# yhinai/EIG-KL-Algorithm

Measured on AMD Instinct MI355X. Metric: wall-clock to final cut (s) + cut size, ibm18.hgr; SpMV GB/s vs HBM peak, lower is better.
Workload: dtype f64 (Lanczos) + f32 (KL gains, bit-exact with cKL)

## Files before the change

### eig-kl-algorithm_amd/csrc/ctx.cpp

```cpp
#include <hip/hip_runtime.h>
#include <rccl/rccl.h>

#include <chrono>
#include <cmath>
#include <cstdlib>
#include <cstring>
#include <atomic>
#include <limits>
#include <map>
#include <memory>
#include <tuple>

#include "ek_internal.hpp"

#ifndef EK_UPD_RED_MAX_NRB
#define EK_UPD_RED_MAX_NRB 256
#endif

#define HIPCHK(call)                                                                                 \
    do {                                                                                             \
        const hipError_t e_ = (call);                                                                \
        if (e_ != hipSuccess) {                                                                      \
            (void)hipGetLastError();     \
            ek::fail(EK_EHIP, "%s failed: %s (%s:%d)", #call, hipGetErrorString(e_), __FILE__, __LINE__); \
        }                                                                                            \
    } while (0)
#define NCCLCHK(call)                                                                                 \
    do {                                                                                              \
        const ncclResult_t r_ = (call);                                                               \
        if (r_ != ncclSuccess) ek::fail(EK_ECOMM, "%s failed: %s", #call, ncclGetErrorString(r_));    \
    } while (0)

namespace {

struct DBuf {
    void* p = nullptr;
    size_t bytes = 0;
    DBuf() = default;
    DBuf(const DBuf&) = delete;
    DBuf& operator=(const DBuf&) = delete;
    ~DBuf() { reset(); }
    void reset() {
        if (p) (void)hipFree(p);
        p = nullptr;
        bytes = 0;
    }
    void ensure(size_t b) {
        if (b <= bytes && p) return;
        reset();
        HIPCHK(hipMalloc(&p, b ? b : 16));
        bytes = b;
    }
    template <class T>
    T* as() const {
        return static_cast<T*>(p);
    }
};

template <class T>
void upload(DBuf& d, const T* h, size_t n, hipStream_t s) {
    d.ensure(n * sizeof(T));
    if (n) HIPCHK(hipMemcpyAsync(d.p, h, n * sizeof(T), hipMemcpyHostToDevice, s));
}

inline int64_t round_up(int64_t x, int64_t m) { return (x + m - 1) / m * m; }

}

struct Uploader {
    ek_ctx* c;
    hipStream_t s;
    unsigned char*& buf;
    size_t& cap;
    size_t off = 0;
    Uploader(ek_ctx* ctx, hipStream_t st, size_t total);
    template <class T>
    void put(DBuf& d, const T* h, size_t n);
};

namespace {
inline int64_t chunk_pad(int64_t n) { return std::max<int64_t>(round_up(n, ek::dev::KL_CHUNK_PAD), ek::dev::KL_CHUNK_PAD); }

}

struct ek_ctx {
    int device = 0;
    int num_cu = 256;
    hipStream_t stream = nullptr;
    hipStream_t kstream = nullptr;
    ncclComm_t comm = nullptr;
    int nranks = 1, rank = 0;
    bool mr = false;
    ek_allgather_fn host_ag = nullptr;
    ek_allreduce_fn host_ar = nullptr;
    void* host_user = nullptr;
    double* stage = nullptr;
    size_t stage_doubles = 0;
    unsigned char* up = nullptr;
    size_t up_bytes = 0;
    unsigned char* kup = nullptr;
    size_t kup_bytes = 0;
    double comm_ms = 0.0;
    int64_t n_ag = 0, n_ar = 0;
    int64_t n = 0, row0 = 0, nrows = 0, nloc = 0, nnz = 0;
    std::vector<int64_t> shard_off;
    int64_t slot = 0;
    DBuf off_d, xexp;
    DBuf spx;
    bool halo = false;
    int halo_calls = 0;
    std::vector<int64_t> hx_base;
    std::vector<int64_t> hx_rcnt;
    std::vector<int64_t> hx_scnt, hx_soff;
    std::vector<int64_t> hx_src;
    std::vector<int32_t> hx_gidx_h;
    int64_t hx_nsend = 0, hx_smax = 0;
    DBuf hx_sidx, hx_sbuf, hx_X, hx_pidx, hx_gidx, hx_gbuf;
    int64_t hx_exchanges = 0, hx_sends = 0, hx_recvs = 0;
    double x_ms = 0.0, ar_ms = 0.0;
    int64_t x_timed = 0, ar_timed = 0;
    bool comm_time = false;
    std::vector<hipEvent_t> cm_ev;
    std::vector<std::pair<int, int>> cm_rec;
    size_t cm_used = 0;
    DBuf own_rowptr, own_col, own_val, own_rb, yown;
    int own_nrb = 0;
    int64_t own_nnz = 0;
    bool own_ready = false;
    hipStream_t gstream = nullptr;
    hipEvent_t ag_ev[2] = {nullptr, nullptr};
    int pn_G = 0, pn_P = 0, pn_pb = 0, pn_max_rows = 0, pn_ndict = 0;
    DBuf pn_wrow, pn_start, pn_word, pn_rid;
    int block_nnz = 1024, nrb_spmv = 0;
    bool spmv_long = true;
    DBuf rb, rowptr, col, val, pk, rel, dict;
    int colbits = 0;
    int64_t mat_bytes = 0;
    DBuf V, Vn, f, w, xfull, part, h1, h2, alpha, offd, fn2, npart, apart, Qd, scal, bov;
    DBuf V32, Vn32;
    DBuf fbk;
    DBuf actr;
    DBuf gctr;
    DBuf wpart, omega, prost, pflags;
    DBuf cflag;
    std::map<std::tuple<int, int, int, const void*, const void*>, hipGraphExec_t> lz_graphs;
    std::map<std::tuple<int, int, int, const void*, const void*>, int> lz_seen;
    std::vector<uint64_t> lz_sig;
    int64_t kl_n = 0, kl_n0 = 0, kl_n1 = 0, kl_nets = 0;
    DBuf kl_rowptr, kl_col, kl_w, kl_side, kl_side_init, kl_locked, kl_gp0, kl_gp1, kl_order0, kl_order1, kl_plist, kl_pinfo0, kl_pinfo1, kl_nd, kl_cinfo0, kl_cinfo1,
        kl_ckey0, kl_ckey1, kl_aux, kl_seg, kl_cutpart, kl_cut0, kl_log, kl_out, kl_sides_tmp, kl_count, kl_netptr, kl_pins;
    bool kl_graph_ready = false, kl_part_ready = false, kl_seg_ok = false, kl_segc_ok = false;
    DBuf kl_segc, kl_wdict;
    DBuf lb_netptr, lb_pins, lb_icnt, lb_rcnt, lb_cur, lb_ip, lb_rp, lb_tiles, lb_inc, lb_scol, lb_sval, lb_tval,
        lb_ulen, lb_len, lb_diag, lb_long, lb_cnt, lb_off, lb_table, lb_flags, lb_codes;
    int kl_nwd = 0, kl_wcolbits = 0;
    std::vector<int32_t> kl_rowptr_h;
    std::vector<hipEvent_t> spmv_ev;
    double* pin = nullptr;
    size_t pin_doubles = 0;
    hipStream_t cstream = nullptr;
    hipEvent_t chk_done[2] = {nullptr, nullptr}, chk_copied[2] = {nullptr, nullptr};
    hipEvent_t fin_ev = nullptr;
    double* chk_pin = nullptr;
    unsigned* chk_word = nullptr;
    unsigned chk_seq = 0;
    double* q_pin = nullptr;
    DBuf fied, sp_out, sp_tmp;
    int64_t fied_n = 0;
    DBuf rk_tmp;
};

Uploader::Uploader(ek_ctx* ctx, hipStream_t st, size_t total)
    : c(ctx), s(st), buf(st == ctx->kstream ? ctx->kup : ctx->up), cap(st == ctx->kstream ? ctx->kup_bytes : ctx->up_bytes) {
    total = (total + 64) * 2;
    if (cap < total) {
        if (buf) HIPCHK(hipHostFree(buf));
        buf = nullptr;
        cap = 0;
        HIPCHK(hipHostMalloc(reinterpret_cast<void**>(&buf), total, hipHostMallocDefault));
        cap = total;
    }
}

template <class T>
void Uploader::put(DBuf& d, const T* h, size_t n) {
    d.ensure(n * sizeof(T));
    if (!n) return;
    off = (off + 63) / 64 * 64;
    if (off + n * sizeof(T) > cap) ek::fail(EK_EINVAL, "upload staging overflow");
    std::memcpy(buf + off, h, n * sizeof(T));
    HIPCHK(hipMemcpyAsync(d.p, buf + off, n * sizeof(T), hipMemcpyHostToDevice, s));
    off += n * sizeof(T);
}

namespace {

void set_device(ek_ctx* c) { HIPCHK(hipSetDevice(c->device)); }

ek_ctx* check_ctx(ek_ctx* c) {
    if (!c) ek::fail(EK_EINVAL, "null ek_ctx");
    set_device(c);
    return c;
}

ek::dev::SpmvMat spmv_mat(const ek_ctx* c) {
    ek::dev::SpmvMat m;
    m.nblocks = c->nrb_spmv;
    if (c->pn_G > 0) {
        m.panel.G = c->pn_G;
        m.panel.P = c->pn_P;
        m.panel.pb = c->pn_pb;
        m.panel.max_rows = c->pn_max_rows;
        m.panel.ndict = c->pn_ndict;
        m.panel.wrow = c->pn_wrow.as<int32_t>();
        m.panel.start = c->pn_start.as<long long>();
        m.panel.word = c->pn_word.as<uint32_t>();
        m.panel.rid = c->pn_rid.as<uint16_t>();
        m.dict = c->dict.as<double>();
        return m;
    }
    m.block_nnz = c->block_nnz;
    m.has_long = c->spmv_long;
    m.desc = c->rb.as<int32_t>();
    m.rowptr = c->rowptr.as<int32_t>();
    if (c->colbits > 0) {
        m.colbits = c->colbits;
        m.pk = c->pk.as<uint32_t>();
        m.rel = c->rel.as<uint16_t>();
        m.dict = c->dict.as<double>();
    } else {
        m.col = c->col.as<int32_t>();
        m.val = c->val.as<double>();
    }
    return m;
}
// ... 2252 lines not shown
        HIPCHK(hipStreamSynchronize(s));
    }
    if (L.proi) {
        ek::dev::ProState ps{};
        HIPCHK(hipMemcpyAsync(&ps, c->prost.p, sizeof(ps), hipMemcpyDeviceToHost, s));
        HIPCHK(hipStreamSynchronize(s));
        if (ps.timeouts)
            ek::fail(EK_EHIP, "Lanczos: %d in-launch wait(s) of the partially reorthogonalised step gave up "
                              "(EK_PRO_INLAUNCH=0 runs the step without them)", ps.timeouts);
    }
    int64_t imax = 0;
    for (int64_t i = 1; i < n; ++i)
        if (std::fabs(v[i]) > std::fabs(v[imax])) imax = i;
    const double sgn = v[imax] < 0 ? -inv : inv;
    c->fied.ensure(size_t(n) * 8);
    ek::dev::fiedler_scale(s, xc, sgn, int(n), c->fied.as<double>());
    HIPCHK(hipGetLastError());
    c->fied_n = n;
    if (c->comm_time) {
        HIPCHK(hipStreamSynchronize(s));
        comm_collect(c);
    }
    c->comm_time = false;
    if (lambda_out) *lambda_out = lambda;
    if (v_out)
        for (int64_t i = 0; i < n; ++i) v_out[i] = v[i] * sgn;
    if (stats) {
        stats->restarts = restarts;
        stats->matvecs = L.matvecs;
        stats->converged = 1;
        stats->residual = std::sqrt(r2);
        stats->total_ms = std::chrono::duration<double, std::milli>(std::chrono::steady_clock::now() - t0).count();
        stats->spmv_ms = L.spmv_ms;
        stats->spmv_timed = L.spmv_timed;
        stats->comm_ms = c->comm_ms;
        stats->allgathers = int32_t(c->n_ag);
        stats->allreduces = int32_t(c->n_ar);
        stats->update32_steps = L.u32_steps;
        stats->update32_fallbacks = 0;
        stats->projected_steps = L.matvecs;
        stats->reprojected = L.repairs;
        stats->ortho_max = ortho_max;
        if (L.pro) {
            ek::dev::ProState ps{};
            HIPCHK(hipMemcpyAsync(&ps, c->prost.p, sizeof(ps), hipMemcpyDeviceToHost, c->stream));
            HIPCHK(hipStreamSynchronize(c->stream));
            stats->projected_steps = ps.projected;
        }
        if (L.b32) {
            unsigned fbn = 0;
            HIPCHK(hipMemcpyAsync(&fbn, c->fbk.p, 4, hipMemcpyDeviceToHost, c->stream));
            HIPCHK(hipStreamSynchronize(c->stream));
            stats->update32_fallbacks = int32_t(fbn);
        }
    }
    return EK_OK;
    EK_CATCH
}

extern "C" {

int ek_kl_graph_setup(ek_ctx* c, int64_t n, const int32_t* rowptr, const int32_t* col, const float* w) {
    EK_TRY
    check_ctx(c);
    ek::PhaseTimer pt("kl_graph_setup");
    if (n <= 0 || n > INT32_MAX || !rowptr || !col || !w) ek::fail(EK_EINVAL, "ek_kl_graph_setup: bad argument");
    const int64_t nnz = rowptr[n];
    for (int64_t r = 0; r < n; ++r)
        if (rowptr[r + 1] < rowptr[r]) ek::fail(EK_EINVAL, "ek_kl_graph_setup: rowptr not monotone");
    {
        std::atomic<bool> bad{false};
        ek::parallel_for(nnz, [&](int64_t lo, int64_t hi) {
            for (int64_t p = lo; p < hi; ++p)
                if (col[p] < 0 || col[p] >= n) bad = true;
        });
        if (bad) ek::fail(EK_EINVAL, "ek_kl_graph_setup: column out of range");
    }
    pt.mark("checks");
    hipStream_t s = c->kstream;
    c->kl_graph_ready = false;
    c->kl_part_ready = false;
    c->kl_n = n;
    c->kl_rowptr_h.assign(rowptr, rowptr + n + 1);
    Uploader up(c, s, (size_t(n) + 1) * 4 + size_t(nnz) * 8 + size_t(nnz) * 4);
    up.put(c->kl_rowptr, rowptr, size_t(n) + 1);
    c->kl_col.ensure((size_t(nnz) + 16) * 4);
    c->kl_w.ensure((size_t(nnz) + 16) * 4);
    HIPCHK(hipMemsetAsync(c->kl_col.as<int32_t>() + nnz, 0, 16 * 4, s));
    HIPCHK(hipMemsetAsync(c->kl_w.as<float>() + nnz, 0, 16 * 4, s));
    if (nnz) {
        unsigned char* const dc = up.buf + up.off;
        unsigned char* const dw = dc + size_t(nnz) * 4;
        ek::parallel_for(nnz, [&](int64_t lo, int64_t hi) {
            std::memcpy(dc + size_t(lo) * 4, col + lo, size_t(hi - lo) * 4);
            std::memcpy(dw + size_t(lo) * 4, w + lo, size_t(hi - lo) * 4);
        });
        HIPCHK(hipMemcpyAsync(c->kl_col.p, dc, size_t(nnz) * 4, hipMemcpyHostToDevice, s));
        HIPCHK(hipMemcpyAsync(c->kl_w.p, dw, size_t(nnz) * 4, hipMemcpyHostToDevice, s));
        up.off += size_t(nnz) * 8;
    }
    pt.mark("CSR staged");
    std::vector<uint32_t> kw;
    std::vector<float> wdict;
    int wcolbits = 0;
    c->kl_segc_ok = !std::getenv("EK_KL_NOSEGC") &&
                    size_t(nnz) * ek::dev::KL_SEGC_PIECES * sizeof(ek::dev::KLInfo) <= (size_t(32) << 30) &&
                    ek::dev::kl_weight_codes(n, nnz, col, w, kw, wdict, wcolbits);
    pt.mark("weight codes");
    c->kl_seg_ok = !c->kl_segc_ok && size_t(nnz) * ek::dev::KL_SEG_LANES * sizeof(ek::dev::KLInfo) <= (size_t(32) << 30);
    if (c->kl_segc_ok) {
        DBuf dkw;
        up.put(dkw, kw.data(), kw.size());
        upload(c->kl_wdict, wdict.data(), wdict.size(), s);
        c->kl_nwd = int(wdict.size());
        c->kl_wcolbits = wcolbits;
        c->kl_seg.reset();
        c->kl_segc.ensure(size_t(std::max<int64_t>(nnz, 1)) * ek::dev::KL_SEGC_PIECES * sizeof(ek::dev::KLInfo));
        ek::dev::kl_build_segc(s, nnz, c->kl_rowptr.as<int32_t>(), c->kl_col.as<int32_t>(), dkw.as<uint32_t>(),
                               c->kl_segc.as<ek::dev::KLInfo>());
        HIPCHK(hipGetLastError());
        HIPCHK(hipStreamSynchronize(s));
    }
    if (c->kl_seg_ok) {
        c->kl_segc.reset();
        c->kl_seg.ensure(size_t(std::max<int64_t>(nnz, 1)) * ek::dev::KL_SEG_LANES * sizeof(ek::dev::KLInfo));
        ek::dev::kl_build_seg(s, nnz, c->kl_rowptr.as<int32_t>(), c->kl_col.as<int32_t>(), c->kl_w.as<float>(),
                              c->kl_seg.as<ek::dev::KLInfo>());
        HIPCHK(hipGetLastError());
    }
    c->kl_side.ensure(size_t(n));
    c->kl_side_init.ensure(size_t(n));
    c->kl_locked.ensure(std::max(size_t(n), size_t((n + 31) / 32) * 8 + 64));
    c->kl_plist.ensure(size_t(n) * 4);
    c->kl_sides_tmp.ensure(size_t(n));
    c->kl_cutpart.ensure(size_t((n + 255) / 256) * 8);
    c->kl_cut0.ensure(16);
    c->kl_out.ensure(sizeof(ek::dev::KLOut));
    c->kl_count.ensure(64);
    pt.mark("segments queued");
    HIPCHK(hipStreamSynchronize(s));
    pt.mark("synchronised");
    c->kl_graph_ready = true;
    c->kl_part_ready = false;
    return EK_OK;
    EK_CATCH
}

int ek_kl_nets_setup(ek_ctx* c, int64_t nets, const int64_t* net_ptr, const int32_t* pins) {
    EK_TRY
    check_ctx(c);
    if (nets < 0 || !net_ptr || (net_ptr[nets] > 0 && !pins)) ek::fail(EK_EINVAL, "ek_kl_nets_setup: bad argument");
    c->kl_nets = nets;
    Uploader up(c, c->kstream, (size_t(nets) + 1) * 8 + size_t(net_ptr[nets]) * 4);
    up.put(c->kl_netptr, net_ptr, size_t(nets) + 1);
    up.put(c->kl_pins, pins, size_t(net_ptr[nets]));
    c->kl_count.ensure(size_t(3) * size_t(ek::dev::net_cut_blocks(nets)) * sizeof(unsigned));
    HIPCHK(hipStreamSynchronize(c->kstream));
    return EK_OK;
    EK_CATCH
}

}

namespace {
void partition_on_device(ek_ctx* c, int64_t n0, int64_t n1) {
    hipStream_t s = c->stream;
    const int64_t n = c->kl_n;
    c->kl_n0 = n0;
    c->kl_n1 = n1;
    {
        c->kl_pinfo0.ensure(size_t(chunk_pad(n0)) * sizeof(ek::dev::KLInfo));
        c->kl_pinfo1.ensure(size_t(chunk_pad(n1)) * sizeof(ek::dev::KLInfo));
        c->kl_nd.ensure(size_t(std::max<int64_t>(n, 1)) * sizeof(ek::dev::KLInfo));
        ek::dev::kl_build_desc(s, int(n), int(n0), int(n1), int(chunk_pad(n0)), int(chunk_pad(n1)),
                               c->kl_order0.as<int32_t>(), c->kl_order1.as<int32_t>(), c->kl_plist.as<uint32_t>(),
                               c->kl_rowptr.as<int32_t>(), c->kl_pinfo0.as<ek::dev::KLInfo>(),
                               c->kl_pinfo1.as<ek::dev::KLInfo>(), c->kl_nd.as<ek::dev::KLInfo>());
        HIPCHK(hipGetLastError());
        const int64_t nnz = c->kl_rowptr_h[size_t(n)];
        c->kl_aux.ensure(size_t(std::max<int64_t>(nnz, 1)) * sizeof(ek::dev::KLInfo));
        ek::dev::kl_build_aux(s, nnz, c->kl_col.as<int32_t>(), c->kl_nd.as<ek::dev::KLInfo>(),
                              c->kl_aux.as<ek::dev::KLInfo>());
        HIPCHK(hipGetLastError());
        c->kl_cinfo0.ensure(size_t((n0 + ek::dev::KL_CHUNK - 1) / ek::dev::KL_CHUNK + 1) * sizeof(ek::dev::KLInfo));
        c->kl_cinfo1.ensure(size_t((n1 + ek::dev::KL_CHUNK - 1) / ek::dev::KL_CHUNK + 1) * sizeof(ek::dev::KLInfo));
    }
    c->kl_gp0.ensure(size_t(chunk_pad(n0)) * 4);
    c->kl_gp1.ensure(size_t(chunk_pad(n1)) * 4);
    HIPCHK(hipMemsetAsync(c->kl_gp0.p, 0xFF, c->kl_gp0.bytes, s));
    HIPCHK(hipMemsetAsync(c->kl_gp1.p, 0xFF, c->kl_gp1.bytes, s));
    c->kl_ckey0.ensure(size_t((n0 + ek::dev::KL_CHUNK - 1) / ek::dev::KL_CHUNK + 1) * 8);
    c->kl_ckey1.ensure(size_t((n1 + ek::dev::KL_CHUNK - 1) / ek::dev::KL_CHUNK + 1) * 8);
    c->kl_log.ensure(size_t(std::max<int64_t>(1, std::min(n0, n1))) * sizeof(ek_swap));
    HIPCHK(hipStreamSynchronize(s));
    c->kl_part_ready = true;
}

}

extern "C" {

int ek_kl_set_partition(ek_ctx* c, const int32_t* order0, int64_t n0, const int32_t* order1, int64_t n1) {
    EK_TRY
    check_ctx(c);
    if (!c->kl_graph_ready) ek::fail(EK_ESTATE, "ek_kl_set_partition before ek_kl_graph_setup");
    const int64_t n = c->kl_n;
    if (n0 < 0 || n1 < 0 || n0 + n1 != n || (n0 && !order0) || (n1 && !order1))
        ek::fail(EK_EINVAL, "ek_kl_set_partition: the two lists must cover all %lld nodes", (long long)n);
    std::vector<uint8_t> side(size_t(n), 2);
    std::vector<uint32_t> plist(size_t(n), 0);
    for (int64_t i = 0; i < n0; ++i) {
        const int32_t u = order0[i];
        if (u < 0 || u >= n || side[size_t(u)] != 2) ek::fail(EK_EINVAL, "ek_kl_set_partition: bad/duplicate node %d", u);
        side[size_t(u)] = 0;
        plist[size_t(u)] = uint32_t(i);
    }
    for (int64_t i = 0; i < n1; ++i) {
        const int32_t u = order1[i];
        if (u < 0 || u >= n || side[size_t(u)] != 2) ek::fail(EK_EINVAL, "ek_kl_set_partition: bad/duplicate node %d", u);
        side[size_t(u)] = 1;
        plist[size_t(u)] = uint32_t(i) | 0x80000000u;
    }
    hipStream_t s = c->stream;
    Uploader up(c, s, size_t(n0) * 4 + size_t(n1) * 4 + size_t(n) + size_t(n) * 4);
    up.put(c->kl_order0, order0, size_t(n0));
    up.put(c->kl_order1, order1, size_t(n1));
    up.put(c->kl_side_init, side.data(), size_t(n));
    up.put(c->kl_plist, plist.data(), size_t(n));
    partition_on_device(c, n0, n1);
    return EK_OK;
    EK_CATCH
}

int ek_kl_set_partition_fiedler(ek_ctx* c, double* median_out, int64_t* n0_out, int64_t* n1_out) {
    EK_TRY
    check_ctx(c);
    if (!c->kl_graph_ready) ek::fail(EK_ESTATE, "ek_kl_set_partition_fiedler before ek_kl_graph_setup");
    const int64_t n = c->kl_n;
    if (c->fied_n != n || n < 1)
        ek::fail(EK_ESTATE, "ek_kl_set_partition_fiedler: no Fiedler vector of %lld entries on this context",
                 (long long)n);
    if (n > INT32_MAX - 1) ek::fail(EK_EINVAL, "ek_kl_set_partition_fiedler: %lld nodes", (long long)n);
    hipStream_t s = c->stream;
    const int ni = int(n);
    const double* v = c->fied.as<double>();
    const size_t tb = ek::dev::split_tmp_bytes(ni);
    c->sp_tmp.ensure(tb);
    c->sp_out.ensure(64);
    const unsigned hi = unsigned(n / 2), lo = n % 2 == 0 ? hi - 1 : hi;
    auto* keys = c->sp_out.as<unsigned long long>();
    ek::dev::split_select(s, c->sp_tmp.p, v, ni, lo, hi, keys);
    unsigned long long kk[2] = {0ull, 0ull};
    HIPCHK(hipMemcpyAsync(kk, keys, 16, hipMemcpyDeviceToHost, s));
    HIPCHK(hipStreamSynchronize(s));
    const double mid[2] = {ek::dev::key_value(kk[0]), ek::dev::key_value(kk[1])};
    const double med = n % 2 == 0 ? (mid[0] + mid[1]) / 2.0 : mid[0];
    c->kl_order0.ensure(size_t(n) * 4);
    c->kl_order1.ensure(size_t(n) * 4);
    c->kl_side_init.ensure(size_t(n));
    c->kl_plist.ensure(size_t(n) * 4);
    unsigned* n0_dev = reinterpret_cast<unsigned*>(c->sp_out.as<unsigned long long>() + 2);
    ek::dev::split_partition(s, c->sp_tmp.p, v, ni, med, c->kl_order0.as<int32_t>(), c->kl_order1.as<int32_t>(),
                             c->kl_plist.as<uint32_t>(), c->kl_side_init.as<uint8_t>(), n0_dev);
    HIPCHK(hipGetLastError());
    unsigned n0u = 0;
    HIPCHK(hipMemcpyAsync(&n0u, n0_dev, 4, hipMemcpyDeviceToHost, s));
    HIPCHK(hipStreamSynchronize(s));
    const int64_t n0 = int64_t(n0u);
    partition_on_device(c, n0, n - n0);
    if (median_out) *median_out = med;
    if (n0_out) *n0_out = n0;
    if (n1_out) *n1_out = n - n0;
    return EK_OK;
// ... 86 lines not shown
        if (pins[p] < 0) ek::fail(EK_EINVAL, "ek_kway_metrics: pin %d", pins[p]);
        top = std::max(top, pins[p]);
    }
    out[0] = out[1] = out[2] = 0;
    if (nets == 0 || npins == 0) return EK_OK;
    const int64_t nodes = int64_t(top) + 1;
    std::vector<uint8_t> part8(static_cast<size_t>(nodes));
    for (int64_t i = 0; i < nodes; ++i) {
        if (part_host[i] < 0 || part_host[i] >= k)
            ek::fail(EK_EINVAL, "ek_kway_metrics: part %d of node %lld outside [0, %d)", part_host[i], (long long)i, k);
        part8[size_t(i)] = uint8_t(part_host[i]);
    }
    hipStream_t s = c->stream;
    const int nb = ek::dev::kway_metrics_blocks(nets);
    DBuf d_ptr, d_pins, d_part, d_out;
    upload(d_ptr, net_ptr, size_t(nets) + 1, s);
    upload(d_pins, pins, size_t(npins), s);
    upload(d_part, part8.data(), size_t(nodes), s);
    d_out.ensure(size_t(3) * size_t(nb) * sizeof(unsigned));
    ek::dev::kway_metrics(s, nets, d_ptr.as<int64_t>(), d_pins.as<int32_t>(), d_part.as<uint8_t>(), d_out.as<unsigned>());
    HIPCHK(hipGetLastError());
    std::vector<unsigned> parts(size_t(3) * size_t(nb));
    HIPCHK(hipMemcpyAsync(parts.data(), d_out.p, parts.size() * sizeof(unsigned), hipMemcpyDeviceToHost, s));
    HIPCHK(hipStreamSynchronize(s));
    for (int j = 0; j < 3; ++j)
        for (int b = 0; b < nb; ++b) out[j] += int64_t(parts[size_t(j) * size_t(nb) + size_t(b)]);
    return EK_OK;
    EK_CATCH
}

int ek_kl_set_partition_bits(ek_ctx* c, int64_t n, const uint8_t* bits) {
    EK_TRY
    if (n < 0 || (n && !bits)) ek::fail(EK_EINVAL, "ek_kl_set_partition_bits: bad argument");
    std::vector<int32_t> o[2];
    o[0].reserve(size_t(n) / 2 + 1);
    o[1].reserve(size_t(n) / 2 + 1);
    for (int64_t i = 0; i < n; ++i) {
        if (bits[i] > 1) ek::fail(EK_EINVAL, "ek_kl_set_partition_bits: bit %d at node %lld", int(bits[i]), (long long)i);
        o[bits[i]].push_back(int32_t(i));
    }
    return ek_kl_set_partition(c, o[0].data(), int64_t(o[0].size()), o[1].data(), int64_t(o[1].size()));
    EK_CATCH
}

}

namespace {

ek::dev::KLDev kl_dev(ek_ctx* c) {
    ek::dev::KLDev d;
    d.n = int(c->kl_n);
    d.nnz = c->kl_rowptr_h.empty() ? 0 : c->kl_rowptr_h.back();
    d.rowptr = c->kl_rowptr.as<int32_t>();
    d.col = c->kl_col.as<int32_t>();
    d.w = c->kl_w.as<float>();
    d.side = c->kl_side.as<uint8_t>();
    d.side_init = c->kl_side_init.as<uint8_t>();
    d.locked = c->kl_locked.as<uint8_t>();
    d.gp0 = c->kl_gp0.as<float>();
    d.gp1 = c->kl_gp1.as<float>();
    d.order0 = c->kl_order0.as<int32_t>();
    d.order1 = c->kl_order1.as<int32_t>();
    d.plist = c->kl_plist.as<uint32_t>();
    d.pinfo0 = c->kl_pinfo0.as<ek::dev::KLInfo>();
    d.pinfo1 = c->kl_pinfo1.as<ek::dev::KLInfo>();
    d.nd = c->kl_nd.as<ek::dev::KLInfo>();
    d.cinfo0 = c->kl_cinfo0.as<ek::dev::KLInfo>();
    d.cinfo1 = c->kl_cinfo1.as<ek::dev::KLInfo>();
    d.aux = c->kl_aux.as<ek::dev::KLInfo>();
    const bool noseg = std::getenv("EK_KL_NOSEG") != nullptr;
    d.seg = c->kl_seg_ok && !noseg ? c->kl_seg.as<ek::dev::KLInfo>() : nullptr;
    d.segc = c->kl_segc_ok && !noseg ? c->kl_segc.as<ek::dev::KLInfo>() : nullptr;
    d.wdict = c->kl_wdict.as<float>();
    d.nwd = c->kl_nwd;
    d.wcolbits = c->kl_wcolbits;
    d.n0 = int(c->kl_n0);
    d.n1 = int(c->kl_n1);
    d.nck0 = int((c->kl_n0 + ek::dev::KL_CHUNK - 1) / ek::dev::KL_CHUNK);
    d.nck1 = int((c->kl_n1 + ek::dev::KL_CHUNK - 1) / ek::dev::KL_CHUNK);
    d.ckey0 = c->kl_ckey0.as<unsigned long long>();
    d.ckey1 = c->kl_ckey1.as<unsigned long long>();
    d.cut_part = c->kl_cutpart.as<double>();
    d.cut0 = c->kl_cut0.as<float>();
    return d;
}

}

extern "C" int ek_kl_run(ek_ctx* c, int32_t limit, ek_swap* log_out, int64_t cap, ek_kl_result* res) {
    EK_TRY
    check_ctx(c);
    if (!c->kl_graph_ready || !c->kl_part_ready) ek::fail(EK_ESTATE, "ek_kl_run before graph/partition setup");
    hipStream_t s = c->stream;
    const int64_t n = c->kl_n;
    const int lim = limit >= 0 ? limit : int(std::log2(double(n))) + 5;
    const auto d = kl_dev(c);
    hipEvent_t e0, e1, e2;
    HIPCHK(hipEventCreate(&e0));
    HIPCHK(hipEventCreate(&e1));
    HIPCHK(hipEventCreate(&e2));
    struct G {
        hipEvent_t a, b, c;
        ~G() {
            (void)hipEventDestroy(a);
            (void)hipEventDestroy(b);
            (void)hipEventDestroy(c);
        }
    } guard{e0, e1, e2};
    const long long dcap = std::max<int64_t>(1, std::min(c->kl_n0, c->kl_n1));
    auto* out = c->kl_out.as<ek::dev::KLOut>();
    HIPCHK(hipEventRecord(e0, s));
    HIPCHK(hipMemcpyAsync(c->kl_side.p, c->kl_side_init.p, size_t(n), hipMemcpyDeviceToDevice, s));
    HIPCHK(hipMemsetAsync(c->kl_locked.p, 0, size_t(n), s));
    ek::dev::kl_prepare(s, d);
    HIPCHK(hipEventRecord(e1, s));
    ek::dev::kl_loop(s, d, lim, c->kl_log.as<ek_swap>(), dcap, out);
    HIPCHK(hipGetLastError());
    HIPCHK(hipEventRecord(e2, s));
    const bool nets = c->kl_nets > 0;
    const int ncb = nets ? ek::dev::net_cut_blocks(c->kl_nets) : 0;
    std::vector<unsigned> cparts(size_t(3) * size_t(ncb));
    if (nets) {
        ek::dev::kl_replay(s, int(n), c->kl_side_init.as<uint8_t>(), c->kl_log.as<ek_swap>(), &out->best_iter, dcap,
                           c->kl_sides_tmp.as<uint8_t>());
        ek::dev::net_cut(s, c->kl_nets, c->kl_netptr.as<int64_t>(), c->kl_pins.as<int32_t>(),
                         c->kl_side_init.as<uint8_t>(), c->kl_sides_tmp.as<uint8_t>(), c->kl_side.as<uint8_t>(),
                         c->kl_count.as<unsigned>());
    }
    ek::dev::KLOut ho{};
    HIPCHK(hipMemcpyAsync(&ho, out, sizeof ho, hipMemcpyDeviceToHost, s));
    if (nets)
        HIPCHK(hipMemcpyAsync(cparts.data(), c->kl_count.p, cparts.size() * sizeof(unsigned), hipMemcpyDeviceToHost, s));
    HIPCHK(hipStreamSynchronize(s));
    if (ho.status == 3u)
        ek::fail(EK_EHIP, "KL swap loop: an in-launch wait gave up (EK_KL_PIPE=0 runs the loop without them)");
    unsigned long long hc[3] = {0, 0, 0};
    for (int k = 0; k < 3; ++k)
        for (int b = 0; b < ncb; ++b) hc[k] += cparts[size_t(k) * size_t(ncb) + size_t(b)];
    if (log_out && cap > 0) {
        const int64_t k = std::min<int64_t>(cap, ho.iterations);
        if (k) HIPCHK(hipMemcpy(log_out, c->kl_log.p, size_t(k) * sizeof(ek_swap), hipMemcpyDeviceToHost));
    }
    if (res) {
        float loop_ms = 0.f, prep_ms = 0.f;
        HIPCHK(hipEventElapsedTime(&prep_ms, e0, e1));
        HIPCHK(hipEventElapsedTime(&loop_ms, e1, e2));
        res->iterations = ho.iterations;
        res->initial_cut = ho.initial_cut;
        res->best_cut = ho.best_cut;
        res->final_cut = ho.final_cut;
        res->best_iter = ho.best_iter;
        res->net_cut_initial = nets ? int64_t(hc[0]) : -1;
        res->net_cut_best = nets ? int64_t(hc[1]) : -1;
        res->net_cut_final = nets ? int64_t(hc[2]) : -1;
        res->loop_ms = loop_ms;
        if (std::getenv("EK_KL_PROF") && ho.prof[13] == 0x9199ull) {
            const double sw = double(std::max<long long>(1, ho.iterations)), gs = double(std::max<unsigned long long>(1, ho.prof[2]));
            std::fprintf(stderr, "[kl-pipe] %lld swaps: speculated %.1f %%, hits %.1f %%; loop %.0f cycles/swap\n",
                         (long long)ho.iterations, 100.0 * double(ho.prof[0]) / sw, 100.0 * double(ho.prof[1]) / gs,
                         double(ho.prof[12]) / sw);
            std::fprintf(stderr, "[kl-pipe] gain wave 0, cycles/swap: pair wait %.0f, P %.0f, speculative rows %.0f (per "
                         "speculation), pair->barrier1 %.0f\n", double(ho.prof[3]) / gs, double(ho.prof[4]) / gs,
                         double(ho.prof[5]) / double(std::max<unsigned long long>(1, ho.prof[0])), double(ho.prof[6]) / gs);
            std::fprintf(stderr, "[kl-pipe] W wave, cycles/swap: barrier-2 wait %.0f, selection %.0f, pair->barrier1 %.0f, "
                         "G2 span %.0f; G2a wave's G2 span %.0f\n", double(ho.prof[7]) / sw, double(ho.prof[8]) / sw,
                         double(ho.prof[9]) / sw, double(ho.prof[10]) / sw, double(ho.prof[11]) / sw);
// ... 48 lines not shown
```

### eig-kl-algorithm_amd/csrc/ek_internal.hpp

```cpp
#pragma once

#include <cstdint>
#include <cstdio>
#include <functional>
#include <memory>
#include <utility>
#include <string>
#include <type_traits>
#include <vector>

#include "../../include/eigkl.h"

namespace ek {
void set_error(const char* fmt, ...) __attribute__((format(printf, 1, 2)));
struct Error {
    int code;
};
[[noreturn]] void fail(int code, const char* fmt, ...) __attribute__((format(printf, 2, 3)));
int guard_exceptions();

int host_threads();
struct ThreadCap {
    explicit ThreadCap(int cap);
    ~ThreadCap();
    int prev;
};
struct PhaseTimer {
    explicit PhaseTimer(const char* tag);
    void mark(const char* what);
    const char* tag;
    double t0;
    bool on;
};
void cold_stamp(const char* what);
template <class F>
void parallel_for(int64_t n, F&& fn);
template <class F>
void run_threads(int T, F&& fn);
void pool_run(int T, void (*fn)(void*, int), void* ctx);
}

#define EK_TRY try {
#define EK_CATCH \
    }            \
    catch (...) { return ek::guard_exceptions(); }

namespace ek {
template <class T>
struct default_init_allocator : std::allocator<T> {
    template <class U>
    struct rebind {
        using other = default_init_allocator<U>;
    };
    default_init_allocator() = default;
    template <class U>
    default_init_allocator(const default_init_allocator<U>&) noexcept {}
    template <class U>
    void construct(U* p) noexcept {
        ::new (static_cast<void*>(p)) U;
    }
    template <class U, class... A>
    void construct(U* p, A&&... a) {
        ::new (static_cast<void*>(p)) U(std::forward<A>(a)...);
    }
};
template <class T>
using dvec = std::vector<T, default_init_allocator<T>>;
}

struct ek_hgr {
    int64_t nets = 0, nodes = 0;
    ek::dvec<int64_t> net_ptr;
    ek::dvec<int32_t> pins;
    int64_t raw_pairs = -1;
};
namespace ek {
int spmv_setup_hgr(ek_ctx* c, const ek_hgr& h, int32_t* on_device);
}

struct ek_csr {
    int64_t nrows = 0;
    int32_t value_bytes = 8;
    ek::dvec<int32_t> rowptr, col, nfwd;
    ek::dvec<double> val64;
    ek::dvec<float> val32;
};

namespace ek {
void build_laplacian(const ek_hgr& h, ek_csr& out);
void build_laplacian_rows(const ek_hgr& h, int64_t r0, int64_t r1, ek_csr& out);
void build_kl_graph(const ek_hgr& h, ek_csr& out);
void hashtable_order(const uint32_t* keys, int64_t cnt, uint32_t* out, std::vector<int32_t>& scratch);
void hashtable_order(const uint32_t* keys, int64_t cnt, uint32_t* out, std::vector<int32_t>& scratch,
                     std::vector<int32_t>& bk0, std::vector<int32_t>& bk1);
// ... 220 lines not shown
    double* a3 = nullptr;
    double* npart = nullptr;
    const float* V32 = nullptr;
    unsigned* fb = nullptr;
    int merged = 0;
    int cgw = 0;
    int seg0 = 0, m = 0;
    double thresh = 0.0, eps1 = 0.0;
    unsigned* tix = nullptr;
    int rev = 0;
    int cap = 0;
};
int gemvt_pro_capacity(bool nt, bool wide, bool merged, bool b32u, int num_cu);
int gemvt_pro_grid(int nrb, int ncgl, int ldv, bool merged);
void finalize_step(hipStream_t s, const double* npart, int nb, double* fn2_out, const double* h1,
                   const double* h2, int step, double* alpha, double* offd, const double* a3 = nullptr,
                   const double* fn2_i = nullptr, const double* bov_i = nullptr);
void three_term(hipStream_t s, int ldv, const double* apart, int nparts, double* alpha_io, const double* w,
                const double* vi, const double* vim1, const double* fn2_i, const double* bov_i, double* fp,
                float* v32col = nullptr);
void gemm_vq(hipStream_t s, int ldv, const double* V, int m, const double* Q, int kk, double* out,
             float* out32 = nullptr);
void inject_random(hipStream_t s, double* f, int ldv, long long row0, long long nrows, unsigned long long st0);
void zero_pad_rows(hipStream_t s, double* V, int ldv, int nreal, int ncols);
size_t split_tmp_bytes(int n);
void fiedler_scale(hipStream_t s, const double* x, double sgn, int n, double* out);
void split_select(hipStream_t s, void* tmp, const double* v, int n, unsigned k0, unsigned k1,
                  unsigned long long* keys_out);
double key_value(unsigned long long key);
void split_partition(hipStream_t s, void* tmp, const double* v, int n, double med, int32_t* order0, int32_t* order1,
                     uint32_t* plist, uint8_t* side, unsigned* n0_out);
void axpby_norm(hipStream_t s, int ldv, double* f, double sigma, const double* x, double hk, double* npart);
void scale_sub_mean(hipStream_t s, int ldv, double* x, int nreal, const double* mean_sum, double inv_n);
void sum_partial(hipStream_t s, int ldv, const double* x, int nreal, double* npart, int squares);
void resid_partial(hipStream_t s, int ldv, const double* w, const double* x, double lambda, int nreal, double* part);
void start_vector(hipStream_t s, int ldv, long long row0, int nreal, double* x);

#ifndef EK_KL_THREADS
#define EK_KL_THREADS 512
#endif
constexpr int KL_LOOP_THREADS = EK_KL_THREADS;
#ifndef EK_KL_CHUNK
#define EK_KL_CHUNK 2048
#endif
constexpr int KL_CHUNK = EK_KL_CHUNK;
#ifndef EK_KL_CHUNK_GB
#define EK_KL_CHUNK_GB 4096
#endif
constexpr int KL_CHUNK_GB = EK_KL_CHUNK_GB;
constexpr int KL_CHUNK_PAD = KL_CHUNK > KL_CHUNK_GB ? KL_CHUNK : KL_CHUNK_GB;
static_assert(KL_CHUNK_PAD % KL_CHUNK == 0 && KL_CHUNK_PAD % KL_CHUNK_GB == 0, "chunk sizes must nest");
struct alignas(16) KLInfo {
    int32_t a, b, c, d;
};
struct KLDev {
    int n = 0;
    long long nnz = 0;
    const int32_t* rowptr = nullptr;
    const int32_t* col = nullptr;
    const float* w = nullptr;
    uint8_t* side = nullptr;
    const uint8_t* side_init = nullptr;
    uint8_t* locked = nullptr;
    float* gp0 = nullptr;
    float* gp1 = nullptr;
    const int32_t* order0 = nullptr;
    const int32_t* order1 = nullptr;
    const uint32_t* plist = nullptr;
    int n0 = 0, n1 = 0, nck0 = 0, nck1 = 0;
    unsigned long long* ckey0 = nullptr;
    unsigned long long* ckey1 = nullptr;
    double* cut_part = nullptr;
    float* cut0 = nullptr;
    const KLInfo* pinfo0 = nullptr;
    const KLInfo* pinfo1 = nullptr;
    const KLInfo* nd = nullptr;
    KLInfo* cinfo0 = nullptr;
    KLInfo* cinfo1 = nullptr;
    const KLInfo* aux = nullptr;
    const KLInfo* seg = nullptr;
    const KLInfo* segc = nullptr;
    const float* wdict = nullptr;
    int nwd = 0, wcolbits = 0;
};
constexpr int KL_SEGC_PIECES = 8;
constexpr int KL_WDICT_CAP = 4096;
constexpr int KL_SEG_LANES = 16;
constexpr int KL_ITEM_CAP = 256;
size_t kl_loop_lds_bytes(const KLDev& d, bool bitmaps = true, bool fixed = false);
struct KLOut {
    long long iterations;
    long long best_iter;
    float initial_cut, best_cut, final_cut;
    unsigned int status;
    unsigned long long prof[16];
    unsigned long long warr[42];
};
void kl_prepare(hipStream_t s, const KLDev& d);
void kl_build_aux(hipStream_t s, int64_t nnz, const int32_t* col, const KLInfo* nd, KLInfo* aux);
void kl_build_seg(hipStream_t s, int64_t nnz, const int32_t* rowptr, const int32_t* col, const float* w, KLInfo* seg);
void kl_build_desc(hipStream_t s, int n, int n0, int n1, int pad0, int pad1, const int32_t* order0,
                   const int32_t* order1, const uint32_t* plist, const int32_t* rowptr, KLInfo* p0, KLInfo* p1,
                   KLInfo* nd);
void kl_build_segc(hipStream_t s, int64_t nnz, const int32_t* rowptr, const int32_t* col, const uint32_t* kw,
                   KLInfo* segc);
bool kl_weight_codes(int64_t n, int64_t nnz, const int32_t* col, const float* w, std::vector<uint32_t>& kw,
                     std::vector<float>& wdict, int& wcolbits);
void kl_loop(hipStream_t s, const KLDev& d, int limit, ek_swap* log, long long cap, KLOut* out);
void kl_replay(hipStream_t s, int n, const uint8_t* side_init, const ek_swap* log, const long long* count,
               long long cap, uint8_t* sides_out);
int net_cut_blocks(int64_t nets);
void net_cut(hipStream_t s, int64_t nets, const int64_t* net_ptr, const int32_t* pins, const uint8_t* side_a,
             const uint8_t* side_b, const uint8_t* side_c, unsigned* part);

size_t rank_tmp_bytes(int n);
void rank_partition(hipStream_t s, void* tmp, const double* v, int n, const unsigned long long* key, unsigned n1,
                    int32_t* order0, int32_t* order1, uint32_t* plist, uint8_t* side, unsigned* n0_out);
int kway_metrics_blocks(int64_t nets);
void kway_metrics(hipStream_t s, int64_t nets, const int64_t* net_ptr, const int32_t* pins, const uint8_t* part,
                  unsigned* out);

}
}

#include <algorithm>
#include <thread>
template <class F>
void ek::parallel_for(int64_t n, F&& fn) {
    const int64_t T = std::min<int64_t>(host_threads(), std::max<int64_t>(1, n / 4096));
    if (T <= 1) {
        fn(int64_t(0), n);
        return;
    }
    run_threads(int(T), [&](int t) { fn(n * t / T, n * (t + 1) / T); });
}

template <class F>
void ek::run_threads(int T, F&& fn) {
    if (T <= 1) {
        if (T == 1) fn(0);
        return;
    }
    using Fn = std::remove_reference_t<F>;
    pool_run(T, [](void* c, int t) { (*static_cast<Fn*>(c))(t); }, const_cast<void*>(static_cast<const void*>(&fn)));
}
```

### eig-kl-algorithm_amd/csrc/kernels_kl.hip

```cpp
#include <hip/hip_runtime.h>

#include <cfloat>
#include <algorithm>
#include <atomic>
#include <cstdlib>
#include <cstring>

#include "ek_internal.hpp"

#ifndef EK_KL_PREFETCH
#define EK_KL_PREFETCH 1
#endif
#ifndef EK_KL_NEXT
#define EK_KL_NEXT 0
#endif
#ifndef EK_E_TWO_TRIPS
#define EK_E_TWO_TRIPS 1
#endif
#ifndef EK_G1_DRAIN
#define EK_G1_DRAIN 0
#endif
#ifndef EK_PIPE_SLEEP
#define EK_PIPE_SLEEP 1
#endif
// ... 248 lines not shown
                     (2 * size_t(fixed ? KL_FIX_NCK : kl_sel_pad(d.nck0, d.nck1)) + nck + KL_ITEM_CAP + 4 + 2 * KL_AB_CAP + 2) * 8 +
                     (2 * nck + KL_ITEM_CAP + 4 + 4 + 4) * 4 + 2 * words * 4 +
                     (fixed ? size_t(KL_WDICT_CAP) : size_t(d.segc ? d.nwd : 0)) * 4 +
                     128;
    return b <= 152 * 1024 ? b : 0;
}

template <int CH = KL_CHUNK>
__device__ __forceinline__ u64 chunk_rescan(const float* __restrict__ gp, const KLInfo* __restrict__ pinfo, int s,
                                            int c, int skip, int lane, KLInfo* info, bool* mine) {
    float g[CH / 64];
#pragma unroll
    for (int q = 0; q < CH / 64; ++q) g[q] = gp[c * CH + q * 64 + lane];
    int bq;
    const u64 k = lane_best<CH / 64>(g, s, c * CH, lane, skip, &bq);
    const int bp = c * CH + (bq < 0 ? 0 : bq) * 64 + lane;
    const u64 m = wave_max_u64(k);
    const u64 bal = __ballot(m != 0ull && k == m);
    *mine = bal ? (lane == __ffsll((long long)bal) - 1) : (lane == 0);
    KLInfo inf{0, 0, 0, 0};
    if (bal && *mine) {
        const int4 x = *reinterpret_cast<const int4*>(pinfo + bp);
        inf = KLInfo{x.x, x.y, x.z, x.w};
    }
    __builtin_amdgcn_s_waitcnt(0x0F70);
    *info = inf;
    return m;
}

template <int NQ>
__device__ __forceinline__ u64 chunk_rescan2(const float* __restrict__ gp, const KLInfo* __restrict__ pinfo, int s,
                                             int p0, int skip, int lane, KLInfo* info, bool* mine) {
    float g[NQ];
#pragma unroll
    for (int q = 0; q < NQ; ++q) g[q] = gp[p0 + q * 64 + lane];
    int bq;
    const u64 k = lane_best<NQ>(g, s, p0, lane, skip, &bq);
    const u64 m = wave_max_u64(k);
    const u64 bal = __ballot(m != 0ull && k == m);
    *mine = bal ? (lane == __ffsll((long long)bal) - 1) : (lane == 0);
    KLInfo inf{0, 0, 0, 0};
    if (bal && *mine) {
        const int4 x = *reinterpret_cast<const int4*>(pinfo + p0 + bq * 64 + lane);
        inf = KLInfo{x.x, x.y, x.z, x.w};
    }
    *info = inf;
    return m;
}

template <int NQ>
__device__ __forceinline__ u64 chunk_rescan1(const float* __restrict__ gp, const KLInfo* __restrict__ pinfo, int s,
                                             int p0, int skip, int lane, KLInfo* info, bool* mine) {
    float g[NQ];
    int4 pi[NQ];
#pragma unroll
    for (int q = 0; q < NQ; ++q) {
        const int p = p0 + q * 64 + lane;
        g[q] = gp[p];
        pi[q] = *reinterpret_cast<const int4*>(pinfo + p);
    }
    float bg = s ? FLT_MAX : -FLT_MAX;
    int bq = -1;
    int4 bi = make_int4(0, 0, 0, 0);
#pragma unroll
    for (int q = 0; q < NQ; ++q) {
        const float gq = p0 + q * 64 + lane == skip ? __builtin_nanf("") : g[q];
        const bool better = s ? gq < bg : gq > bg;
        bg = better ? gq : bg;
        bq = better ? q : bq;
        bi.x = better ? pi[q].x : bi.x;
        bi.y = better ? pi[q].y : bi.y;
        bi.z = better ? pi[q].z : bi.z;
        bi.w = better ? pi[q].w : bi.w;
    }
    const int bp = p0 + (bq < 0 ? 0 : bq) * 64 + lane;
    const u64 k = bq < 0 ? 0ull : (s ? key_min(bg, bp) : key_max(bg, bp));
    const u64 m = wave_max_u64(k);
    const u64 bal = __ballot(m != 0ull && k == m);
    *mine = bal ? (lane == __ffsll((long long)bal) - 1) : (lane == 0);
    *info = bal ? KLInfo{bi.x, bi.y, bi.z, bi.w} : KLInfo{0, 0, 0, 0};
    return m;
}

template <bool PROF, bool SEGC, bool GB = false, bool FIX = false>
__global__ __launch_bounds__(KL_LOOP_THREADS) void k_kl_swap_loop(KLDev d, int limit, ek_swap* __restrict__ log,
                                                                  long long cap, KLOut* __restrict__ out) {
    constexpr int NW = KL_LOOP_THREADS / 64;
    constexpr int CH = GB ? KL_CHUNK_GB : KL_CHUNK;
    constexpr int E_PARTS = KL_E_PARTS, NQ_E = CH / 64 / E_PARTS;
    constexpr int W_W = NW - 1, W_EA = NW - 2, W_EB = W_EA - E_PARTS, NG = W_EB - E_PARTS + 1;
    constexpr int W_PF = W_W;
    constexpr int W_FLIP = W_EA - 1;
    static_assert(NG == KL_LOOP_THREADS / 64 - 1 - 2 * KL_E_PARTS, "kl_loop_lds_bytes reserves staging for NG gain waves");
    extern __shared__ __attribute__((aligned(16))) unsigned char smem[];
    const int tid = threadIdx.x, lane = tid & 63, wv = tid >> 6;
    const int half = lane >> 5, hl = lane & 31;
    const int nsel = FIX ? KL_FIX_NCK : kl_sel_pad(d.nck0, d.nck1);
    const int words = (d.n + 31) / 32;
    const int lc0 = FIX ? KL_FIX_NCK : d.nck0, lc1 = FIX ? KL_FIX_NCK : d.nck1;
    KLInfo* ci0 = reinterpret_cast<KLInfo*>(smem);
    KLInfo* ci1 = ci0 + lc0;
    KLInfo* it_info = ci1 + lc1;
    KLInfo* er_info = it_info + KL_ITEM_CAP;
    KLInfo* ab_info = er_info + 2 * E_PARTS;
    KLInfo* nx_info = ab_info + 2 * KL_AB_CAP;
    int4* sg_stage = reinterpret_cast<int4*>(nx_info + 2);
    u64* ck0 = reinterpret_cast<u64*>(sg_stage + NG * KL_STAGE_ROWS * KL_STAGE_ROW);
    u64* ck1 = ck0 + nsel;
    u64* ckn0 = ck1 + nsel;
    u64* ckn1 = ckn0 + lc0;
    u64* it_key = ckn1 + lc1;
    u64* er_key = it_key + KL_ITEM_CAP;
    u64* ab_key = er_key + 2 * E_PARTS;
    u64* nx_key = ab_key + 2 * KL_AB_CAP;
    int* dtag0 = reinterpret_cast<int*>(nx_key + 2);
    int* dtag1 = dtag0 + lc0;
    int* ctag0 = dtag1 + lc1;
    int* ctag1 = ctag0 + lc0;
    int* it_cs = ctag1 + lc1;
    int* s_stop = it_cs + KL_ITEM_CAP;
    int* ab_cnt = s_stop + 4;
    int* nx_ok = ab_cnt + 4;
    uint32_t* s_side = GB ? reinterpret_cast<uint32_t*>(d.locked)
                     : FIX ? reinterpret_cast<uint32_t*>(nx_ok + 4 + KL_WDICT_CAP)
                           : reinterpret_cast<uint32_t*>(nx_ok + 4);
    uint32_t* s_lock = s_side + words;
    float* s_wd = (GB || FIX) ? reinterpret_cast<float*>(nx_ok + 4) : reinterpret_cast<float*>(s_lock + words);
    auto bits_at = [&](const uint32_t* p) -> uint32_t {
        if constexpr (GB) return __hip_atomic_load(p, __ATOMIC_RELAXED, __HIP_MEMORY_SCOPE_AGENT);
        else return *p;
    };
    if constexpr (SEGC)
        for (int i = tid; i < d.nwd; i += KL_LOOP_THREADS) s_wd[i] = d.wdict[i];
    for (int i = tid; i < nsel; i += KL_LOOP_THREADS) {
        ck0[i] = i < d.nck0 ? d.ckey0[i] : 0ull;
        ck1[i] = i < d.nck1 ? d.ckey1[i] : 0ull;
    }
    for (int i = tid; i < d.nck0; i += KL_LOOP_THREADS) {
        ckn0[i] = d.ckey0[i];
        ci0[i] = d.cinfo0[i];
        dtag0[i] = ctag0[i] = -1;
    }
    for (int i = tid; i < d.nck1; i += KL_LOOP_THREADS) {
        ckn1[i] = d.ckey1[i];
        ci1[i] = d.cinfo1[i];
        dtag1[i] = ctag1[i] = -1;
    }
    for (int i = tid; i < words; i += KL_LOOP_THREADS) {
        if constexpr (GB) {
            __hip_atomic_store(s_side + i, side_word(d.side_init, d.n, i), __ATOMIC_RELAXED, __HIP_MEMORY_SCOPE_AGENT);
            __hip_atomic_store(s_lock + i, 0u, __ATOMIC_RELAXED, __HIP_MEMORY_SCOPE_AGENT);
        } else {
            s_side[i] = side_word(d.side_init, d.n, i);
            s_lock[i] = 0u;
        }
    }
    if constexpr (GB) asm volatile("s_waitcnt vmcnt(0)" ::: "memory");
    if (tid < 4) s_stop[tid] = tid == 3 ? -1 : 0;
    if (tid < 4) ab_cnt[tid] = 0;
    if (tid < 4) nx_ok[tid] = 0;
    __syncthreads();
    float cut = *d.cut0, best = cut;
    long long best_it = 0, it = 0;
    unsigned term = 0;
    unsigned long long tph[12] = {}, tstamp = 0;
    int4 pf_inf = make_int4(0, 0, 0, 0);
    int4 pf_seg = make_int4(0, 0, 0, 0), pf_seg2 = make_int4(0, 0, 0, 0), pf_aux = make_int4(0, 0, 0, 0);
    int pf_col = 0;
    float pf_w = 0.0f;
    uint32_t pf_sink = 0u;
    unsigned long long pf_hit_a = 0, pf_hit_b = 0;
    const unsigned long long c_start = PROF ? __builtin_amdgcn_s_memtime() : 0ull;
    const unsigned long long r_start = PROF ? __builtin_amdgcn_s_memrealtime() : 0ull;
    auto stamp = [&](int ph) {
        if constexpr (PROF) {
            if (tid == 0) {
                const unsigned long long t = __builtin_amdgcn_s_memrealtime();
                if (ph >= 0) tph[ph] += t - tstamp;
                tstamp = t;
            }
        }
    };
    unsigned long long w_top = 0, w_arr1 = 0, w_arr2 = 0, w_g2a = 0, w_sel = 0, w_g2r = 0;
    for (;; ++it) {
        stamp(-1);
        if constexpr (PROF) w_top = __builtin_amdgcn_s_memtime();
        if constexpr (EK_KL_PREFETCH) {
            if (wv == W_PF) {
                const int rp = __builtin_amdgcn_readlane(pf_inf.y, 0), ln = __builtin_amdgcn_readlane(pf_inf.z, 0);
                const int rq = __builtin_amdgcn_readlane(pf_inf.y, 32), lq = __builtin_amdgcn_readlane(pf_inf.z, 32);
                const int r0 = half ? rq : rp, l0 = half ? lq : ln;
                if (l0 > 0) {
                    const int last = r0 + l0 - 1;
                    const int rs = min(r0 + hl, last);
                    if constexpr (SEGC) {
                        pf_seg = *reinterpret_cast<const int4*>(d.segc + size_t(rs) * KL_SEGC_PIECES);
                    } else if (d.seg) {
                        pf_seg = *reinterpret_cast<const int4*>(d.seg + size_t(rs) * KL_SEG_LANES);
                        pf_seg2 = *reinterpret_cast<const int4*>(d.seg + size_t(rs) * KL_SEG_LANES + KL_SEG_LANES / 2);
                    }
                    pf_aux = *reinterpret_cast<const int4*>(d.aux + min(r0 + 8 * hl, last));
                    pf_col = d.col[min(r0 + 32 * hl, last)];
                    pf_w = d.w[min(r0 + 32 * hl, last)];
                }
            }
        }
#if EK_G1_DRAIN
        if (wv < NG) __builtin_amdgcn_s_waitcnt(0x0F70);
#endif
        u64 k0 = 0ull, k1 = 0ull;
        v4i dA = v4i{0, 0, 0, 0}, dB = v4i{0, 0, 0, 0};
        bool sel = true;
        if constexpr (EK_KL_NEXT) {
            const int ok = nx_ok[0];
            const u64 nk0 = nx_key[0], nk1 = nx_key[1];
            const v4i ni0 = *reinterpret_cast<const v4i*>(nx_info), ni1 = *reinterpret_cast<const v4i*>(nx_info + 1);
            if (__builtin_amdgcn_readfirstlane(ok)) {
                sel = false;
                k0 = readlane_u64(nk0, 0);
                k1 = readlane_u64(nk1, 0);
                dA = v4i{__builtin_amdgcn_readfirstlane(ni0.x), __builtin_amdgcn_readfirstlane(ni0.y),
                         __builtin_amdgcn_readfirstlane(ni0.z), 0};
                dB = v4i{__builtin_amdgcn_readfirstlane(ni1.x), __builtin_amdgcn_readfirstlane(ni1.y),
                         __builtin_amdgcn_readfirstlane(ni1.z), 0};
            }
        }
        if (sel) {
            u64 k = 0ull;
            const u64* ck = half ? ck1 : ck0;
            if (nsel <= 4 * 32) {
                u64 kv[4];
#pragma unroll
                for (int u = 0; u < 4; ++u) kv[u] = ck[min(hl + 32 * u, nsel - 1)];
#pragma unroll
                for (int u = 0; u < 4; ++u) k = kv[u] > k ? kv[u] : k;
            } else {
                for (int c0 = hl; c0 < nsel; c0 += 8 * 32) {
                    u64 kv[8];
#pragma unroll
                    for (int u = 0; u < 8; ++u) kv[u] = ck[min(c0 + 32 * u, nsel - 1)];
#pragma unroll
                    for (int u = 0; u < 8; ++u) k = kv[u] > k ? kv[u] : k;
                }
            }
            k = half_max_u64(k);
            k0 = readlane_u64(k, 0);
            k1 = readlane_u64(k, 32);
        }
        if (k0 == 0ull || k1 == 0ull) break;
        const int posA = int(~uint32_t(k0 & 0xffffffffull)), posB = int(~uint32_t(k1 & 0xffffffffull));
        const int cA = posA / CH, cB = posB / CH;
        if (sel) {
            dA = *reinterpret_cast<const v4i*>(ci0 + cA);
            dB = *reinterpret_cast<const v4i*>(ci1 + cB);
        }
        const int A = dA.x, pa = dA.y, la = dA.z, B = dB.x, pb = dB.y, lb = dB.z;
        if constexpr (PROF && EK_KL_PREFETCH) {
            if (wv == W_PF) {
                pf_hit_a += __builtin_amdgcn_readlane(pf_inf.x, 0) == A && __builtin_amdgcn_readlane(pf_inf.z, 0) > 0;
                pf_hit_b += __builtin_amdgcn_readlane(pf_inf.x, 32) == B && __builtin_amdgcn_readlane(pf_inf.z, 32) > 0;
            }
        }
        stamp(0);
        if constexpr (PROF) {
            if (A == -7) s_stop[2] = 0;
            w_sel += __builtin_amdgcn_s_memtime() - w_top;
        }
        auto side_now = [&](int x) -> bool {
            return (((bits_at(s_side + (x >> 5)) >> (x & 31)) & 1u) != 0) ^ (x == A) ^ (x == B);
        };
        auto locked_now = [&](int x) -> bool {
            return ((bits_at(s_lock + (x >> 5)) >> (x & 31)) & 1u) || x == A || x == B;
        };
        const int tot = la + lb;
        const int tag = int(it);
        const int abp = EK_KL_NEXT ? (tag & 1) * 2 : 0;
        if (wv == W_W) {
            float gA = 0.f, gB = 0.f;
            if (lane == 0) {
                gA = d.gp0[posA];
                gB = d.gp1[posB];
            }
            float wab = 0.0f;
            bool found = false;
            for (int i = lane; i < la; i += 64)
                if (d.col[pa + i] == B) {
                    wab = d.w[pa + i];
                    found = true;
                }
            const u64 bal = __ballot(found);
            if (bal) wab = __shfl(wab, __ffsll((long long)bal) - 1, 64);
            if (lane == 0) {
                d.gp0[posA] = __builtin_nanf("");
                d.gp1[posB] = __builtin_nanf("");
                const float gain = gA - gB - 2.0f * wab;
                cut -= gain;
                if (cut < best) {
                    best = cut;
                    best_it = it + 1;
                }
                if (it < cap)
                    log[it] = ek_swap{uint32_t(it + 1), uint32_t(A), uint32_t(B), gA, gB, gain, cut, 0u};
                int stop = 0;
                if (gain <= 0.0f) {
                    if (++term > unsigned(limit)) stop = 1;
                } else {
                    term = 0;
                }
                if (it + 1 >= d.n0 || it + 1 >= d.n1) stop = 1;
                s_stop[it & 1] = stop;
            }
            if constexpr (EK_KL_PREFETCH)
                pf_sink ^= uint32_t(pf_seg.x ^ pf_seg.w ^ pf_seg2.x ^ pf_aux.x ^ pf_col) ^ __float_as_uint(pf_w);
        } else if (wv > W_EB - E_PARTS) {
            const int s = wv <= W_EB ? 1 : 0, part = (s ? W_EB : W_EA) - wv;
            const int p0 = (s ? cB : cA) * CH + part * NQ_E * 64;
            if constexpr (EK_E_SLEEP > 0) __builtin_amdgcn_s_sleep(EK_E_SLEEP);
            KLInfo info;
            bool mine;
#if EK_E_TWO_TRIPS
            const u64 kk = s ? chunk_rescan2<NQ_E>(d.gp1, d.pinfo1, 1, p0, posB, lane, &info, &mine)
                             : chunk_rescan2<NQ_E>(d.gp0, d.pinfo0, 0, p0, posA, lane, &info, &mine);
#else
            const u64 kk = s ? chunk_rescan1<NQ_E>(d.gp1, d.pinfo1, 1, p0, posB, lane, &info, &mine)
                             : chunk_rescan1<NQ_E>(d.gp0, d.pinfo0, 0, p0, posA, lane, &info, &mine);
#endif
            if (mine) {
                er_key[s * E_PARTS + part] = kk;
                er_info[s * E_PARTS + part] = info;
            }
        } else {
            constexpr int LPR = SEGC ? 4 : 8, RPW = 64 / LPR;
            int4* stage = sg_stage + wv * KL_STAGE_ROWS * KL_STAGE_ROW;
            for (int i0 = wv * RPW; i0 < tot; i0 += NG * RPW) {
                constexpr int PPL = (SEGC ? KL_SEGC_PIECES : KL_SEG_LANES) / LPR;
                const int gi = i0 + lane / LPR, j8 = lane % LPR, srow = lane / LPR;
                const int pg = gi < tot ? (gi < la ? pa + gi : pb + gi - la) : pa;
                int4 piece[PPL];
                if constexpr (SEGC) {
#pragma unroll
                    for (int r = 0; r < PPL; ++r)
                        piece[r] = *reinterpret_cast<const int4*>(d.segc + size_t(pg) * KL_SEGC_PIECES + j8 + LPR * r);
                } else {
#pragma unroll
                    for (int r = 0; r < PPL; ++r)
                        piece[r] = d.seg ? *reinterpret_cast<const int4*>(d.seg + size_t(pg) * KL_SEG_LANES + j8 + LPR * r)
                                         : make_int4(0, 0, 0, 0);
                }
                const int4 a = j8 == 0 ? *reinterpret_cast<const int4*>(d.aux + pg) : make_int4(0, 0, 0, 0);
                if constexpr (PROF) {
                    if (tid == 0 && (piece[0].x == -12345 || a.x == -12345)) s_stop[2] = 0;
                }
                stamp(10);
                v2f ie_seg = {0.0f, 0.0f};
                if constexpr (SEGC) {
                    const uint32_t cmask = (1u << d.wcolbits) - 1u;
                    v2f cc[PPL][4];
#pragma unroll
                    for (int r = 0; r < PPL; ++r) {
                        const uint32_t wv4[4] = {uint32_t(piece[r].x), uint32_t(piece[r].y), uint32_t(piece[r].z),
                                                 uint32_t(piece[r].w)};
#pragma unroll
                        for (int k = 0; k < 4; ++k) {
                            const float wk = s_wd[wv4[k] >> d.wcolbits];
                            const bool ek = side_now(int(wv4[k] & cmask));
                            cc[r][k] = v2f{ek ? 0.0f : wk, ek ? wk : 0.0f};
                        }
                    }
                    const int lenq = a.z;
#pragma unroll
                    for (int st = 0; st < 4 * PPL; ++st) {
                        if (!__ballot(lenq > 4 * st)) break;
                        v2f x = ie_seg;
#pragma unroll
                        for (int k = 0; k < 4; ++k) x += cc[st / 4][k];
                        ie_seg.x = quad_bcast(x.x, st % 4);
                        ie_seg.y = quad_bcast(x.y, st % 4);
                    }
                } else if (d.seg) {
#pragma unroll
                    for (int r = 0; r < PPL; ++r) {
                        const int4 pc = piece[r];
                        const bool e0 = side_now(pc.x);
                        const bool e1 = side_now(pc.z);
                        const float w0 = __int_as_float(pc.y), w1 = __int_as_float(pc.w);
                        stage[srow * KL_STAGE_ROW + j8 + LPR * r] =
                            make_int4(__float_as_int(e0 ? 0.0f : w0), __float_as_int(e0 ? w0 : 0.0f),
                                      __float_as_int(e1 ? 0.0f : w1), __float_as_int(e1 ? w1 : 0.0f));
                    }
                }
                stamp(11);
                if (j8 != 0 || gi >= tot) continue;
                const int i = gi;
                int4 sg[KL_SEG_LANES];
                if (!SEGC && d.seg) {
#pragma unroll
                    for (int j = 0; j < KL_SEG_LANES; ++j) sg[j] = stage[srow * KL_STAGE_ROW + j];
                }
                const int u = a.x, rp = a.y, len = a.z;
                const bool act = !locked_now(u);
                const uint32_t pl = uint32_t(a.w);
                const int ls = int(pl >> 31), pp = int(pl & 0x7fffffffu), c = pp / CH;
                const bool ab = ls ? c == cB : c == cA;
                const u64 K = (ls ? ck1 : ck0)[c];
                stamp(6);
                float internal = 0.0f, external = 0.0f;
                {
                    int q = 0;
                    if constexpr (SEGC) {
                        internal = ie_seg.x;
                        external = ie_seg.y;
                        q = 2 * KL_SEG_LANES;
                    } else if (d.seg) {
                        v2f ie = {0.0f, 0.0f};
#pragma unroll
                        for (int b = 0; b < KL_SEG_LANES / 4; ++b) {
                            if (!__ballot(len > 8 * b)) break;
#pragma unroll
                            for (int j = 4 * b; j < 4 * b + 4; ++j) {
                                ie += v2f{__int_as_float(sg[j].x), __int_as_float(sg[j].y)};
                                ie += v2f{__int_as_float(sg[j].z), __int_as_float(sg[j].w)};
                            }
                        }
                        internal = ie.x;
                        external = ie.y;
                        q = 2 * KL_SEG_LANES;
                    }
                    if constexpr (PROF) {
                        if (q < len) atomicAdd(&s_stop[2], 1);
                    }
                    for (; q < len; q += 16) {
                        int cc[16];
                        float ww[16];
#pragma unroll
                        for (int k2 = 0; k2 < 16; ++k2) {
                            cc[k2] = d.col[rp + q + k2];
                            ww[k2] = q + k2 < len ? d.w[rp + q + k2] : 0.0f;
                        }
#pragma unroll
                        for (int k2 = 0; k2 < 16; ++k2) {
                            cc[k2] = q + k2 < len ? cc[k2] : 0;
                            const bool e = side_now(cc[k2]);
                            internal += e ? 0.0f : ww[k2];
                            external += e ? ww[k2] : 0.0f;
                        }
                    }
                }
                if constexpr (PROF) {
                    if (tid == 0 && internal == -1.0f) s_stop[2] = 0;
                }
                stamp(7);
                int cs = -1;
                u64 kn = 0ull;
                KLInfo inf{0, 0, 0, 0};
                if (act) {
                    const float g = external - internal;
                    const int s = ls;
                    (s ? d.gp1 : d.gp0)[pp] = g;
                    kn = key_max(s ? -g : g, pp);
                    if (ab) {
                        const int slot = atomicAdd(&ab_cnt[abp + s], 1);
                        if (slot < KL_AB_CAP) {
                            ab_key[s * KL_AB_CAP + slot] = kn;
                            ab_info[s * KL_AB_CAP + slot] = KLInfo{u, rp, len, pp};
                        }
                    } else {
                        if (uint32_t(~uint32_t(K & 0xffffffffull)) == uint32_t(pp) && kn < K) {
                            (s ? dtag1 : dtag0)[c] = tag;
                            s_stop[3] = tag;
                        } else if (kn > K) {
                            atomicMax(&(s ? ckn1 : ckn0)[c], kn);
                            if (i >= KL_ITEM_CAP) {
                                (s ? dtag1 : dtag0)[c] = tag;
                                s_stop[3] = tag;
                            }
                        }
                    }
                    cs = int((pl & 0x80000000u) | uint32_t(c));
                    inf = KLInfo{u, rp, len, pp};
                }
                if (i < KL_ITEM_CAP) {
                    it_key[i] = kn;
                    it_cs[i] = cs;
                    it_info[i] = inf;
                }
            }
        }
        stamp(1);
        if constexpr (PROF) w_arr1 += __builtin_amdgcn_s_memtime() - w_top;
        __syncthreads();
        stamp(2);
        const bool any_tag = s_stop[3] == tag;
        if (wv == W_EA) {
            const int s = half, cS = s ? cB : cA;
            u64 rk[E_PARTS];
            v4i rf[E_PARTS];
#pragma unroll
            for (int q = 0; q < E_PARTS; ++q) {
                rk[q] = er_key[s * E_PARTS + q];
                rf[q] = *reinterpret_cast<const v4i*>(er_info + s * E_PARTS + q);
            }
            const int cnt = ab_cnt[abp + s];
            const int hs = hl < KL_AB_CAP ? hl : KL_AB_CAP - 1;
            const u64 bk_raw = ab_key[s * KL_AB_CAP + hs];
            const v4i bf = *reinterpret_cast<const v4i*>(ab_info + s * KL_AB_CAP + hs);
            const bool have = hl < cnt && hl < KL_AB_CAP;
            const u64 bk = have ? bk_raw : 0ull;
            if (hl == 0) ab_cnt[(EK_KL_NEXT ? 2 - abp : 0) + s] = 0;
            u64 R = rk[0];
            v4i Rf = rf[0];
#pragma unroll
            for (int q = 1; q < E_PARTS; ++q) {
                const bool b = rk[q] > R;
                R = b ? rk[q] : R;
                Rf.x = b ? rf[q].x : Rf.x;
                Rf.y = b ? rf[q].y : Rf.y;
                Rf.z = b ? rf[q].z : Rf.z;
                Rf.w = b ? rf[q].w : Rf.w;
            }
            const int Rpos = int(~uint32_t(R & 0xffffffffull));
            const bool stale = have && R != 0ull && bf.w == Rpos && bk < R;
            if constexpr (PROF) {
                if (stale && bf.x == -7) s_stop[2] = 0;
                w_g2r += __builtin_amdgcn_s_memtime() - w_top;
            }
            const u64 hmask = s ? 0xffffffff00000000ull : 0x00000000ffffffffull;
            const bool st = (__ballot(stale) & hmask) != 0ull || cnt > KL_AB_CAP;
            u64 m = 0ull;
            if (__ballot(cnt > 0)) m = half_max_u64(bk);
            if (!st) {
                if (m > R) {
                    if (have && bk == m) {
                        (s ? ck1 : ck0)[cS] = m;
                        (s ? ckn1 : ckn0)[cS] = m;
                        *reinterpret_cast<v4i*>((s ? ci1 : ci0) + cS) = bf;
                    }
                } else if (hl == 0) {
                    (s ? ck1 : ck0)[cS] = R;
                    (s ? ckn1 : ckn0)[cS] = R;
                    *reinterpret_cast<v4i*>((s ? ci1 : ci0) + cS) = Rf;
                }
            }
            const bool stA = __builtin_amdgcn_readlane(int(st), 0) != 0, stB = __builtin_amdgcn_readlane(int(st), 32) != 0;
            if constexpr (PROF) {
                if (lane == 0) atomicAdd(&s_stop[2], 1000000 * (int(stA) + int(stB)));
            }
            for (int q = 0; q < 2; ++q) {
                if (!(q ? stB : stA)) continue;
                KLInfo info;
                bool mine;
                const u64 kk = q ? chunk_rescan<CH>(d.gp1, d.pinfo1, 1, cB, -1, lane, &info, &mine)
                                 : chunk_rescan<CH>(d.gp0, d.pinfo0, 0, cA, -1, lane, &info, &mine);
                if (mine) {
                    (q ? ck1 : ck0)[q ? cB : cA] = kk;
                    (q ? ckn1 : ckn0)[q ? cB : cA] = kk;
                    (q ? ci1 : ci0)[q ? cB : cA] = info;
                }
            }
        }
        stamp(3);
        if constexpr (PROF) w_g2a += __builtin_amdgcn_s_memtime() - w_top;
        if (wv == W_FLIP && lane == 0) {
            if constexpr (GB) {
                __hip_atomic_fetch_or(s_side + (A >> 5), 1u << (A & 31), __ATOMIC_RELAXED, __HIP_MEMORY_SCOPE_AGENT);
                __hip_atomic_fetch_and(s_side + (B >> 5), ~(1u << (B & 31)), __ATOMIC_RELAXED, __HIP_MEMORY_SCOPE_AGENT);
                __hip_atomic_fetch_or(s_lock + (A >> 5), 1u << (A & 31), __ATOMIC_RELAXED, __HIP_MEMORY_SCOPE_AGENT);
                __hip_atomic_fetch_or(s_lock + (B >> 5), 1u << (B & 31), __ATOMIC_RELAXED, __HIP_MEMORY_SCOPE_AGENT);
                asm volatile("s_waitcnt vmcnt(0)" ::: "memory");
            } else {
                atomicOr(&s_side[A >> 5], 1u << (A & 31));
                atomicAnd(&s_side[B >> 5], ~(1u << (B & 31)));
                atomicOr(&s_lock[A >> 5], 1u << (A & 31));
                atomicOr(&s_lock[B >> 5], 1u << (B & 31));
            }
        }
        if constexpr (EK_KL_NEXT) {
            if (wv == W_PF) {
                const int s = half, cS = s ? cB : cA, nck = s ? d.nck1 : d.nck0;
                const u64* ckn = s ? ckn1 : ckn0;
                u64 k = 0ull;
                for (int c0 = hl; c0 < nck; c0 += 4 * 32) {
                    u64 kv[4];
#pragma unroll
                    for (int u = 0; u < 4; ++u) kv[u] = ckn[min(c0 + 32 * u, nck - 1)];
#pragma unroll
                    for (int u = 0; u < 4; ++u) {
                        const u64 v = kv[u] & (min(c0 + 32 * u, nck - 1) == cS ? 0ull : ~0ull);
                        k = v > k ? v : k;
                    }
                }
                u64 rk[E_PARTS];
                v4i rf[E_PARTS];
#pragma unroll
                for (int q = 0; q < E_PARTS; ++q) {
                    rk[q] = er_key[s * E_PARTS + q];
                    rf[q] = *reinterpret_cast<const v4i*>(er_info + s * E_PARTS + q);
                }
                const int cnt = ab_cnt[abp + s];
                const int hs = hl < KL_AB_CAP ? hl : KL_AB_CAP - 1;
                const u64 bk_raw = ab_key[s * KL_AB_CAP + hs];
                const v4i bf = *reinterpret_cast<const v4i*>(ab_info + s * KL_AB_CAP + hs);
                const int il = lane < tot ? lane : 0;
                const u64 ik = it_key[il];
                const int ics = it_cs[il];
                const v4i iinf = *reinterpret_cast<const v4i*>(it_info + il);
                const bool have = hl < cnt && hl < KL_AB_CAP;
                const u64 bk = have ? bk_raw : 0ull;
                u64 R = rk[0];
                v4i Rf = rf[0];
#pragma unroll
                for (int q = 1; q < E_PARTS; ++q) {
                    const bool b = rk[q] > R;
                    R = b ? rk[q] : R;
                    Rf.x = b ? rf[q].x : Rf.x;
                    Rf.y = b ? rf[q].y : Rf.y;
                    Rf.z = b ? rf[q].z : Rf.z;
                    Rf.w = b ? rf[q].w : Rf.w;
                }
                const int Rpos = int(~uint32_t(R & 0xffffffffull));
                const bool stale = have && R != 0ull && bf.w == Rpos && bk < R;
                const bool bad = any_tag || tot > 64 || __ballot(stale || cnt > KL_AB_CAP) != 0ull;
                const u64 m = __ballot(cnt > 0) ? half_max_u64(bk) : 0ull;
                const u64 kS = m > R ? m : R;
                k = kS > k ? kS : k;
                k = half_max_u64(k);
                const u64 kA = readlane_u64(k, 0), kB = readlane_u64(k, 32);
                const bool own = lane < tot && ics != -1;
                const u64 mA = __ballot(own && ics >= 0 && ik == kA), mB = __ballot(own && ics < 0 && ik == kB);
                const u64 mS = s ? mB : mA;
                v4i desc = Rf;
                if (mA) {
                    const int l = __ffsll((long long)mA) - 1;
                    const v4i t = v4i{__builtin_amdgcn_readlane(iinf.x, l), __builtin_amdgcn_readlane(iinf.y, l),
                                      __builtin_amdgcn_readlane(iinf.z, l), 0};
                    if (!s) desc = t;
                }
                if (mB) {
                    const int l = __ffsll((long long)mB) - 1;
                    const v4i t = v4i{__builtin_amdgcn_readlane(iinf.x, l), __builtin_amdgcn_readlane(iinf.y, l),
                                      __builtin_amdgcn_readlane(iinf.z, l), 0};
                    if (s) desc = t;
                }
                if (!mS && k != R && k != 0ull)
                    desc = *reinterpret_cast<const v4i*>((s ? ci1 : ci0) + int(~uint32_t(k & 0xffffffffull)) / CH);
                if (hl == 0) {
                    nx_key[s] = k;
                    *reinterpret_cast<v4i*>(nx_info + s) = desc;
                }
                if (lane == 0) nx_ok[0] = bad ? 0 : 1;
                if constexpr (EK_KL_PREFETCH) pf_inf = make_int4(desc.x, desc.y, desc.z, 0);
            }
        } else if constexpr (EK_KL_PREFETCH) {
            if (wv == W_PF) {
                const u64* ckn = half ? ckn1 : ckn0;
                const int nck = half ? d.nck1 : d.nck0, cS = half ? cB : cA;
                u64 k = 0ull;
                for (int c0 = hl; c0 < nck; c0 += 4 * 32) {
                    u64 kv[4];
#pragma unroll
                    for (int u = 0; u < 4; ++u) kv[u] = ckn[min(c0 + 32 * u, nck - 1)];
#pragma unroll
                    for (int u = 0; u < 4; ++u) {
                        const u64 v = kv[u] & (min(c0 + 32 * u, nck - 1) == cS ? 0ull : ~0ull);
                        k = v > k ? v : k;
                    }
                }
#pragma unroll
                for (int q = 0; q < E_PARTS; ++q) {
                    const u64 v = er_key[half * E_PARTS + q];
                    k = v > k ? v : k;
                }
                k = half_max_u64(k);
                pf_inf = make_int4(0, 0, 0, 0);
                if (k != 0ull && hl == 0)
                    pf_inf = *reinterpret_cast<const int4*>((half ? d.pinfo1 : d.pinfo0) + int(~uint32_t(k & 0xffffffffull)));
            }
        }
        if (wv == W_EB || wv == W_EB - 1) {
            for (int i = (W_EB - wv) * 64 + lane; i < tot && i < KL_ITEM_CAP; i += 128) {
                const int cs = it_cs[i];
                const u64 kn = it_key[i];
                const int4 inf = *reinterpret_cast<const int4*>(it_info + i);
                if (cs == -1) continue;
                const int s = int(uint32_t(cs) >> 31), c = cs & 0x7fffffff;
                const u64 kmerged = (s ? ckn1 : ckn0)[c];
                const int dt = (s ? dtag1 : dtag0)[c];
                if ((s ? c == cB : c == cA) || dt == tag) continue;
                (s ? ck1 : ck0)[c] = kmerged;
                if (kmerged == kn) *reinterpret_cast<int4*>((s ? ci1 : ci0) + c) = inf;
            }
        }
        for (int i = wv; any_tag && i < tot; i += NW) {
            int cs;
            if (i < KL_ITEM_CAP) cs = it_cs[i];
            else {
                const int u = i < la ? d.col[pa + i] : d.col[pb + i - la];
                cs = locked_now(u) ? -1 : int((uint32_t(d.nd[u].c) & 0x80000000u) |
                                                                     ((uint32_t(d.nd[u].c) & 0x7fffffffu) / CH));
            }
            if (cs == -1) continue;
            const int s = int(uint32_t(cs) >> 31), c = cs & 0x7fffffff;
            if ((s ? dtag1 : dtag0)[c] != tag) continue;
            int claimed = 0;
            if (lane == 0) claimed = atomicMax(&(s ? ctag1 : ctag0)[c], tag) < tag;
            if (!__shfl(claimed, 0, 64)) continue;
            if constexpr (PROF) {
                if (lane == 0) atomicAdd(&s_stop[2], 1);
            }
            KLInfo info;
            bool mine;
            const u64 kk = s ? chunk_rescan<CH>(d.gp1, d.pinfo1, 1, c, -1, lane, &info, &mine)
                             : chunk_rescan<CH>(d.gp0, d.pinfo0, 0, c, -1, lane, &info, &mine);
            if (mine) {
                (s ? ck1 : ck0)[c] = kk;
                (s ? ckn1 : ckn0)[c] = kk;
                (s ? ci1 : ci0)[c] = info;
            }
        }
        stamp(4);
        if constexpr (PROF) w_arr2 += __builtin_amdgcn_s_memtime() - w_top;
        __syncthreads();
        stamp(5);
        if (s_stop[it & 1]) {
            ++it;
            break;
        }
    }
    __syncthreads();
    for (int u = tid; u < d.n; u += KL_LOOP_THREADS) d.side[u] = uint8_t((bits_at(s_side + (u >> 5)) >> (u & 31)) & 1u);
    if (EK_KL_PREFETCH && wv == W_PF && lane == 0 && pf_sink == 0x5a5a5a5au) out->prof[12] = 1ull;
    if (lane == 0 && (NW <= 8 || wv < 8)) {
        out->warr[wv] = w_arr1;
        out->warr[8 + wv] = w_arr2;
        out->warr[16 + wv] = w_g2a;
        out->warr[24 + wv] = w_sel;
        out->warr[32 + wv] = w_g2r;
        if (wv == W_PF) {
            out->warr[40] = pf_hit_a;
            out->warr[41] = pf_hit_b;
        }
    }
    if (wv == W_W && lane == 0) {
        out->iterations = it;
        out->best_iter = best_it;
        out->initial_cut = *d.cut0;
        out->best_cut = best;
        out->final_cut = cut;
        out->status = 2u;
    }
    if (tid == 0) {
        if constexpr (PROF) {
            tph[8] = 100ull * (unsigned long long)(s_stop[2] / 1000000);
            tph[9] = 100ull * (unsigned long long)(s_stop[2] % 1000000);
        }
        for (int i = 0; i < 12; ++i) out->prof[i] = tph[i];
        out->prof[14] = PROF ? __builtin_amdgcn_s_memtime() - c_start : 0ull;
        out->prof[15] = PROF ? __builtin_amdgcn_s_memrealtime() - r_start : 0ull;
    }
}


template <bool PROF, bool SEGC>
__global__ __launch_bounds__(KL_LOOP_THREADS) void k_kl_swap_pipe(KLDev d, int limit, ek_swap* __restrict__ log,
                                                                  long long cap, KLOut* __restrict__ out) {
    constexpr int NW = KL_LOOP_THREADS / 64;
    constexpr int E_PARTS = KL_E_PARTS, NQ_E = KL_CHUNK / 64 / E_PARTS;
    constexpr int W_W = NW - 1, W_EA = NW - 2, W_EB = W_EA - E_PARTS, NG = W_EB - E_PARTS + 1;
    constexpr int W_FLIP = W_EA - 1;
    constexpr int LPR = SEGC ? 4 : 8, RPW = 64 / LPR;
    constexpr int PPL = (SEGC ? KL_SEGC_PIECES : KL_SEG_LANES) / LPR;
    constexpr unsigned POLL_CAP = 1u << 22;
    static_assert(NG == KL_LOOP_THREADS / 64 - 1 - 2 * KL_E_PARTS, "kl_loop_lds_bytes reserves staging for NG gain waves");
    extern __shared__ __attribute__((aligned(16))) unsigned char smem[];
    const int tid = threadIdx.x, lane = tid & 63, wv = tid >> 6;
    const int half = lane >> 5, hl = lane & 31;
    const int nsel = kl_sel_pad(d.nck0, d.nck1);
    const int words = (d.n + 31) / 32;
    KLInfo* ci0 = reinterpret_cast<KLInfo*>(smem);
    KLInfo* ci1 = ci0 + d.nck0;
    KLInfo* it_info = ci1 + d.nck1;
    KLInfo* er_info = it_info + KL_ITEM_CAP;
    KLInfo* ab_info = er_info + 2 * E_PARTS;
    KLInfo* nx_info = ab_info + 2 * KL_AB_CAP;
    int4* sg_stage = reinterpret_cast<int4*>(nx_info + 2);
    u64* ck0 = reinterpret_cast<u64*>(sg_stage + NG * KL_STAGE_ROWS * KL_STAGE_ROW);
    u64* ck1 = ck0 + nsel;
    u64* ckn0 = ck1 + nsel;
    u64* ckn1 = ckn0 + d.nck0;
    u64* it_key = ckn1 + d.nck1;
    u64* er_key = it_key + KL_ITEM_CAP;
    u64* ab_key = er_key + 2 * E_PARTS;
    u64* nx_key = ab_key + 2 * KL_AB_CAP;
    int* dtag0 = reinterpret_cast<int*>(nx_key + 2);
    int* dtag1 = dtag0 + d.nck0;
    int* ctag0 = dtag1 + d.nck1;
    int* ctag1 = ctag0 + d.nck0;
    int* it_cs = ctag1 + d.nck1;
    int* s_stop = it_cs + KL_ITEM_CAP;
    int* ab_cnt = s_stop + 4;
    int* sync = ab_cnt + 4;
    uint32_t* s_side = reinterpret_cast<uint32_t*>(sync + 4);
    uint32_t* s_lock = s_side + words;
    float* s_wd = reinterpret_cast<float*>(s_lock + words);
    u64* sp = reinterpret_cast<u64*>((reinterpret_cast<uintptr_t>(s_wd + (SEGC ? d.nwd : 0)) + 15) & ~uintptr_t(15));
    if constexpr (SEGC)
        for (int i = tid; i < d.nwd; i += KL_LOOP_THREADS) s_wd[i] = d.wdict[i];
    for (int i = tid; i < nsel; i += KL_LOOP_THREADS) {
        ck0[i] = i < d.nck0 ? d.ckey0[i] : 0ull;
        ck1[i] = i < d.nck1 ? d.ckey1[i] : 0ull;
    }
    for (int i = tid; i < d.nck0; i += KL_LOOP_THREADS) {
        ckn0[i] = d.ckey0[i];
        ci0[i] = d.cinfo0[i];
        dtag0[i] = ctag0[i] = -1;
    }
    for (int i = tid; i < d.nck1; i += KL_LOOP_THREADS) {
        ckn1[i] = d.ckey1[i];
        ci1[i] = d.cinfo1[i];
        dtag1[i] = ctag1[i] = -1;
    }
    for (int i = tid; i < words; i += KL_LOOP_THREADS) {
        s_side[i] = side_word(d.side_init, d.n, i);
        s_lock[i] = 0u;
    }
    if (tid < 4) s_stop[tid] = tid == 3 ? -1 : 0;
    if (tid < 4) ab_cnt[tid] = 0;
    if (tid < 4) sync[tid] = 0;
    __syncthreads();
    float cut = *d.cut0, best = cut;
    long long best_it = 0, it = 0;
    unsigned term = 0;
    unsigned long long pc[12] = {};
    unsigned long long t_a = 0, t_b = 0;
    auto now = [&]() -> unsigned long long { return PROF ? __builtin_amdgcn_s_memtime() : 0ull; };
    const unsigned long long t_start = now();

    auto aborted = [&]() -> bool { return __hip_atomic_load(&sync[2], __ATOMIC_RELAXED, __HIP_MEMORY_SCOPE_WORKGROUP) != 0; };
    auto give_up = [&]() { __hip_atomic_store(&sync[2], 1, __ATOMIC_RELAXED, __HIP_MEMORY_SCOPE_WORKGROUP); };
    auto arrive = [&]() {
        __builtin_amdgcn_fence(__ATOMIC_RELEASE, "workgroup");
        if (lane == 0) __hip_atomic_fetch_add(&sync[0], 1, __ATOMIC_RELAXED, __HIP_MEMORY_SCOPE_WORKGROUP);
    };
    auto wait_word = [&](int w, int target) -> bool {
        for (unsigned p = 0;; ++p) {
            const int v = __hip_atomic_load(&sync[w], __ATOMIC_RELAXED, __HIP_MEMORY_SCOPE_WORKGROUP);
            if (__builtin_amdgcn_readfirstlane(v) >= target) break;
            if constexpr (EK_PIPE_SLEEP > 0) __builtin_amdgcn_s_sleep(EK_PIPE_SLEEP);
            if ((p & 255u) == 255u) {
                if (__builtin_amdgcn_readfirstlane(int(aborted()))) return false;
                if (p >= POLL_CAP) {
                    give_up();
                    return false;
                }
            }
        }
        __builtin_amdgcn_fence(__ATOMIC_ACQUIRE, "workgroup");
        return true;
    };

    auto g1_rows = [&](int i0, int pa, int la, int pb, int lb, auto&& side_fn, auto&& lock_fn, int& gi_o, int4& a_o,
                       float& in_o, float& ex_o, bool& act_o) {
        const int tot = la + lb;
        const int gi = i0 + lane / LPR, j8 = lane % LPR, srow = lane / LPR;
        int pg = gi < tot ? (gi < la ? pa + gi : pb + gi - la) : pa;
        pg = min(max(pg, 0), int(d.nnz) - 1);
        int4 piece[PPL];
        if constexpr (SEGC) {
#pragma unroll
            for (int r = 0; r < PPL; ++r)
                piece[r] = *reinterpret_cast<const int4*>(d.segc + size_t(pg) * KL_SEGC_PIECES + j8 + LPR * r);
        } else {
#pragma unroll
            for (int r = 0; r < PPL; ++r)
                piece[r] = d.seg ? *reinterpret_cast<const int4*>(d.seg + size_t(pg) * KL_SEG_LANES + j8 + LPR * r)
                                 : make_int4(0, 0, 0, 0);
        }
        const int4 a = j8 == 0 ? *reinterpret_cast<const int4*>(d.aux + pg) : make_int4(0, 0, 0, 0);
        v2f ie_seg = {0.0f, 0.0f};
        int4* stage = sg_stage + wv * KL_STAGE_ROWS * KL_STAGE_ROW;
        if constexpr (SEGC) {
            const uint32_t cmask = (1u << d.wcolbits) - 1u;
            v2f cc[PPL][4];
#pragma unroll
            for (int r = 0; r < PPL; ++r) {
                const uint32_t wv4[4] = {uint32_t(piece[r].x), uint32_t(piece[r].y), uint32_t(piece[r].z),
                                         uint32_t(piece[r].w)};
#pragma unroll
                for (int k = 0; k < 4; ++k) {
                    const float wk = s_wd[wv4[k] >> d.wcolbits];
                    const bool ek = side_fn(int(wv4[k] & cmask));
                    cc[r][k] = v2f{ek ? 0.0f : wk, ek ? wk : 0.0f};
                }
            }
            const int lenq = a.z;
#pragma unroll
            for (int st = 0; st < 4 * PPL; ++st) {
                if (!__ballot(lenq > 4 * st)) break;
                v2f x = ie_seg;
#pragma unroll
                for (int k = 0; k < 4; ++k) x += cc[st / 4][k];
                ie_seg.x = quad_bcast(x.x, st % 4);
                ie_seg.y = quad_bcast(x.y, st % 4);
            }
        } else if (d.seg) {
#pragma unroll
            for (int r = 0; r < PPL; ++r) {
                const int4 pc = piece[r];
                const bool e0 = side_fn(pc.x);
                const bool e1 = side_fn(pc.z);
                const float w0 = __int_as_float(pc.y), w1 = __int_as_float(pc.w);
                stage[srow * KL_STAGE_ROW + j8 + LPR * r] =
                    make_int4(__float_as_int(e0 ? 0.0f : w0), __float_as_int(e0 ? w0 : 0.0f),
                              __float_as_int(e1 ? 0.0f : w1), __float_as_int(e1 ? w1 : 0.0f));
            }
        }
        gi_o = -1;
        if (j8 != 0 || gi >= tot) return;
        const int len = a.z, rp = a.y;
        float internal = 0.0f, external = 0.0f;
        int q = 0;
        if constexpr (SEGC) {
            internal = ie_seg.x;
            external = ie_seg.y;
            q = 2 * KL_SEG_LANES;
        } else if (d.seg) {
            int4 sg[KL_SEG_LANES];
#pragma unroll
            for (int j = 0; j < KL_SEG_LANES; ++j) sg[j] = stage[srow * KL_STAGE_ROW + j];
            v2f ie = {0.0f, 0.0f};
#pragma unroll
            for (int b = 0; b < KL_SEG_LANES / 4; ++b) {
                if (!__ballot(len > 8 * b)) break;
#pragma unroll
                for (int j = 4 * b; j < 4 * b + 4; ++j) {
                    ie += v2f{__int_as_float(sg[j].x), __int_as_float(sg[j].y)};
                    ie += v2f{__int_as_float(sg[j].z), __int_as_float(sg[j].w)};
                }
            }
            internal = ie.x;
            external = ie.y;
            q = 2 * KL_SEG_LANES;
        }
        for (; q < len; q += 16) {
            int cc[16];
            float ww[16];
            const int lim = int(d.nnz) - 1;
#pragma unroll
            for (int k2 = 0; k2 < 16; ++k2) {
                cc[k2] = d.col[min(rp + q + k2, lim + 16)];
                ww[k2] = q + k2 < len ? d.w[min(rp + q + k2, lim)] : 0.0f;
            }
#pragma unroll
            for (int k2 = 0; k2 < 16; ++k2) {
                cc[k2] = q + k2 < len ? cc[k2] : 0;
                const bool e = side_fn(cc[k2]);
                internal += e ? 0.0f : ww[k2];
                external += e ? ww[k2] : 0.0f;
            }
        }
        gi_o = gi;
        a_o = a;
        in_o = internal;
        ex_o = external;
        act_o = !lock_fn(a.x);
    };
    auto g1_commit = [&](int gi, int4 a, float internal, float external, bool act, int cA, int cB, int tag,
                         int abp) {
        if (gi < 0) return;
        const int u = a.x, rp = a.y, len = a.z;
        const uint32_t pl = uint32_t(a.w);
        const int ls = int(pl >> 31), pp = int(pl & 0x7fffffffu), c = pp / KL_CHUNK;
        const bool ab = ls ? c == cB : c == cA;
        const u64 K = (ls ? ck1 : ck0)[c];
        int cs = -1;
        u64 kn = 0ull;
        KLInfo inf{0, 0, 0, 0};
        if (act) {
            const float g = external - internal;
            const int s = ls;
            (s ? d.gp1 : d.gp0)[pp] = g;
            kn = key_max(s ? -g : g, pp);
            if (ab) {
                const int slot = atomicAdd(&ab_cnt[abp + s], 1);
                if (slot < KL_AB_CAP) {
                    ab_key[s * KL_AB_CAP + slot] = kn;
                    ab_info[s * KL_AB_CAP + slot] = KLInfo{u, rp, len, pp};
                }
            } else {
                if (uint32_t(~uint32_t(K & 0xffffffffull)) == uint32_t(pp) && kn < K) {
                    (s ? dtag1 : dtag0)[c] = tag;
                    s_stop[3] = tag;
                } else if (kn > K) {
                    atomicMax(&(s ? ckn1 : ckn0)[c], kn);
                    if (gi >= KL_ITEM_CAP) {
                        (s ? dtag1 : dtag0)[c] = tag;
                        s_stop[3] = tag;
                    }
                }
            }
            cs = int((pl & 0x80000000u) | uint32_t(c));
            inf = KLInfo{u, rp, len, pp};
        }
        if (gi < KL_ITEM_CAP) {
            it_key[gi] = kn;
            it_cs[gi] = cs;
            it_info[gi] = inf;
        }
    };

    bool fail = false;
    if (wv < NG) {
        bool spec = false;
        u64 sk0 = 0ull, sk1 = 0ull;
        int s_gi = -1;
        int4 s_a = make_int4(0, 0, 0, 0);
        float s_in = 0.0f, s_ex = 0.0f;
        bool s_act = false;
        int pA = -1, pB = -1;
        for (;; ++it) {
            if constexpr (PROF) t_a = now();
            if (!wait_word(1, int(it) + 1)) {
                fail = true;
                break;
            }
            if constexpr (PROF) {
                t_b = now();
                pc[3] += t_b - t_a;
            }
            const u64 k0 = nx_key[0], k1 = nx_key[1];
            const v4i dA = *reinterpret_cast<const v4i*>(nx_info), dB = *reinterpret_cast<const v4i*>(nx_info + 1);
            const u64 K0 = readlane_u64(k0, 0), K1 = readlane_u64(k1, 0);
            if (K0 == 0ull || K1 == 0ull) break;
            const int posA = int(~uint32_t(K0 & 0xffffffffull)), posB = int(~uint32_t(K1 & 0xffffffffull));
            const int cA = posA / KL_CHUNK, cB = posB / KL_CHUNK;
            const int A = __builtin_amdgcn_readfirstlane(dA.x), pa = __builtin_amdgcn_readfirstlane(dA.y),
                      la = __builtin_amdgcn_readfirstlane(dA.z);
            const int B = __builtin_amdgcn_readfirstlane(dB.x), pb = __builtin_amdgcn_readfirstlane(dB.y),
                      lb = __builtin_amdgcn_readfirstlane(dB.z);
            const int tot = la + lb, tag = int(it), abp = (tag & 1) * 2;
            const int qA = pA, qB = pB;
            auto side_cur = [&](int x) -> bool {
                const bool b = x == qA ? true : x == qB ? false : ((s_side[x >> 5] >> (x & 31)) & 1u) != 0;
                return b ^ (x == A) ^ (x == B);
            };
            auto lock_cur = [&](int x) -> bool {
                return ((s_lock[x >> 5] >> (x & 31)) & 1u) || x == qA || x == qB || x == A || x == B;
            };
            if constexpr (PROF) {
                pc[2] += 1;
                pc[1] += spec && sk0 == K0 && sk1 == K1;
            }
            if (spec && sk0 == K0 && sk1 == K1) {
                g1_commit(s_gi, s_a, s_in, s_ex, s_act, cA, cB, tag, abp);
            } else {
                for (int i0 = wv * RPW; i0 < tot; i0 += NG * RPW) {
                    int gi;
                    int4 a;
                    float in_, ex_;
                    bool act;
                    g1_rows(i0, pa, la, pb, lb, side_cur, lock_cur, gi, a, in_, ex_, act);
                    g1_commit(gi, a, in_, ex_, act, cA, cB, tag, abp);
                }
            }
            if constexpr (PROF) {
                if (tid == 0 && s_in == -12345.0f) s_stop[2] = 0;
                t_a = now();
                pc[6] += t_a - t_b;
            }
            __syncthreads();
            if constexpr (PROF) t_a = now();
            if (s_stop[it & 1]) {
                ++it;
                break;
            }
            spec = false;
            u64 kA = 0ull, kB = 0ull;
            int nA = 0, npa = 0, nla = 0, nB = 0, npb = 0, nlb = 0;
            bool okp = false;
            if (wv == 0) {
                const bool any_tag = s_stop[3] == tag;
                const int s = half, cS = s ? cB : cA, nck = s ? d.nck1 : d.nck0;
                const u64* ckn = s ? ckn1 : ckn0;
                u64 k = 0ull;
                for (int c0 = hl; c0 < nck; c0 += 4 * 32) {
                    u64 kv[4];
#pragma unroll
                    for (int u = 0; u < 4; ++u) kv[u] = ckn[min(c0 + 32 * u, nck - 1)];
#pragma unroll
                    for (int u = 0; u < 4; ++u) {
                        const u64 v = kv[u] & (min(c0 + 32 * u, nck - 1) == cS ? 0ull : ~0ull);
                        k = v > k ? v : k;
                    }
                }
                u64 rk[E_PARTS];
                v4i rf[E_PARTS];
#pragma unroll
                for (int q = 0; q < E_PARTS; ++q) {
                    rk[q] = er_key[s * E_PARTS + q];
                    rf[q] = *reinterpret_cast<const v4i*>(er_info + s * E_PARTS + q);
                }
                const int cnt = ab_cnt[abp + s];
                const int hs = hl < KL_AB_CAP ? hl : KL_AB_CAP - 1;
// ... 29 lines not shown
                const u64 mA = __ballot(own && ics >= 0 && ik == kA), mB = __ballot(own && ics < 0 && ik == kB);
                const u64 mS = s ? mB : mA;
                v4i desc = Rf;
                if (mA) {
                    const int l = __ffsll((long long)mA) - 1;
                    const v4i t = v4i{__builtin_amdgcn_readlane(iinf.x, l), __builtin_amdgcn_readlane(iinf.y, l),
                                      __builtin_amdgcn_readlane(iinf.z, l), 0};
                    if (!s) desc = t;
                }
                if (mB) {
                    const int l = __ffsll((long long)mB) - 1;
                    const v4i t = v4i{__builtin_amdgcn_readlane(iinf.x, l), __builtin_amdgcn_readlane(iinf.y, l),
                                      __builtin_amdgcn_readlane(iinf.z, l), 0};
                    if (s) desc = t;
                }
                if (!mS && k != R && k != 0ull)
                    desc = *reinterpret_cast<const v4i*>((s ? ci1 : ci0) + int(~uint32_t(k & 0xffffffffull)) / KL_CHUNK);
                arrive();
                nA = __builtin_amdgcn_readlane(desc.x, 0);
                npa = __builtin_amdgcn_readlane(desc.y, 0);
                nla = __builtin_amdgcn_readlane(desc.z, 0);
                nB = __builtin_amdgcn_readlane(desc.x, 32);
                npb = __builtin_amdgcn_readlane(desc.y, 32);
                nlb = __builtin_amdgcn_readlane(desc.z, 32);
                okp = !bad && kA != 0ull && kB != 0ull && nla >= 0 && nlb >= 0 && nla + nlb <= NG * RPW && nA != nB;
                if (lane == 0) {
                    sp[0] = okp ? kA : 0ull;
                    sp[1] = kB;
                    reinterpret_cast<v4i*>(sp + 2)[0] = v4i{nA, npa, nla, 0};
                    reinterpret_cast<v4i*>(sp + 2)[1] = v4i{nB, npb, nlb, 0};
                    __builtin_amdgcn_fence(__ATOMIC_RELEASE, "workgroup");
                    __hip_atomic_store(&sync[3], int(it) + 1, __ATOMIC_RELAXED, __HIP_MEMORY_SCOPE_WORKGROUP);
                }
            } else {
                arrive();
                if (!wait_word(3, int(it) + 1)) {
                    fail = true;
                    break;
                }
                kA = sp[0];
                kB = sp[1];
                const v4i a0 = reinterpret_cast<const v4i*>(sp + 2)[0], b0 = reinterpret_cast<const v4i*>(sp + 2)[1];
                kA = readlane_u64(kA, 0);
                kB = readlane_u64(kB, 0);
                okp = kA != 0ull;
                nA = __builtin_amdgcn_readfirstlane(a0.x);
                npa = __builtin_amdgcn_readfirstlane(a0.y);
                nla = __builtin_amdgcn_readfirstlane(a0.z);
                nB = __builtin_amdgcn_readfirstlane(b0.x);
                npb = __builtin_amdgcn_readfirstlane(b0.y);
                nlb = __builtin_amdgcn_readfirstlane(b0.z);
            }
            if constexpr (PROF) {
                t_b = now();
                pc[4] += t_b - t_a;
            }
            {
                if (okp) {
                    auto side_nx = [&](int x) -> bool {
                        const bool b = x == A ? true : x == B ? false : ((s_side[x >> 5] >> (x & 31)) & 1u) != 0;
                        return b ^ (x == nA) ^ (x == nB);
                    };
                    auto lock_nx = [&](int x) -> bool {
                        return ((s_lock[x >> 5] >> (x & 31)) & 1u) || x == A || x == B || x == nA || x == nB;
                    };
                    s_gi = -1;
                    if (wv * RPW < nla + nlb)
                        g1_rows(wv * RPW, npa, nla, npb, nlb, side_nx, lock_nx, s_gi, s_a, s_in, s_ex, s_act);
                    spec = true;
                    if constexpr (PROF) {
                        pc[0] += 1;
                        if (s_gi >= 0 && s_in == -12345.0f) s_stop[2] = 0;
                        pc[5] += now() - t_b;
                    }
                    sk0 = kA;
                    sk1 = kB;
                }
            }
            pA = A;
            pB = B;
        }
    } else {
        for (;; ++it) {
            if constexpr (PROF) t_a = now();
            if (it > 0 && !wait_word(0, 8 * int(it))) {
                fail = true;
                break;
            }
            if constexpr (PROF) {
                t_b = now();
                pc[7] += t_b - t_a;
            }
            u64 k0, k1;
            v4i dA = v4i{0, 0, 0, 0}, dB = v4i{0, 0, 0, 0};
            if (wv == W_W) {
                u64 k = 0ull;
                const u64* ck = half ? ck1 : ck0;
                if (nsel <= 4 * 32) {
                    u64 kv[4];
#pragma unroll
                    for (int u = 0; u < 4; ++u) kv[u] = ck[min(hl + 32 * u, nsel - 1)];
#pragma unroll
                    for (int u = 0; u < 4; ++u) k = kv[u] > k ? kv[u] : k;
                } else {
                    for (int c0 = hl; c0 < nsel; c0 += 8 * 32) {
                        u64 kv[8];
#pragma unroll
                        for (int u = 0; u < 8; ++u) kv[u] = ck[min(c0 + 32 * u, nsel - 1)];
#pragma unroll
                        for (int u = 0; u < 8; ++u) k = kv[u] > k ? kv[u] : k;
                    }
                }
                k = half_max_u64(k);
                k0 = readlane_u64(k, 0);
                k1 = readlane_u64(k, 32);
                if (k0 != 0ull && k1 != 0ull) {
                    dA = *reinterpret_cast<const v4i*>(ci0 + int(~uint32_t(k0 & 0xffffffffull)) / KL_CHUNK);
                    dB = *reinterpret_cast<const v4i*>(ci1 + int(~uint32_t(k1 & 0xffffffffull)) / KL_CHUNK);
                }
                if (lane == 0) {
                    nx_key[0] = k0;
                    nx_key[1] = k1;
                    *reinterpret_cast<v4i*>(nx_info) = dA;
                    *reinterpret_cast<v4i*>(nx_info + 1) = dB;
                    __builtin_amdgcn_fence(__ATOMIC_RELEASE, "workgroup");
                    __hip_atomic_store(&sync[1], int(it) + 1, __ATOMIC_RELAXED, __HIP_MEMORY_SCOPE_WORKGROUP);
                }
            } else {
                if (!wait_word(1, int(it) + 1)) {
                    fail = true;
                    break;
                }
                k0 = readlane_u64(nx_key[0], 0);
                k1 = readlane_u64(nx_key[1], 0);
                const v4i a0 = *reinterpret_cast<const v4i*>(nx_info), b0 = *reinterpret_cast<const v4i*>(nx_info + 1);
                dA = v4i{__builtin_amdgcn_readfirstlane(a0.x), __builtin_amdgcn_readfirstlane(a0.y),
                         __builtin_amdgcn_readfirstlane(a0.z), 0};
                dB = v4i{__builtin_amdgcn_readfirstlane(b0.x), __builtin_amdgcn_readfirstlane(b0.y),
                         __builtin_amdgcn_readfirstlane(b0.z), 0};
            }
            const int posA = int(~uint32_t(k0 & 0xffffffffull)), posB = int(~uint32_t(k1 & 0xffffffffull));
            const int cA = posA / KL_CHUNK, cB = posB / KL_CHUNK;
            if constexpr (PROF) {
                t_a = now();
                pc[8] += t_a - t_b;
            }
            if (k0 == 0ull || k1 == 0ull) break;
            const int A = dA.x, pa = dA.y, la = dA.z, B = dB.x, pb = dB.y, lb = dB.z;
            auto locked_now = [&](int x) -> bool { return ((s_lock[x >> 5] >> (x & 31)) & 1u) || x == A || x == B; };
            const int tot = la + lb;
            const int tag = int(it);
            const int abp = (tag & 1) * 2;
            if (wv == W_W) {
                float gA = 0.f, gB = 0.f;
                if (lane == 0) {
                    gA = d.gp0[posA];
                    gB = d.gp1[posB];
                }
                float wab = 0.0f;
                bool found = false;
                for (int i = lane; i < la; i += 64)
                    if (d.col[pa + i] == B) {
                        wab = d.w[pa + i];
                        found = true;
                    }
                const u64 bal = __ballot(found);
                if (bal) wab = __shfl(wab, __ffsll((long long)bal) - 1, 64);
                if (lane == 0) {
                    d.gp0[posA] = __builtin_nanf("");
                    d.gp1[posB] = __builtin_nanf("");
                    const float gain = gA - gB - 2.0f * wab;
                    cut -= gain;
                    if (cut < best) {
                        best = cut;
                        best_it = it + 1;
                    }
                    if (it < cap) log[it] = ek_swap{uint32_t(it + 1), uint32_t(A), uint32_t(B), gA, gB, gain, cut, 0u};
                    int stop = 0;
                    if (gain <= 0.0f) {
                        if (++term > unsigned(limit)) stop = 1;
                    } else {
                        term = 0;
                    }
                    if (it + 1 >= d.n0 || it + 1 >= d.n1) stop = 1;
                    s_stop[it & 1] = stop;
                }
            } else {
                const int s = wv <= W_EB ? 1 : 0, part = (s ? W_EB : W_EA) - wv;
                const int p0 = (s ? cB : cA) * KL_CHUNK + part * NQ_E * 64;
                KLInfo info;
                bool mine;
                const u64 kk = s ? chunk_rescan2<NQ_E>(d.gp1, d.pinfo1, 1, p0, posB, lane, &info, &mine)
                                 : chunk_rescan2<NQ_E>(d.gp0, d.pinfo0, 0, p0, posA, lane, &info, &mine);
                if (mine) {
                    er_key[s * E_PARTS + part] = kk;
                    er_info[s * E_PARTS + part] = info;
                }
            }
            if constexpr (PROF) {
                t_b = now();
                pc[9] += t_b - t_a;
            }
            __syncthreads();
            if constexpr (PROF) t_a = now();
            if (s_stop[it & 1]) {
                if (wv == W_FLIP && lane == 0) {
                    atomicOr(&s_side[A >> 5], 1u << (A & 31));
                    atomicAnd(&s_side[B >> 5], ~(1u << (B & 31)));
                }
                ++it;
                break;
            }
            const bool any_tag = s_stop[3] == tag;
            if (wv == W_EA) {
                const int s = half, cS = s ? cB : cA;
                u64 rk[E_PARTS];
                v4i rf[E_PARTS];
#pragma unroll
                for (int q = 0; q < E_PARTS; ++q) {
                    rk[q] = er_key[s * E_PARTS + q];
                    rf[q] = *reinterpret_cast<const v4i*>(er_info + s * E_PARTS + q);
                }
                const int cnt = ab_cnt[abp + s];
                const int hs = hl < KL_AB_CAP ? hl : KL_AB_CAP - 1;
                const u64 bk_raw = ab_key[s * KL_AB_CAP + hs];
                const v4i bf = *reinterpret_cast<const v4i*>(ab_info + s * KL_AB_CAP + hs);
                const bool have = hl < cnt && hl < KL_AB_CAP;
                const u64 bk = have ? bk_raw : 0ull;
                if (hl == 0) ab_cnt[2 - abp + s] = 0;
                u64 R = rk[0];
                v4i Rf = rf[0];
#pragma unroll
                for (int q = 1; q < E_PARTS; ++q) {
                    const bool b = rk[q] > R;
                    R = b ? rk[q] : R;
                    Rf.x = b ? rf[q].x : Rf.x;
                    Rf.y = b ? rf[q].y : Rf.y;
                    Rf.z = b ? rf[q].z : Rf.z;
                    Rf.w = b ? rf[q].w : Rf.w;
                }
                const int Rpos = int(~uint32_t(R & 0xffffffffull));
                const bool stale = have && R != 0ull && bf.w == Rpos && bk < R;
                const u64 hmask = s ? 0xffffffff00000000ull : 0x00000000ffffffffull;
                const bool st = (__ballot(stale) & hmask) != 0ull || cnt > KL_AB_CAP;
                u64 m = 0ull;
                if (__ballot(cnt > 0)) m = half_max_u64(bk);
                if (!st) {
                    if (m > R) {
                        if (have && bk == m) {
                            (s ? ck1 : ck0)[cS] = m;
                            (s ? ckn1 : ckn0)[cS] = m;
                            *reinterpret_cast<v4i*>((s ? ci1 : ci0) + cS) = bf;
                        }
                    } else if (hl == 0) {
                        (s ? ck1 : ck0)[cS] = R;
                        (s ? ckn1 : ckn0)[cS] = R;
                        *reinterpret_cast<v4i*>((s ? ci1 : ci0) + cS) = Rf;
                    }
                }
                const bool stA = __builtin_amdgcn_readlane(int(st), 0) != 0, stB = __builtin_amdgcn_readlane(int(st), 32) != 0;
                for (int q = 0; q < 2; ++q) {
                    if (!(q ? stB : stA)) continue;
                    KLInfo info;
                    bool mine;
                    const u64 kk = q ? chunk_rescan(d.gp1, d.pinfo1, 1, cB, -1, lane, &info, &mine)
                                     : chunk_rescan(d.gp0, d.pinfo0, 0, cA, -1, lane, &info, &mine);
                    if (mine) {
                        (q ? ck1 : ck0)[q ? cB : cA] = kk;
                        (q ? ckn1 : ckn0)[q ? cB : cA] = kk;
                        (q ? ci1 : ci0)[q ? cB : cA] = info;
                    }
                }
            }
            if (wv == W_FLIP && lane == 0) {
                atomicOr(&s_side[A >> 5], 1u << (A & 31));
                atomicAnd(&s_side[B >> 5], ~(1u << (B & 31)));
                atomicOr(&s_lock[A >> 5], 1u << (A & 31));
                atomicOr(&s_lock[B >> 5], 1u << (B & 31));
            }
            if (wv == W_EB || wv == W_EB - 1) {
                for (int i = (W_EB - wv) * 64 + lane; i < tot && i < KL_ITEM_CAP; i += 128) {
                    const int cs = it_cs[i];
                    const u64 kn = it_key[i];
                    const int4 inf = *reinterpret_cast<const int4*>(it_info + i);
                    if (cs == -1) continue;
                    const int s = int(uint32_t(cs) >> 31), c = cs & 0x7fffffff;
                    const u64 kmerged = (s ? ckn1 : ckn0)[c];
                    const int dt = (s ? dtag1 : dtag0)[c];
                    if ((s ? c == cB : c == cA) || dt == tag) continue;
                    (s ? ck1 : ck0)[c] = kmerged;
                    if (kmerged == kn) *reinterpret_cast<int4*>((s ? ci1 : ci0) + c) = inf;
                }
            }
            for (int i = wv - NG; any_tag && i < tot; i += NW - NG) {
                int cs;
                if (i < KL_ITEM_CAP) cs = it_cs[i];
                else {
                    const int u = i < la ? d.col[pa + i] : d.col[pb + i - la];
                    cs = locked_now(u) ? -1 : int((uint32_t(d.nd[u].c) & 0x80000000u) |
                                                  ((uint32_t(d.nd[u].c) & 0x7fffffffu) / KL_CHUNK));
                }
                if (cs == -1) continue;
                const int s = int(uint32_t(cs) >> 31), c = cs & 0x7fffffff;
                if ((s ? dtag1 : dtag0)[c] != tag) continue;
                int claimed = 0;
                if (lane == 0) claimed = atomicMax(&(s ? ctag1 : ctag0)[c], tag) < tag;
                if (!__shfl(claimed, 0, 64)) continue;
                KLInfo info;
                bool mine;
                const u64 kk = s ? chunk_rescan(d.gp1, d.pinfo1, 1, c, -1, lane, &info, &mine)
                                 : chunk_rescan(d.gp0, d.pinfo0, 0, c, -1, lane, &info, &mine);
                if (mine) {
                    (s ? ck1 : ck0)[c] = kk;
                    (s ? ckn1 : ckn0)[c] = kk;
                    (s ? ci1 : ci0)[c] = info;
                }
            }
            arrive();
            if constexpr (PROF) pc[10] += now() - t_a;
        }
    }
    if (fail) give_up();
    __syncthreads();
    for (int u = tid; u < d.n; u += KL_LOOP_THREADS) d.side[u] = uint8_t((s_side[u >> 5] >> (u & 31)) & 1u);
    if (wv == W_W && lane == 0) {
        out->iterations = it;
        out->best_iter = best_it;
        out->initial_cut = *d.cut0;
        out->best_cut = best;
        out->final_cut = cut;
        out->status = sync[2] ? 3u : 2u;
    }
    if constexpr (PROF) {
        if (wv == 0 && lane == 0)
            for (int i = 0; i < 7; ++i) out->prof[i] = pc[i];
        if (wv == W_W && lane == 0) {
            for (int i = 7; i < 11; ++i) out->prof[i] = pc[i];
            out->prof[12] = now() - t_start;
            out->prof[13] = 0x9199ull;
        }
        if (wv == W_EA && lane == 0) out->prof[11] = pc[10];
    } else if (tid == 0) {
        for (int i = 0; i < 16; ++i) out->prof[i] = 0ull;
    }
}


template <bool SMEM, bool PROF>
__global__ __launch_bounds__(KL_LOOP_THREADS) void k_kl_loop(KLDev d, int limit, ek_swap* __restrict__ log,
                                                             long long cap, KLOut* __restrict__ out) {
    constexpr int NW = KL_LOOP_THREADS / 64;
    extern __shared__ __attribute__((aligned(16))) unsigned char smem[];
    __shared__ u64 red0[NW], red1[NW];
    __shared__ float s_w;
    __shared__ int s_stop;
    const int tid = threadIdx.x, lane = tid & 63, wv = tid >> 6;
    const int words = (d.n + 31) / 32;
    u64* ck0 = d.ckey0;
    u64* ck1 = d.ckey1;
    uint32_t* s_side = nullptr;
    uint32_t* s_lock = nullptr;
    if constexpr (SMEM) {
        ck0 = reinterpret_cast<u64*>(smem);
        ck1 = ck0 + d.nck0;
        s_side = reinterpret_cast<uint32_t*>(ck1 + d.nck1);
        s_lock = s_side + words;
        for (int i = tid; i < d.nck0; i += KL_LOOP_THREADS) ck0[i] = d.ckey0[i];
        for (int i = tid; i < d.nck1; i += KL_LOOP_THREADS) ck1[i] = d.ckey1[i];
        for (int i = tid; i < words; i += KL_LOOP_THREADS) {
            s_side[i] = side_word(d.side_init, d.n, i);
            s_lock[i] = 0u;
        }
    }
    if (tid == 0) s_w = 0.0f;
    __syncthreads();
    float cut = *d.cut0, best = cut;
    long long best_it = 0, it = 0;
    unsigned term = 0;
    unsigned long long tph[4] = {0, 0, 0, 0}, tstamp = 0;
    auto stamp = [&](int ph) {
        if constexpr (PROF) {
            if (tid == 0) {
                const unsigned long long t = __builtin_amdgcn_s_memrealtime();
                if (ph >= 0) tph[ph] += t - tstamp;
                tstamp = t;
            }
        }
    };
    for (;;) {
        stamp(-1);
        u64 k0 = 0ull, k1 = 0ull;
        for (int c = tid; c < d.nck0; c += KL_LOOP_THREADS) k0 = ck0[c] > k0 ? ck0[c] : k0;
        for (int c = tid; c < d.nck1; c += KL_LOOP_THREADS) k1 = ck1[c] > k1 ? ck1[c] : k1;
        k0 = wave_max_u64(k0);
        k1 = wave_max_u64(k1);
        if (lane == 0) {
            red0[wv] = k0;
            red1[wv] = k1;
        }
        __syncthreads();
        stamp(0);
        k0 = red0[0];
        k1 = red1[0];
#pragma unroll
        for (int i = 1; i < NW; ++i) {
            k0 = red0[i] > k0 ? red0[i] : k0;
            k1 = red1[i] > k1 ? red1[i] : k1;
        }
        if (k0 == 0ull || k1 == 0ull) break;
        const int posA = int(~uint32_t(k0 & 0xffffffffull)), posB = int(~uint32_t(k1 & 0xffffffffull));
        const int A = d.order0[posA], B = d.order1[posB];
        const int pa = d.rowptr[A], la = d.rowptr[A + 1] - pa;
        const int pb = d.rowptr[B], lb = d.rowptr[B + 1] - pb;
        float gA = 0.f, gB = 0.f;
        if (tid == 0) {
            gA = d.gp0[posA];
            gB = d.gp1[posB];
            d.gp0[posA] = __builtin_nanf("");
            d.gp1[posB] = __builtin_nanf("");
            if constexpr (SMEM) {
                s_side[A >> 5] |= 1u << (A & 31);
                s_side[B >> 5] &= ~(1u << (B & 31));
                s_lock[A >> 5] |= 1u << (A & 31);
                s_lock[B >> 5] |= 1u << (B & 31);
            } else {
                d.side[A] = 1;
                d.side[B] = 0;
                d.locked[A] = 1;
                d.locked[B] = 1;
            }
        }
        for (int i = tid; i < la; i += KL_LOOP_THREADS)
            if (d.col[pa + i] == B) s_w = d.w[pa + i];
        __syncthreads();
        stamp(1);
        if (tid == 0) {
            const float gain = gA - gB - 2.0f * s_w;
            cut -= gain;
            ++it;
            if (cut < best) {
                best = cut;
                best_it = it;
            }
            if (it <= cap) log[it - 1] = ek_swap{uint32_t(it), uint32_t(A), uint32_t(B), gA, gB, gain, cut, 0u};
            int stop = 0;
            if (gain <= 0.0f) {
                if (++term > unsigned(limit)) stop = 1;
            } else {
                term = 0;
            }
            if (it >= d.n0 || it >= d.n1) stop = 1;
            s_stop = stop;
        }
        for (int i = tid; i < la + lb; i += KL_LOOP_THREADS) {
            const int u = i < la ? d.col[pa + i] : d.col[pb + i - la];
            bool lk;
            if constexpr (SMEM) lk = (s_lock[u >> 5] >> (u & 31)) & 1u;
            else lk = d.locked[u] != 0;
            if (!lk) {
                const float g = row_gain<SMEM>(d.rowptr, d.col, d.w, s_side, d.side, u, nullptr);
                const uint32_t pl = d.plist[u];
                ((pl >> 31) ? d.gp1 : d.gp0)[pl & 0x7fffffffu] = g;
            }
        }
        __syncthreads();
        stamp(2);
        for (int i = wv; i < la + lb + 2; i += NW) {
            const int u = i < la ? d.col[pa + i] : i < la + lb ? d.col[pb + i - la] : (i == la + lb ? A : B);
            const uint32_t pl = d.plist[u];
            const int s = int(pl >> 31), c = int(pl & 0x7fffffffu) / KL_CHUNK;
            const u64 k = s ? chunk_key(d.gp1, 1, c, lane) : chunk_key(d.gp0, 0, c, lane);
            if (lane == 0) (s ? ck1 : ck0)[c] = k;
        }
        if (tid == 0) s_w = 0.0f;
        __syncthreads();
        stamp(3);
        if (s_stop) break;
    }
    if constexpr (SMEM) {
        __syncthreads();
        for (int u = tid; u < d.n; u += KL_LOOP_THREADS) d.side[u] = uint8_t((s_side[u >> 5] >> (u & 31)) & 1u);
    }
    if (tid == 0) {
        out->iterations = it;
        out->best_iter = best_it;
        out->initial_cut = *d.cut0;
        out->best_cut = best;
        out->final_cut = cut;
        out->status = SMEM ? 1u : 0u;
        for (int i = 0; i < 4; ++i) out->prof[i] = tph[i];
        for (int i = 4; i < 16; ++i) out->prof[i] = 0ull;
    }
}

__global__ __launch_bounds__(256) void k_replay(int n, const uint8_t* __restrict__ side_init,
                                                uint8_t* __restrict__ out) {
    for (long long i = blockIdx.x * 256ll + threadIdx.x; i < n; i += 256ll * gridDim.x) out[i] = side_init[i];
}

__global__ __launch_bounds__(256) void k_replay_swaps(const ek_swap* __restrict__ log, const long long* __restrict__ count,
                                                      long long cap, uint8_t* __restrict__ out) {
    const long long cnt = *count < cap ? *count : cap;
    for (long long i = blockIdx.x * 256ll + threadIdx.x; i < cnt; i += 256ll * gridDim.x) {
        out[log[i].node_left] = 1;
        out[log[i].node_right] = 0;
    }
}

__global__ __launch_bounds__(256) void k_net_cut(long long nets, const int64_t* __restrict__ net_ptr,
                                                 const int32_t* __restrict__ pins, const uint8_t* __restrict__ sa,
                                                 const uint8_t* __restrict__ sb, const uint8_t* __restrict__ sc,
                                                 unsigned* __restrict__ part) {
    __shared__ unsigned wcnt[3][4];
    const long long e = blockIdx.x * 256ll + threadIdx.x;
    bool ca = false, cb = false, cc = false;
    if (e < nets) {
        const int64_t p0 = net_ptr[e], p1 = net_ptr[e + 1];
        if (p1 - p0 >= 2) {
            const int v0 = pins[p0];
            const uint8_t a0 = sa[v0], b0 = sb[v0], c0 = sc[v0];
            for (int64_t p = p0 + 1; p < p1 && !(ca && cb && cc); p += 4) {
                int v[4];
#pragma unroll
                for (int u = 0; u < 4; ++u) v[u] = p + u < p1 ? pins[p + u] : v0;
#pragma unroll
                for (int u = 0; u < 4; ++u) {
                    ca |= sa[v[u]] != a0;
                    cb |= sb[v[u]] != b0;
                    cc |= sc[v[u]] != c0;
                }
            }
        }
    }
    const u64 ma = __ballot(ca), mb = __ballot(cb), mc = __ballot(cc);
    const int w = threadIdx.x >> 6;
    if ((threadIdx.x & 63) == 0) {
        wcnt[0][w] = unsigned(__popcll(ma));
        wcnt[1][w] = unsigned(__popcll(mb));
        wcnt[2][w] = unsigned(__popcll(mc));
    }
    __syncthreads();
    if (threadIdx.x < 3) {
        const unsigned* c = wcnt[threadIdx.x];
        part[threadIdx.x * gridDim.x + blockIdx.x] = c[0] + c[1] + c[2] + c[3];
    }
}

__global__ __launch_bounds__(256) void k_build_aux(long long nnz, const int32_t* __restrict__ col,
                                                   const KLInfo* __restrict__ nd, KLInfo* __restrict__ aux) {
    const long long p = blockIdx.x * 256ll + threadIdx.x;
    if (p >= nnz) return;
    const int v = col[p];
    const int4 x = *reinterpret_cast<const int4*>(nd + v);
    *reinterpret_cast<int4*>(aux + p) = make_int4(v, x.x, x.y, x.z);
}

__global__ __launch_bounds__(256) void k_build_seg(long long nnz, const int32_t* __restrict__ rowptr,
                                                   const int32_t* __restrict__ col, const float* __restrict__ w,
                                                   KLInfo* __restrict__ seg) {
    const long long t = blockIdx.x * 256ll + threadIdx.x;
    const long long p = t / KL_SEG_LANES;
    if (p >= nnz) return;
    const int j = int(t % KL_SEG_LANES), v = col[p];
    const int rp = rowptr[v], len = rowptr[v + 1] - rp;
    const int e0 = 2 * j, e1 = 2 * j + 1;
    int4 o = make_int4(0, 0, 0, 0);
    if (e0 < len) {
        o.x = col[rp + e0];
        o.y = __float_as_int(w[rp + e0]);
// ... 99 lines not shown
    run_threads(T, [&](int t) {
        for (int64_t p = nnz * t / T; p < nnz * (t + 1) / T; ++p) {
            uint32_t k;
            std::memcpy(&k, &w[p], 4);
            kw[size_t(p)] = (uint32_t(glob.slot[glob.find(k)]) << wcolbits) | uint32_t(col[p]);
        }
    });
    return true;
}

__global__ __launch_bounds__(256) void k_build_desc(int n, int n0, int n1, int pad0, int pad1,
                                                    const int32_t* __restrict__ order0,
                                                    const int32_t* __restrict__ order1,
                                                    const uint32_t* __restrict__ plist,
                                                    const int32_t* __restrict__ rowptr, KLInfo* __restrict__ p0,
                                                    KLInfo* __restrict__ p1, KLInfo* __restrict__ nd) {
    const int i = blockIdx.x * 256 + threadIdx.x;
    if (i < pad0) {
        KLInfo v{0, 0, 0, 0};
        if (i < n0) {
            const int u = order0[i];
            v = KLInfo{u, rowptr[u], rowptr[u + 1] - rowptr[u], 0};
        }
        p0[i] = v;
    }
    if (i < pad1) {
        KLInfo v{0, 0, 0, 0};
        if (i < n1) {
            const int u = order1[i];
            v = KLInfo{u, rowptr[u], rowptr[u + 1] - rowptr[u], 0};
        }
        p1[i] = v;
    }
    if (i < n) nd[i] = KLInfo{rowptr[i], rowptr[i + 1] - rowptr[i], int32_t(plist[i]), 0};
}

void kl_build_desc(hipStream_t s, int n, int n0, int n1, int pad0, int pad1, const int32_t* order0,
                   const int32_t* order1, const uint32_t* plist, const int32_t* rowptr, KLInfo* p0, KLInfo* p1,
                   KLInfo* nd) {
    const int m = std::max(n, std::max(pad0, pad1));
    if (m <= 0) return;
    hipLaunchKernelGGL(k_build_desc, dim3((m + 255) / 256), dim3(256), 0, s, n, n0, n1, pad0, pad1, order0, order1,
                       plist, rowptr, p0, p1, nd);
}

namespace {
KLDev with_chunk(KLDev d, int ch) {
    d.nck0 = (d.n0 + ch - 1) / ch;
    d.nck1 = (d.n1 + ch - 1) / ch;
    return d;
}
struct LoopForm {
    size_t lds, lds_gb;
    int ch;
};
LoopForm loop_form(const KLDev& d_in) {
    const KLDev d = with_chunk(d_in, KL_CHUNK);
    const bool force_gb = std::getenv("EK_KL_GBITS") && std::getenv("EK_KL_GBITS")[0] == '1';
    const size_t lds = force_gb ? 0 : kl_loop_lds_bytes(d);
    const size_t lds_gb = d.locked && !std::getenv("EK_KL_GLOBAL_STATE") ? kl_loop_lds_bytes(d, false) : 0;
    if (!lds && lds_gb) return {0, kl_loop_lds_bytes(with_chunk(d, KL_CHUNK_GB), false), KL_CHUNK_GB};
    return {lds, lds_gb, KL_CHUNK};
}
}

void kl_prepare(hipStream_t s, const KLDev& d_in) {
    const KLDev d = with_chunk(d_in, loop_form(d_in).ch);
    const int nb = (d.n + 255) / 256;
    hipLaunchKernelGGL(k_gain_scan, dim3(nb), dim3(256), 0, s, d);
    hipLaunchKernelGGL(k_cut_final, dim3(1), dim3(256), 0, s, d, nb);
    const int waves = d.nck0 + d.nck1;
    if (loop_form(d_in).ch == KL_CHUNK_GB)
        hipLaunchKernelGGL(k_chunk_init<KL_CHUNK_GB>, dim3((waves + 3) / 4), dim3(256), 0, s, d);
    else
        hipLaunchKernelGGL(k_chunk_init<KL_CHUNK>, dim3((waves + 3) / 4), dim3(256), 0, s, d);
}

__global__ __launch_bounds__(256) void k_touch(const int4* __restrict__ p, long long n16, int* __restrict__ sink) {
    int acc = 0;
    for (long long i = blockIdx.x * 256ll + threadIdx.x; i < n16; i += 256ll * gridDim.x) acc ^= p[i].x;
    if (acc == 0x7fffabcd) sink[0] = acc;
}

void kl_loop(hipStream_t s, const KLDev& d_in, int limit, ek_swap* log, long long cap, KLOut* out) {
    const LoopForm form = loop_form(d_in);
    const KLDev d = with_chunk(d_in, form.ch);
    const size_t lds = form.lds, lds_gb = form.lds_gb;
    if (!std::getenv("EK_KL_NOTOUCH")) {
        int* sink = reinterpret_cast<int*>(&out->prof[13]);
        if (d.segc)
            hipLaunchKernelGGL(k_touch, dim3(4096), dim3(256), 0, s, reinterpret_cast<const int4*>(d.segc),
                               (long long)d.nnz * KL_SEGC_PIECES, sink);
        else if (d.seg)
            hipLaunchKernelGGL(k_touch, dim3(4096), dim3(256), 0, s, reinterpret_cast<const int4*>(d.seg),
                               (long long)d.nnz * KL_SEG_LANES, sink);
        hipLaunchKernelGGL(k_touch, dim3(1024), dim3(256), 0, s, reinterpret_cast<const int4*>(d.aux), (long long)d.nnz,
                           sink);
    }
    const bool prof = std::getenv("EK_KL_PROF") != nullptr;
    const char* pe = std::getenv("EK_KL_PIPE");
    const bool pipe = pe && pe[0] ? pe[0] != '0' : false;
    if (lds && pipe && !std::getenv("EK_KL_GLOBAL_STATE")) {
        if (prof && d.segc)
            hipLaunchKernelGGL((k_kl_swap_pipe<true, true>), dim3(1), dim3(KL_LOOP_THREADS), lds, s, d, limit, log, cap, out);
        else if (prof)
            hipLaunchKernelGGL((k_kl_swap_pipe<true, false>), dim3(1), dim3(KL_LOOP_THREADS), lds, s, d, limit, log, cap, out);
        else if (d.segc)
            hipLaunchKernelGGL((k_kl_swap_pipe<false, true>), dim3(1), dim3(KL_LOOP_THREADS), lds, s, d, limit, log, cap, out);
        else
            hipLaunchKernelGGL((k_kl_swap_pipe<false, false>), dim3(1), dim3(KL_LOOP_THREADS), lds, s, d, limit, log, cap, out);
        return;
    }
    const bool global_state = std::getenv("EK_KL_GLOBAL_STATE") != nullptr;
    if (!lds && lds_gb) {
        if (prof && d.segc)
            hipLaunchKernelGGL((k_kl_swap_loop<true, true, true>), dim3(1), dim3(KL_LOOP_THREADS), lds_gb, s, d, limit,
                               log, cap, out);
        else if (d.segc)
            hipLaunchKernelGGL((k_kl_swap_loop<false, true, true>), dim3(1), dim3(KL_LOOP_THREADS), lds_gb, s, d, limit,
                               log, cap, out);
        else
            hipLaunchKernelGGL((k_kl_swap_loop<false, false, true>), dim3(1), dim3(KL_LOOP_THREADS), lds_gb, s, d, limit,
                               log, cap, out);
        return;
    }
    const char* fx = std::getenv("EK_KL_FIXLDS");
    const size_t lds_fix = lds && !global_state && !prof && !(fx && fx[0] == '0') ? kl_loop_lds_bytes(d, true, true) : 0;
    if (lds_fix) {
        if (d.segc)
            hipLaunchKernelGGL((k_kl_swap_loop<false, true, false, true>), dim3(1), dim3(KL_LOOP_THREADS), lds_fix, s, d,
                               limit, log, cap, out);
        else
            hipLaunchKernelGGL((k_kl_swap_loop<false, false, false, true>), dim3(1), dim3(KL_LOOP_THREADS), lds_fix, s, d,
                               limit, log, cap, out);
        return;
    }
    if (lds && !global_state && prof && d.segc)
        hipLaunchKernelGGL((k_kl_swap_loop<true, true>), dim3(1), dim3(KL_LOOP_THREADS), lds, s, d, limit, log, cap, out);
    else if (lds && !global_state && prof)
        hipLaunchKernelGGL((k_kl_swap_loop<true, false>), dim3(1), dim3(KL_LOOP_THREADS), lds, s, d, limit, log, cap, out);
    else if (lds && !global_state && d.segc)
        hipLaunchKernelGGL((k_kl_swap_loop<false, true>), dim3(1), dim3(KL_LOOP_THREADS), lds, s, d, limit, log, cap,
                           out);
    else if (lds && !global_state)
        hipLaunchKernelGGL((k_kl_swap_loop<false, false>), dim3(1), dim3(KL_LOOP_THREADS), lds, s, d, limit, log, cap,
                           out);
    else if (prof)
        hipLaunchKernelGGL((k_kl_loop<false, true>), dim3(1), dim3(KL_LOOP_THREADS), 0, s, d, limit, log, cap, out);
    else
        hipLaunchKernelGGL((k_kl_loop<false, false>), dim3(1), dim3(KL_LOOP_THREADS), 0, s, d, limit, log, cap, out);
}

void kl_replay(hipStream_t s, int n, const uint8_t* side_init, const ek_swap* log, const long long* count,
               long long cap, uint8_t* sides_out) {
    const int nb = std::min(2048, (n + 255) / 256);
    hipLaunchKernelGGL(k_replay, dim3(nb), dim3(256), 0, s, n, side_init, sides_out);
    hipLaunchKernelGGL(k_replay_swaps, dim3(64), dim3(256), 0, s, log, count, cap, sides_out);
}

int net_cut_blocks(int64_t nets) { return int((nets + 255) / 256); }

void net_cut(hipStream_t s, int64_t nets, const int64_t* net_ptr, const int32_t* pins, const uint8_t* side_a,
             const uint8_t* side_b, const uint8_t* side_c, unsigned* part) {
    if (nets <= 0) return;
    hipLaunchKernelGGL(k_net_cut, dim3(unsigned(net_cut_blocks(nets))), dim3(256), 0, s, (long long)nets, net_ptr,
                       pins, side_a, side_b, side_c, part);
}



__global__ __launch_bounds__(256) void k_fiedler_scale(const double* __restrict__ x, double sgn, int n,
                                                       double* __restrict__ out) {
    const int i = blockIdx.x * 256 + threadIdx.x;
    if (i < n) out[i] = x[i] * sgn;
}

constexpr int SEL_THREADS = 256, SEL_PER = 8, SEL_PASSES = 8;
constexpr int SEL_SUB = 16;
struct SelState {
    unsigned long long prefix[2], mask[2];
    unsigned k[2];
    unsigned pad[2];
    unsigned hist[SEL_PASSES][2][256];
    unsigned ctr[(SEL_SUB + 1) * 64];
};

__device__ __forceinline__ unsigned long long ord_key(double v) {
    const unsigned long long u = static_cast<unsigned long long>(__double_as_longlong(v));
    return (u >> 63) ? ~u : (u | 0x8000000000000000ull);
}

__global__ __launch_bounds__(SEL_THREADS) void k_select_init(SelState* st, unsigned k0, unsigned k1) {
    if (threadIdx.x < 2) {
        st->prefix[threadIdx.x] = 0ull;
        st->mask[threadIdx.x] = 0ull;
        st->k[threadIdx.x] = threadIdx.x ? k1 : k0;
    }
}

__global__ __launch_bounds__(SEL_THREADS) void k_select_pass(const double* __restrict__ v, int n, SelState* st,
                                                             int pass, unsigned long long* keys_out) {
    __shared__ unsigned h[2][256];
    __shared__ int s_last;
    const int t = threadIdx.x;
    h[0][t] = 0u;
    h[1][t] = 0u;
    const unsigned long long p0 = st->prefix[0], m0 = st->mask[0], p1 = st->prefix[1], m1 = st->mask[1];
    const int shift = 56 - 8 * pass;
    __syncthreads();
    const int base = int(blockIdx.x) * SEL_THREADS * SEL_PER;
#pragma unroll
    for (int u = 0; u < SEL_PER; ++u) {
        const int i = base + u * SEL_THREADS + t;
        if (i < n) {
            const unsigned long long key = ord_key(v[i]);
            const unsigned d = unsigned(key >> shift) & 255u;
            if ((key & m0) == p0) atomicAdd(&h[0][d], 1u);
            if ((key & m1) == p1) atomicAdd(&h[1][d], 1u);
        }
    }
    __syncthreads();
    for (int r = 0; r < 2; ++r)
        if (h[r][t]) __hip_atomic_fetch_add(&st->hist[pass][r][t], h[r][t], __ATOMIC_RELAXED, __HIP_MEMORY_SCOPE_AGENT);
    asm volatile("s_waitcnt vmcnt(0)" ::: "memory");
    __syncthreads();
    if (t == 0) {
        const unsigned nb = gridDim.x, g = blockIdx.x % SEL_SUB;
        const unsigned gsize = (nb - g + SEL_SUB - 1) / SEL_SUB, ngroups = nb < SEL_SUB ? nb : SEL_SUB;
        s_last = 0;
        if (__hip_atomic_fetch_add(st->ctr + g * 64, 1u, __ATOMIC_RELAXED, __HIP_MEMORY_SCOPE_AGENT) == gsize - 1u)
            s_last = __hip_atomic_fetch_add(st->ctr + SEL_SUB * 64, 1u, __ATOMIC_RELAXED, __HIP_MEMORY_SCOPE_AGENT) ==
                     ngroups - 1u;
    }
// ... 144 lines not shown
```

Baseline: 0.05964.

## Place KL device arrays in one arena and pass 32-bit offsets to loop kernels

All KL device arrays are carved from a single arena allocation, and the loop kernels now take a compact argument struct holding a base pointer plus 32-bit offsets instead of many 64-bit pointers. The aim is to cut scalar-register and kernarg pressure in the single-block KL swap loop and to let one touch kernel prefetch the contiguous segment and aux data. Optional asm pins can keep offsets or thread roles in specific registers. In exchange the code adds address arithmetic on every access and fixed arena sizing, so buffers can no longer grow later without failing.

```diff
diff --git a/eig-kl-algorithm_amd/csrc/ctx.cpp b/eig-kl-algorithm_amd/csrc/ctx.cpp
--- a/eig-kl-algorithm_amd/csrc/ctx.cpp
+++ b/eig-kl-algorithm_amd/csrc/ctx.cpp
@@ -40,13 +40,22 @@
     DBuf(const DBuf&) = delete;
     DBuf& operator=(const DBuf&) = delete;
     ~DBuf() { reset(); }
+    bool owned = true;
     void reset() {
-        if (p) (void)hipFree(p);
+        if (p && owned) (void)hipFree(p);
         p = nullptr;
         bytes = 0;
+        owned = true;
+    }
+    void view(void* q, size_t b) {
+        reset();
+        p = q;
+        bytes = b;
+        owned = false;
     }
     void ensure(size_t b) {
         if (b <= bytes && p) return;
+        if (p && !owned) ek::fail(EK_ESTATE, "device range of %zu bytes asked for %zu", bytes, b);
         reset();
         HIPCHK(hipMalloc(&p, b ? b : 16));
         bytes = b;
@@ -151,6 +160,8 @@
         kl_ckey0, kl_ckey1, kl_aux, kl_seg, kl_cutpart, kl_cut0, kl_log, kl_out, kl_sides_tmp, kl_count, kl_netptr, kl_pins;
     bool kl_graph_ready = false, kl_part_ready = false, kl_seg_ok = false, kl_segc_ok = false;
     DBuf kl_segc, kl_wdict;
+    DBuf kl_arena;
+    ek::dev::KLArenaLayout kl_layout;
     DBuf lb_netptr, lb_pins, lb_icnt, lb_rcnt, lb_cur, lb_ip, lb_rp, lb_tiles, lb_inc, lb_scol, lb_sval, lb_tval,
         lb_ulen, lb_len, lb_diag, lb_long, lb_cnt, lb_off, lb_table, lb_flags, lb_codes;
     int kl_nwd = 0, kl_wcolbits = 0;
@@ -2569,10 +2580,47 @@
     c->kl_part_ready = false;
     c->kl_n = n;
     c->kl_rowptr_h.assign(rowptr, rowptr + n + 1);
+    std::vector<uint32_t> kw;
+    std::vector<float> wdict;
+    int wcolbits = 0;
+    c->kl_segc_ok = !std::getenv("EK_KL_NOSEGC") &&
+                    size_t(nnz) * ek::dev::KL_SEGC_PIECES * sizeof(ek::dev::KLInfo) <= (size_t(32) << 30) &&
+                    ek::dev::kl_weight_codes(n, nnz, col, w, kw, wdict, wcolbits);
+    pt.mark("weight codes");
+    c->kl_seg_ok = !c->kl_segc_ok && size_t(nnz) * ek::dev::KL_SEG_LANES * sizeof(ek::dev::KLInfo) <= (size_t(32) << 30);
+    {
+        using namespace ek::dev;
+        const uint64_t nz1 = uint64_t(std::max<int64_t>(nnz, 1)), n1 = uint64_t(n);
+        const uint64_t pad = uint64_t(chunk_pad(n)), nck = uint64_t((n + KL_CHUNK - 1) / KL_CHUNK + 1);
+        uint64_t b[KA_COUNT] = {};
+        b[KA_SEGC] = c->kl_segc_ok ? nz1 * KL_SEGC_PIECES * sizeof(KLInfo) : 0;
+        b[KA_SEG] = c->kl_seg_ok ? nz1 * KL_SEG_LANES * sizeof(KLInfo) : 0;
+        b[KA_AUX] = nz1 * sizeof(KLInfo);
+        b[KA_PINFO0] = b[KA_PINFO1] = pad * sizeof(KLInfo);
+        b[KA_ND] = n1 * sizeof(KLInfo);
+        b[KA_CINFO0] = b[KA_CINFO1] = nck * sizeof(KLInfo);
+        b[KA_CKEY0] = b[KA_CKEY1] = nck * 8;
+        b[KA_GP0] = b[KA_GP1] = pad * 4;
+        b[KA_COL] = b[KA_W] = (uint64_t(nnz) + 16) * 4;
+        b[KA_WDICT] = c->kl_segc_ok ? uint64_t(wdict.size()) * 4 : 0;
+        b[KA_LOCKED] = std::max(n1, uint64_t((n + 31) / 32) * 8 + 64);
+        b[KA_SIDE_INIT] = b[KA_SIDE] = n1;
+        b[KA_CUT0] = 16;
+        b[KA_ROWPTR] = (n1 + 1) * 4;
+        b[KA_ORDER0] = b[KA_ORDER1] = b[KA_PLIST] = n1 * 4;
+        const KLArenaLayout L = kl_arena_layout(b);
+        if (!L.ok) ek::fail(EK_EINVAL, "ek_kl_graph_setup: the KL arrays exceed the arena's 32-bit offsets");
+        c->kl_arena.ensure(size_t(L.total));
+        c->kl_layout = L;
+        auto* base = c->kl_arena.as<unsigned char>();
+        DBuf* const slot[KA_COUNT] = {&c->kl_segc,  &c->kl_seg,    &c->kl_aux,   &c->kl_pinfo0, &c->kl_pinfo1,    &c->kl_nd,
+                                      &c->kl_cinfo0, &c->kl_cinfo1, &c->kl_ckey0, &c->kl_ckey1,  &c->kl_gp0,       &c->kl_gp1,
+                                      &c->kl_col,   &c->kl_w,      &c->kl_wdict, &c->kl_locked, &c->kl_side_init, &c->kl_side,
+                                      &c->kl_cut0,  &c->kl_rowptr, &c->kl_order0, &c->kl_order1, &c->kl_plist};
+        for (int k = 0; k < KA_COUNT; ++k) slot[k]->view(base + L.begin(k), size_t(b[k]));
+    }
     Uploader up(c, s, (size_t(n) + 1) * 4 + size_t(nnz) * 8 + size_t(nnz) * 4);
     up.put(c->kl_rowptr, rowptr, size_t(n) + 1);
-    c->kl_col.ensure((size_t(nnz) + 16) * 4);
-    c->kl_w.ensure((size_t(nnz) + 16) * 4);
     HIPCHK(hipMemsetAsync(c->kl_col.as<int32_t>() + nnz, 0, 16 * 4, s));
     HIPCHK(hipMemsetAsync(c->kl_w.as<float>() + nnz, 0, 16 * 4, s));
     if (nnz) {
@@ -2587,14 +2635,6 @@
         up.off += size_t(nnz) * 8;
     }
     pt.mark("CSR staged");
-    std::vector<uint32_t> kw;
-    std::vector<float> wdict;
-    int wcolbits = 0;
-    c->kl_segc_ok = !std::getenv("EK_KL_NOSEGC") &&
-                    size_t(nnz) * ek::dev::KL_SEGC_PIECES * sizeof(ek::dev::KLInfo) <= (size_t(32) << 30) &&
-                    ek::dev::kl_weight_codes(n, nnz, col, w, kw, wdict, wcolbits);
-    pt.mark("weight codes");
-    c->kl_seg_ok = !c->kl_segc_ok && size_t(nnz) * ek::dev::KL_SEG_LANES * sizeof(ek::dev::KLInfo) <= (size_t(32) << 30);
     if (c->kl_segc_ok) {
         DBuf dkw;
         up.put(dkw, kw.data(), kw.size());
@@ -2674,8 +2714,8 @@
     }
     c->kl_gp0.ensure(size_t(chunk_pad(n0)) * 4);
     c->kl_gp1.ensure(size_t(chunk_pad(n1)) * 4);
-    HIPCHK(hipMemsetAsync(c->kl_gp0.p, 0xFF, c->kl_gp0.bytes, s));
-    HIPCHK(hipMemsetAsync(c->kl_gp1.p, 0xFF, c->kl_gp1.bytes, s));
+    HIPCHK(hipMemsetAsync(c->kl_gp0.p, 0xFF, size_t(chunk_pad(n0)) * 4, s));
+    HIPCHK(hipMemsetAsync(c->kl_gp1.p, 0xFF, size_t(chunk_pad(n1)) * 4, s));
     c->kl_ckey0.ensure(size_t((n0 + ek::dev::KL_CHUNK - 1) / ek::dev::KL_CHUNK + 1) * 8);
     c->kl_ckey1.ensure(size_t((n1 + ek::dev::KL_CHUNK - 1) / ek::dev::KL_CHUNK + 1) * 8);
     c->kl_log.ensure(size_t(std::max<int64_t>(1, std::min(n0, n1))) * sizeof(ek_swap));
@@ -2928,6 +2968,8 @@
     d.ckey1 = c->kl_ckey1.as<unsigned long long>();
     d.cut_part = c->kl_cutpart.as<double>();
     d.cut0 = c->kl_cut0.as<float>();
+    d.arena = c->kl_arena.as<unsigned char>();
+    d.arena_bytes = c->kl_arena.bytes;
     return d;
 }
 
diff --git a/eig-kl-algorithm_amd/csrc/ek_internal.hpp b/eig-kl-algorithm_amd/csrc/ek_internal.hpp
--- a/eig-kl-algorithm_amd/csrc/ek_internal.hpp
+++ b/eig-kl-algorithm_amd/csrc/ek_internal.hpp
@@ -10,6 +10,7 @@
 #include <vector>
 
 #include "../../include/eigkl.h"
+#include "ek_kl_arena.hpp"
 
 namespace ek {
 void set_error(const char* fmt, ...) __attribute__((format(printf, 1, 2)));
@@ -396,7 +397,18 @@
     const KLInfo* segc = nullptr;
     const float* wdict = nullptr;
     int nwd = 0, wcolbits = 0;
-};
+    unsigned char* arena = nullptr;
+    size_t arena_bytes = 0;
+};
+struct KLArgs {
+    unsigned char* base = nullptr;
+    uint32_t off[KA_COUNT] = {};
+    int n = 0, n0 = 0, n1 = 0, nck0 = 0, nck1 = 0;
+    int nwd = 0, wcolbits = 0;
+    int has_seg = 0;
+    long long nnz = 0;
+};
+KLArgs kl_args(const KLDev& d);
 constexpr int KL_SEGC_PIECES = 8;
 constexpr int KL_WDICT_CAP = 4096;
 constexpr int KL_SEG_LANES = 16;
diff --git a/eig-kl-algorithm_amd/csrc/ek_kl_arena.hpp b/eig-kl-algorithm_amd/csrc/ek_kl_arena.hpp
--- /dev/null
+++ b/eig-kl-algorithm_amd/csrc/ek_kl_arena.hpp
@@ -0,0 +1,59 @@
+#pragma once
+#include <cstdint>
+
+namespace ek {
+namespace dev {
+
+enum KLArenaSlot : int {
+    KA_SEGC = 0,
+    KA_SEG,
+    KA_AUX,
+    KA_PINFO0,
+    KA_PINFO1,
+    KA_ND,
+    KA_CINFO0,
+    KA_CINFO1,
+    KA_CKEY0,
+    KA_CKEY1,
+    KA_GP0,
+    KA_GP1,
+    KA_COL,
+    KA_W,
+    KA_WDICT,
+    KA_LOCKED,
+    KA_SIDE_INIT,
+    KA_SIDE,
+    KA_CUT0,
+    KA_ROWPTR,
+    KA_ORDER0,
+    KA_ORDER1,
+    KA_PLIST,
+    KA_COUNT
+};
+
+constexpr uint64_t KL_ARENA_ALIGN = 256;
+constexpr int KL_ARENA_UNIT_SHIFT = 4;
+
+struct KLArenaLayout {
+    uint32_t off[KA_COUNT] = {};
+    uint64_t total = 0;
+    bool ok = false;
+    uint64_t begin(int k) const { return uint64_t(off[k]) << KL_ARENA_UNIT_SHIFT; }
+};
+
+inline KLArenaLayout kl_arena_layout(const uint64_t (&bytes)[KA_COUNT]) {
+    KLArenaLayout L;
+    uint64_t cur = 0;
+    for (int k = 0; k < KA_COUNT; ++k) {
+        if ((cur >> KL_ARENA_UNIT_SHIFT) > uint64_t(UINT32_MAX)) return L;
+        L.off[k] = uint32_t(cur >> KL_ARENA_UNIT_SHIFT);
+        if (bytes[k] > UINT64_MAX / 2 - cur) return L;
+        L.total = cur + bytes[k];
+        cur = (L.total + KL_ARENA_ALIGN - 1) / KL_ARENA_ALIGN * KL_ARENA_ALIGN;
+    }
+    L.ok = true;
+    return L;
+}
+
+}
+}
diff --git a/eig-kl-algorithm_amd/csrc/kernels_kl.hip b/eig-kl-algorithm_amd/csrc/kernels_kl.hip
--- a/eig-kl-algorithm_amd/csrc/kernels_kl.hip
+++ b/eig-kl-algorithm_amd/csrc/kernels_kl.hip
@@ -354,9 +354,53 @@
     return m;
 }
 
+#ifndef EK_KL_ROLE_PIN
+#define EK_KL_ROLE_PIN 0
+#endif
+#ifndef EK_KL_ARG_PIN
+#define EK_KL_ARG_PIN 0
+#endif
+struct KLView : KLArgs {
+    uint32_t z = 0;
+    __device__ __forceinline__ explicit KLView(const KLArgs& a) : KLArgs(a) {}
+    __device__ __forceinline__ void pin() {
+#if EK_KL_ARG_PIN
+        asm volatile("" : "+s"(z));
+#endif
+    }
+    template <class T, int K>
+    __device__ __forceinline__ T* at() const {
+        return reinterpret_cast<T*>(base + (size_t(off[K] | z) << KL_ARENA_UNIT_SHIFT));
+    }
+    __device__ __forceinline__ float* gp0() const { return at<float, KA_GP0>(); }
+    __device__ __forceinline__ float* gp1() const { return at<float, KA_GP1>(); }
+    __device__ __forceinline__ const KLInfo* pinfo0() const { return at<const KLInfo, KA_PINFO0>(); }
+    __device__ __forceinline__ const KLInfo* pinfo1() const { return at<const KLInfo, KA_PINFO1>(); }
+    __device__ __forceinline__ const KLInfo* nd() const { return at<const KLInfo, KA_ND>(); }
+    __device__ __forceinline__ const KLInfo* cinfo0() const { return at<const KLInfo, KA_CINFO0>(); }
+    __device__ __forceinline__ const KLInfo* cinfo1() const { return at<const KLInfo, KA_CINFO1>(); }
+    __device__ __forceinline__ const KLInfo* aux() const { return at<const KLInfo, KA_AUX>(); }
+    __device__ __forceinline__ const KLInfo* seg() const { return at<const KLInfo, KA_SEG>(); }
+    __device__ __forceinline__ const KLInfo* segc() const { return at<const KLInfo, KA_SEGC>(); }
+    __device__ __forceinline__ const int32_t* col() const { return at<const int32_t, KA_COL>(); }
+    __device__ __forceinline__ const float* w() const { return at<const float, KA_W>(); }
+    __device__ __forceinline__ u64* ckey0() const { return at<u64, KA_CKEY0>(); }
+    __device__ __forceinline__ u64* ckey1() const { return at<u64, KA_CKEY1>(); }
+    __device__ __forceinline__ const float* wdict() const { return at<const float, KA_WDICT>(); }
+    __device__ __forceinline__ uint8_t* locked() const { return at<uint8_t, KA_LOCKED>(); }
+    __device__ __forceinline__ const uint8_t* side_init() const { return at<const uint8_t, KA_SIDE_INIT>(); }
+    __device__ __forceinline__ uint8_t* side() const { return at<uint8_t, KA_SIDE>(); }
+    __device__ __forceinline__ const float* cut0() const { return at<const float, KA_CUT0>(); }
+    __device__ __forceinline__ const int32_t* rowptr() const { return at<const int32_t, KA_ROWPTR>(); }
+    __device__ __forceinline__ const int32_t* order0() const { return at<const int32_t, KA_ORDER0>(); }
+    __device__ __forceinline__ const int32_t* order1() const { return at<const int32_t, KA_ORDER1>(); }
+    __device__ __forceinline__ const uint32_t* plist() const { return at<const uint32_t, KA_PLIST>(); }
+};
+
 template <bool PROF, bool SEGC, bool GB = false, bool FIX = false>
-__global__ __launch_bounds__(KL_LOOP_THREADS) void k_kl_swap_loop(KLDev d, int limit, ek_swap* __restrict__ log,
+__global__ __launch_bounds__(KL_LOOP_THREADS) void k_kl_swap_loop(KLArgs args, int limit, ek_swap* __restrict__ log,
                                                                   long long cap, KLOut* __restrict__ out) {
+    KLView d(args);
     constexpr int NW = KL_LOOP_THREADS / 64;
     constexpr int CH = GB ? KL_CHUNK_GB : KL_CHUNK;
     constexpr int E_PARTS = KL_E_PARTS, NQ_E = CH / 64 / E_PARTS;
@@ -393,7 +437,7 @@
     int* s_stop = it_cs + KL_ITEM_CAP;
     int* ab_cnt = s_stop + 4;
     int* nx_ok = ab_cnt + 4;
-    uint32_t* s_side = GB ? reinterpret_cast<uint32_t*>(d.locked)
+    uint32_t* s_side = GB ? reinterpret_cast<uint32_t*>(d.locked())
                      : FIX ? reinterpret_cast<uint32_t*>(nx_ok + 4 + KL_WDICT_CAP)
                            : reinterpret_cast<uint32_t*>(nx_ok + 4);
     uint32_t* s_lock = s_side + words;
@@ -403,27 +447,27 @@
         else return *p;
     };
     if constexpr (SEGC)
-        for (int i = tid; i < d.nwd; i += KL_LOOP_THREADS) s_wd[i] = d.wdict[i];
+        for (int i = tid; i < d.nwd; i += KL_LOOP_THREADS) s_wd[i] = d.wdict()[i];
     for (int i = tid; i < nsel; i += KL_LOOP_THREADS) {
-        ck0[i] = i < d.nck0 ? d.ckey0[i] : 0ull;
-        ck1[i] = i < d.nck1 ? d.ckey1[i] : 0ull;
+        ck0[i] = i < d.nck0 ? d.ckey0()[i] : 0ull;
+        ck1[i] = i < d.nck1 ? d.ckey1()[i] : 0ull;
     }
     for (int i = tid; i < d.nck0; i += KL_LOOP_THREADS) {
-        ckn0[i] = d.ckey0[i];
-        ci0[i] = d.cinfo0[i];
+        ckn0[i] = d.ckey0()[i];
+        ci0[i] = d.cinfo0()[i];
         dtag0[i] = ctag0[i] = -1;
     }
     for (int i = tid; i < d.nck1; i += KL_LOOP_THREADS) {
-        ckn1[i] = d.ckey1[i];
-        ci1[i] = d.cinfo1[i];
+        ckn1[i] = d.ckey1()[i];
+        ci1[i] = d.cinfo1()[i];
         dtag1[i] = ctag1[i] = -1;
     }
     for (int i = tid; i < words; i += KL_LOOP_THREADS) {
         if constexpr (GB) {
-            __hip_atomic_store(s_side + i, side_word(d.side_init, d.n, i), __ATOMIC_RELAXED, __HIP_MEMORY_SCOPE_AGENT);
+            __hip_atomic_store(s_side + i, side_word(d.side_init(), d.n, i), __ATOMIC_RELAXED, __HIP_MEMORY_SCOPE_AGENT);
             __hip_atomic_store(s_lock + i, 0u, __ATOMIC_RELAXED, __HIP_MEMORY_SCOPE_AGENT);
         } else {
-            s_side[i] = side_word(d.side_init, d.n, i);
+            s_side[i] = side_word(d.side_init(), d.n, i);
             s_lock[i] = 0u;
         }
     }
@@ -432,7 +476,7 @@
     if (tid < 4) ab_cnt[tid] = 0;
     if (tid < 4) nx_ok[tid] = 0;
     __syncthreads();
-    float cut = *d.cut0, best = cut;
+    float cut = *d.cut0(), best = cut;
     long long best_it = 0, it = 0;
     unsigned term = 0;
     unsigned long long tph[12] = {}, tstamp = 0;
@@ -455,6 +499,12 @@
     };
     unsigned long long w_top = 0, w_arr1 = 0, w_arr2 = 0, w_g2a = 0, w_sel = 0, w_g2r = 0;
     for (;; ++it) {
+        d.pin();
+#if EK_KL_ROLE_PIN
+        int tid_p = tid;
+        asm volatile("" : "+v"(tid_p));
+        const int lane = tid_p & 63, wv = tid_p >> 6, half = lane >> 5, hl = lane & 31;
+#endif
         stamp(-1);
         if constexpr (PROF) w_top = __builtin_amdgcn_s_memtime();
         if constexpr (EK_KL_PREFETCH) {
@@ -466,14 +516,14 @@
                     const int last = r0 + l0 - 1;
                     const int rs = min(r0 + hl, last);
                     if constexpr (SEGC) {
-                        pf_seg = *reinterpret_cast<const int4*>(d.segc + size_t(rs) * KL_SEGC_PIECES);
-                    } else if (d.seg) {
-                        pf_seg = *reinterpret_cast<const int4*>(d.seg + size_t(rs) * KL_SEG_LANES);
-                        pf_seg2 = *reinterpret_cast<const int4*>(d.seg + size_t(rs) * KL_SEG_LANES + KL_SEG_LANES / 2);
+                        pf_seg = *reinterpret_cast<const int4*>(d.segc() + size_t(rs) * KL_SEGC_PIECES);
+                    } else if (d.has_seg) {
+                        pf_seg = *reinterpret_cast<const int4*>(d.seg() + size_t(rs) * KL_SEG_LANES);
+                        pf_seg2 = *reinterpret_cast<const int4*>(d.seg() + size_t(rs) * KL_SEG_LANES + KL_SEG_LANES / 2);
                     }
-                    pf_aux = *reinterpret_cast<const int4*>(d.aux + min(r0 + 8 * hl, last));
-                    pf_col = d.col[min(r0 + 32 * hl, last)];
-                    pf_w = d.w[min(r0 + 32 * hl, last)];
+                    pf_aux = *reinterpret_cast<const int4*>(d.aux() + min(r0 + 8 * hl, last));
+                    pf_col = d.col()[min(r0 + 32 * hl, last)];
+                    pf_w = d.w()[min(r0 + 32 * hl, last)];
                 }
             }
         }
@@ -550,21 +600,21 @@
         if (wv == W_W) {
             float gA = 0.f, gB = 0.f;
             if (lane == 0) {
-                gA = d.gp0[posA];
-                gB = d.gp1[posB];
+                gA = d.gp0()[posA];
+                gB = d.gp1()[posB];
             }
             float wab = 0.0f;
             bool found = false;
             for (int i = lane; i < la; i += 64)
-                if (d.col[pa + i] == B) {
-                    wab = d.w[pa + i];
+                if (d.col()[pa + i] == B) {
+                    wab = d.w()[pa + i];
                     found = true;
                 }
             const u64 bal = __ballot(found);
             if (bal) wab = __shfl(wab, __ffsll((long long)bal) - 1, 64);
             if (lane == 0) {
-                d.gp0[posA] = __builtin_nanf("");
-                d.gp1[posB] = __builtin_nanf("");
+                d.gp0()[posA] = __builtin_nanf("");
+                d.gp1()[posB] = __builtin_nanf("");
                 const float gain = gA - gB - 2.0f * wab;
                 cut -= gain;
                 if (cut < best) {
@@ -591,11 +641,11 @@
             KLInfo info;
             bool mine;
 #if EK_E_TWO_TRIPS
-            const u64 kk = s ? chunk_rescan2<NQ_E>(d.gp1, d.pinfo1, 1, p0, posB, lane, &info, &mine)
-                             : chunk_rescan2<NQ_E>(d.gp0, d.pinfo0, 0, p0, posA, lane, &info, &mine);
+            const u64 kk = s ? chunk_rescan2<NQ_E>(d.gp1(), d.pinfo1(), 1, p0, posB, lane, &info, &mine)
+                             : chunk_rescan2<NQ_E>(d.gp0(), d.pinfo0(), 0, p0, posA, lane, &info, &mine);
 #else
-            const u64 kk = s ? chunk_rescan1<NQ_E>(d.gp1, d.pinfo1, 1, p0, posB, lane, &info, &mine)
-                             : chunk_rescan1<NQ_E>(d.gp0, d.pinfo0, 0, p0, posA, lane, &info, &mine);
+            const u64 kk = s ? chunk_rescan1<NQ_E>(d.gp1(), d.pinfo1(), 1, p0, posB, lane, &info, &mine)
+                             : chunk_rescan1<NQ_E>(d.gp0(), d.pinfo0(), 0, p0, posA, lane, &info, &mine);
 #endif
             if (mine) {
                 er_key[s * E_PARTS + part] = kk;
@@ -612,14 +662,14 @@
                 if constexpr (SEGC) {
 #pragma unroll
                     for (int r = 0; r < PPL; ++r)
-                        piece[r] = *reinterpret_cast<const int4*>(d.segc + size_t(pg) * KL_SEGC_PIECES + j8 + LPR * r);
+                        piece[r] = *reinterpret_cast<const int4*>(d.segc() + size_t(pg) * KL_SEGC_PIECES + j8 + LPR * r);
                 } else {
 #pragma unroll
                     for (int r = 0; r < PPL; ++r)
-                        piece[r] = d.seg ? *reinterpret_cast<const int4*>(d.seg + size_t(pg) * KL_SEG_LANES + j8 + LPR * r)
+                        piece[r] = d.has_seg ? *reinterpret_cast<const int4*>(d.seg() + size_t(pg) * KL_SEG_LANES + j8 + LPR * r)
                                          : make_int4(0, 0, 0, 0);
                 }
-                const int4 a = j8 == 0 ? *reinterpret_cast<const int4*>(d.aux + pg) : make_int4(0, 0, 0, 0);
+                const int4 a = j8 == 0 ? *reinterpret_cast<const int4*>(d.aux() + pg) : make_int4(0, 0, 0, 0);
                 if constexpr (PROF) {
                     if (tid == 0 && (piece[0].x == -12345 || a.x == -12345)) s_stop[2] = 0;
                 }
@@ -649,7 +699,7 @@
                         ie_seg.x = quad_bcast(x.x, st % 4);
                         ie_seg.y = quad_bcast(x.y, st % 4);
                     }
-                } else if (d.seg) {
+                } else if (d.has_seg) {
 #pragma unroll
                     for (int r = 0; r < PPL; ++r) {
                         const int4 pc = piece[r];
@@ -665,7 +715,7 @@
                 if (j8 != 0 || gi >= tot) continue;
                 const int i = gi;
                 int4 sg[KL_SEG_LANES];
-                if (!SEGC && d.seg) {
+                if (!SEGC && d.has_seg) {
 #pragma unroll
                     for (int j = 0; j < KL_SEG_LANES; ++j) sg[j] = stage[srow * KL_STAGE_ROW + j];
                 }
@@ -683,7 +733,7 @@
                         internal = ie_seg.x;
                         external = ie_seg.y;
                         q = 2 * KL_SEG_LANES;
-                    } else if (d.seg) {
+                    } else if (d.has_seg) {
                         v2f ie = {0.0f, 0.0f};
 #pragma unroll
                         for (int b = 0; b < KL_SEG_LANES / 4; ++b) {
@@ -706,8 +756,8 @@
                         float ww[16];
 #pragma unroll
                         for (int k2 = 0; k2 < 16; ++k2) {
-                            cc[k2] = d.col[rp + q + k2];
-                            ww[k2] = q + k2 < len ? d.w[rp + q + k2] : 0.0f;
+                            cc[k2] = d.col()[rp + q + k2];
+                            ww[k2] = q + k2 < len ? d.w()[rp + q + k2] : 0.0f;
                         }
 #pragma unroll
                         for (int k2 = 0; k2 < 16; ++k2) {
@@ -728,7 +778,7 @@
                 if (act) {
                     const float g = external - internal;
                     const int s = ls;
-                    (s ? d.gp1 : d.gp0)[pp] = g;
+                    (s ? d.gp1() : d.gp0())[pp] = g;
                     kn = key_max(s ? -g : g, pp);
                     if (ab) {
                         const int slot = atomicAdd(&ab_cnt[abp + s], 1);
@@ -821,8 +871,8 @@
                 if (!(q ? stB : stA)) continue;
                 KLInfo info;
                 bool mine;
-                const u64 kk = q ? chunk_rescan<CH>(d.gp1, d.pinfo1, 1, cB, -1, lane, &info, &mine)
-                                 : chunk_rescan<CH>(d.gp0, d.pinfo0, 0, cA, -1, lane, &info, &mine);
+                const u64 kk = q ? chunk_rescan<CH>(d.gp1(), d.pinfo1(), 1, cB, -1, lane, &info, &mine)
+                                 : chunk_rescan<CH>(d.gp0(), d.pinfo0(), 0, cA, -1, lane, &info, &mine);
                 if (mine) {
                     (q ? ck1 : ck0)[q ? cB : cA] = kk;
                     (q ? ckn1 : ckn0)[q ? cB : cA] = kk;
@@ -945,7 +995,7 @@
                 k = half_max_u64(k);
                 pf_inf = make_int4(0, 0, 0, 0);
                 if (k != 0ull && hl == 0)
-                    pf_inf = *reinterpret_cast<const int4*>((half ? d.pinfo1 : d.pinfo0) + int(~uint32_t(k & 0xffffffffull)));
+                    pf_inf = *reinterpret_cast<const int4*>((half ? d.pinfo1() : d.pinfo0()) + int(~uint32_t(k & 0xffffffffull)));
             }
         }
         if (wv == W_EB || wv == W_EB - 1) {
@@ -966,9 +1016,9 @@
             int cs;
             if (i < KL_ITEM_CAP) cs = it_cs[i];
             else {
-                const int u = i < la ? d.col[pa + i] : d.col[pb + i - la];
-                cs = locked_now(u) ? -1 : int((uint32_t(d.nd[u].c) & 0x80000000u) |
-                                                                     ((uint32_t(d.nd[u].c) & 0x7fffffffu) / CH));
+                const int u = i < la ? d.col()[pa + i] : d.col()[pb + i - la];
+                cs = locked_now(u) ? -1 : int((uint32_t(d.nd()[u].c) & 0x80000000u) |
+                                                                     ((uint32_t(d.nd()[u].c) & 0x7fffffffu) / CH));
             }
             if (cs == -1) continue;
             const int s = int(uint32_t(cs) >> 31), c = cs & 0x7fffffff;
@@ -981,8 +1031,8 @@
             }
             KLInfo info;
             bool mine;
-            const u64 kk = s ? chunk_rescan<CH>(d.gp1, d.pinfo1, 1, c, -1, lane, &info, &mine)
-                             : chunk_rescan<CH>(d.gp0, d.pinfo0, 0, c, -1, lane, &info, &mine);
+            const u64 kk = s ? chunk_rescan<CH>(d.gp1(), d.pinfo1(), 1, c, -1, lane, &info, &mine)
+                             : chunk_rescan<CH>(d.gp0(), d.pinfo0(), 0, c, -1, lane, &info, &mine);
             if (mine) {
                 (s ? ck1 : ck0)[c] = kk;
                 (s ? ckn1 : ckn0)[c] = kk;
@@ -999,7 +1049,7 @@
         }
     }
     __syncthreads();
-    for (int u = tid; u < d.n; u += KL_LOOP_THREADS) d.side[u] = uint8_t((bits_at(s_side + (u >> 5)) >> (u & 31)) & 1u);
+    for (int u = tid; u < d.n; u += KL_LOOP_THREADS) d.side()[u] = uint8_t((bits_at(s_side + (u >> 5)) >> (u & 31)) & 1u);
     if (EK_KL_PREFETCH && wv == W_PF && lane == 0 && pf_sink == 0x5a5a5a5au) out->prof[12] = 1ull;
     if (lane == 0 && (NW <= 8 || wv < 8)) {
         out->warr[wv] = w_arr1;
@@ -1015,7 +1065,7 @@
     if (wv == W_W && lane == 0) {
         out->iterations = it;
         out->best_iter = best_it;
-        out->initial_cut = *d.cut0;
+        out->initial_cut = *d.cut0();
         out->best_cut = best;
         out->final_cut = cut;
         out->status = 2u;
@@ -1033,8 +1083,9 @@
 
 
 template <bool PROF, bool SEGC>
-__global__ __launch_bounds__(KL_LOOP_THREADS) void k_kl_swap_pipe(KLDev d, int limit, ek_swap* __restrict__ log,
+__global__ __launch_bounds__(KL_LOOP_THREADS) void k_kl_swap_pipe(KLArgs args, int limit, ek_swap* __restrict__ log,
                                                                   long long cap, KLOut* __restrict__ out) {
+    KLView d(args);
     constexpr int NW = KL_LOOP_THREADS / 64;
     constexpr int E_PARTS = KL_E_PARTS, NQ_E = KL_CHUNK / 64 / E_PARTS;
     constexpr int W_W = NW - 1, W_EA = NW - 2, W_EB = W_EA - E_PARTS, NG = W_EB - E_PARTS + 1;
@@ -1076,30 +1127,30 @@
     float* s_wd = reinterpret_cast<float*>(s_lock + words);
     u64* sp = reinterpret_cast<u64*>((reinterpret_cast<uintptr_t>(s_wd + (SEGC ? d.nwd : 0)) + 15) & ~uintptr_t(15));
     if constexpr (SEGC)
-        for (int i = tid; i < d.nwd; i += KL_LOOP_THREADS) s_wd[i] = d.wdict[i];
+        for (int i = tid; i < d.nwd; i += KL_LOOP_THREADS) s_wd[i] = d.wdict()[i];
     for (int i = tid; i < nsel; i += KL_LOOP_THREADS) {
-        ck0[i] = i < d.nck0 ? d.ckey0[i] : 0ull;
-        ck1[i] = i < d.nck1 ? d.ckey1[i] : 0ull;
+        ck0[i] = i < d.nck0 ? d.ckey0()[i] : 0ull;
+        ck1[i] = i < d.nck1 ? d.ckey1()[i] : 0ull;
     }
     for (int i = tid; i < d.nck0; i += KL_LOOP_THREADS) {
-        ckn0[i] = d.ckey0[i];
-        ci0[i] = d.cinfo0[i];
+        ckn0[i] = d.ckey0()[i];
+        ci0[i] = d.cinfo0()[i];
         dtag0[i] = ctag0[i] = -1;
     }
     for (int i = tid; i < d.nck1; i += KL_LOOP_THREADS) {
-        ckn1[i] = d.ckey1[i];
-        ci1[i] = d.cinfo1[i];
+        ckn1[i] = d.ckey1()[i];
+        ci1[i] = d.cinfo1()[i];
         dtag1[i] = ctag1[i] = -1;
     }
     for (int i = tid; i < words; i += KL_LOOP_THREADS) {
-        s_side[i] = side_word(d.side_init, d.n, i);
+        s_side[i] = side_word(d.side_init(), d.n, i);
         s_lock[i] = 0u;
     }
     if (tid < 4) s_stop[tid] = tid == 3 ? -1 : 0;
     if (tid < 4) ab_cnt[tid] = 0;
     if (tid < 4) sync[tid] = 0;
     __syncthreads();
-    float cut = *d.cut0, best = cut;
+    float cut = *d.cut0(), best = cut;
     long long best_it = 0, it = 0;
     unsigned term = 0;
     unsigned long long pc[12] = {};
@@ -1140,14 +1191,14 @@
         if constexpr (SEGC) {
 #pragma unroll
             for (int r = 0; r < PPL; ++r)
-                piece[r] = *reinterpret_cast<const int4*>(d.segc + size_t(pg) * KL_SEGC_PIECES + j8 + LPR * r);
+                piece[r] = *reinterpret_cast<const int4*>(d.segc() + size_t(pg) * KL_SEGC_PIECES + j8 + LPR * r);
         } else {
 #pragma unroll
             for (int r = 0; r < PPL; ++r)
-                piece[r] = d.seg ? *reinterpret_cast<const int4*>(d.seg + size_t(pg) * KL_SEG_LANES + j8 + LPR * r)
+                piece[r] = d.has_seg ? *reinterpret_cast<const int4*>(d.seg() + size_t(pg) * KL_SEG_LANES + j8 + LPR * r)
                                  : make_int4(0, 0, 0, 0);
         }
-        const int4 a = j8 == 0 ? *reinterpret_cast<const int4*>(d.aux + pg) : make_int4(0, 0, 0, 0);
+        const int4 a = j8 == 0 ? *reinterpret_cast<const int4*>(d.aux() + pg) : make_int4(0, 0, 0, 0);
         v2f ie_seg = {0.0f, 0.0f};
         int4* stage = sg_stage + wv * KL_STAGE_ROWS * KL_STAGE_ROW;
         if constexpr (SEGC) {
@@ -1174,7 +1225,7 @@
                 ie_seg.x = quad_bcast(x.x, st % 4);
                 ie_seg.y = quad_bcast(x.y, st % 4);
             }
-        } else if (d.seg) {
+        } else if (d.has_seg) {
 #pragma unroll
             for (int r = 0; r < PPL; ++r) {
                 const int4 pc = piece[r];
@@ -1195,7 +1246,7 @@
             internal = ie_seg.x;
             external = ie_seg.y;
             q = 2 * KL_SEG_LANES;
-        } else if (d.seg) {
+        } else if (d.has_seg) {
             int4 sg[KL_SEG_LANES];
 #pragma unroll
             for (int j = 0; j < KL_SEG_LANES; ++j) sg[j] = stage[srow * KL_STAGE_ROW + j];
@@ -1219,8 +1270,8 @@
             const int lim = int(d.nnz) - 1;
 #pragma unroll
             for (int k2 = 0; k2 < 16; ++k2) {
-                cc[k2] = d.col[min(rp + q + k2, lim + 16)];
-                ww[k2] = q + k2 < len ? d.w[min(rp + q + k2, lim)] : 0.0f;
+                cc[k2] = d.col()[min(rp + q + k2, lim + 16)];
+                ww[k2] = q + k2 < len ? d.w()[min(rp + q + k2, lim)] : 0.0f;
             }
 #pragma unroll
             for (int k2 = 0; k2 < 16; ++k2) {
@@ -1250,7 +1301,7 @@
         if (act) {
             const float g = external - internal;
             const int s = ls;
-            (s ? d.gp1 : d.gp0)[pp] = g;
+            (s ? d.gp1() : d.gp0())[pp] = g;
             kn = key_max(s ? -g : g, pp);
             if (ab) {
                 const int slot = atomicAdd(&ab_cnt[abp + s], 1);
@@ -1290,6 +1341,7 @@
         bool s_act = false;
         int pA = -1, pB = -1;
         for (;; ++it) {
+            d.pin();
             if constexpr (PROF) t_a = now();
             if (!wait_word(1, int(it) + 1)) {
                 fail = true;
@@ -1485,6 +1537,7 @@
         }
     } else {
         for (;; ++it) {
+            d.pin();
             if constexpr (PROF) t_a = now();
             if (it > 0 && !wait_word(0, 8 * int(it))) {
                 fail = true;
@@ -1557,21 +1610,21 @@
             if (wv == W_W) {
                 float gA = 0.f, gB = 0.f;
                 if (lane == 0) {
-                    gA = d.gp0[posA];
-                    gB = d.gp1[posB];
+                    gA = d.gp0()[posA];
+                    gB = d.gp1()[posB];
                 }
                 float wab = 0.0f;
                 bool found = false;
                 for (int i = lane; i < la; i += 64)
-                    if (d.col[pa + i] == B) {
-                        wab = d.w[pa + i];
+                    if (d.col()[pa + i] == B) {
+                        wab = d.w()[pa + i];
                         found = true;
                     }
                 const u64 bal = __ballot(found);
                 if (bal) wab = __shfl(wab, __ffsll((long long)bal) - 1, 64);
                 if (lane == 0) {
-                    d.gp0[posA] = __builtin_nanf("");
-                    d.gp1[posB] = __builtin_nanf("");
+                    d.gp0()[posA] = __builtin_nanf("");
+                    d.gp1()[posB] = __builtin_nanf("");
                     const float gain = gA - gB - 2.0f * wab;
                     cut -= gain;
                     if (cut < best) {
@@ -1593,8 +1646,8 @@
                 const int p0 = (s ? cB : cA) * KL_CHUNK + part * NQ_E * 64;
                 KLInfo info;
                 bool mine;
-                const u64 kk = s ? chunk_rescan2<NQ_E>(d.gp1, d.pinfo1, 1, p0, posB, lane, &info, &mine)
-                                 : chunk_rescan2<NQ_E>(d.gp0, d.pinfo0, 0, p0, posA, lane, &info, &mine);
+                const u64 kk = s ? chunk_rescan2<NQ_E>(d.gp1(), d.pinfo1(), 1, p0, posB, lane, &info, &mine)
+                                 : chunk_rescan2<NQ_E>(d.gp0(), d.pinfo0(), 0, p0, posA, lane, &info, &mine);
                 if (mine) {
                     er_key[s * E_PARTS + part] = kk;
                     er_info[s * E_PARTS + part] = info;
@@ -1666,8 +1719,8 @@
                     if (!(q ? stB : stA)) continue;
                     KLInfo info;
                     bool mine;
-                    const u64 kk = q ? chunk_rescan(d.gp1, d.pinfo1, 1, cB, -1, lane, &info, &mine)
-                                     : chunk_rescan(d.gp0, d.pinfo0, 0, cA, -1, lane, &info, &mine);
+                    const u64 kk = q ? chunk_rescan(d.gp1(), d.pinfo1(), 1, cB, -1, lane, &info, &mine)
+                                     : chunk_rescan(d.gp0(), d.pinfo0(), 0, cA, -1, lane, &info, &mine);
                     if (mine) {
                         (q ? ck1 : ck0)[q ? cB : cA] = kk;
                         (q ? ckn1 : ckn0)[q ? cB : cA] = kk;
@@ -1699,9 +1752,9 @@
                 int cs;
                 if (i < KL_ITEM_CAP) cs = it_cs[i];
                 else {
-                    const int u = i < la ? d.col[pa + i] : d.col[pb + i - la];
-                    cs = locked_now(u) ? -1 : int((uint32_t(d.nd[u].c) & 0x80000000u) |
-                                                  ((uint32_t(d.nd[u].c) & 0x7fffffffu) / KL_CHUNK));
+                    const int u = i < la ? d.col()[pa + i] : d.col()[pb + i - la];
+                    cs = locked_now(u) ? -1 : int((uint32_t(d.nd()[u].c) & 0x80000000u) |
+                                                  ((uint32_t(d.nd()[u].c) & 0x7fffffffu) / KL_CHUNK));
                 }
                 if (cs == -1) continue;
                 const int s = int(uint32_t(cs) >> 31), c = cs & 0x7fffffff;
@@ -1711,8 +1764,8 @@
                 if (!__shfl(claimed, 0, 64)) continue;
                 KLInfo info;
                 bool mine;
-                const u64 kk = s ? chunk_rescan(d.gp1, d.pinfo1, 1, c, -1, lane, &info, &mine)
-                                 : chunk_rescan(d.gp0, d.pinfo0, 0, c, -1, lane, &info, &mine);
+                const u64 kk = s ? chunk_rescan(d.gp1(), d.pinfo1(), 1, c, -1, lane, &info, &mine)
+                                 : chunk_rescan(d.gp0(), d.pinfo0(), 0, c, -1, lane, &info, &mine);
                 if (mine) {
                     (s ? ck1 : ck0)[c] = kk;
                     (s ? ckn1 : ckn0)[c] = kk;
@@ -1725,11 +1778,11 @@
     }
     if (fail) give_up();
     __syncthreads();
-    for (int u = tid; u < d.n; u += KL_LOOP_THREADS) d.side[u] = uint8_t((s_side[u >> 5] >> (u & 31)) & 1u);
+    for (int u = tid; u < d.n; u += KL_LOOP_THREADS) d.side()[u] = uint8_t((s_side[u >> 5] >> (u & 31)) & 1u);
     if (wv == W_W && lane == 0) {
         out->iterations = it;
         out->best_iter = best_it;
-        out->initial_cut = *d.cut0;
+        out->initial_cut = *d.cut0();
         out->best_cut = best;
         out->final_cut = cut;
         out->status = sync[2] ? 3u : 2u;
@@ -1750,8 +1803,9 @@
 
 
 template <bool SMEM, bool PROF>
-__global__ __launch_bounds__(KL_LOOP_THREADS) void k_kl_loop(KLDev d, int limit, ek_swap* __restrict__ log,
+__global__ __launch_bounds__(KL_LOOP_THREADS) void k_kl_loop(KLArgs args, int limit, ek_swap* __restrict__ log,
                                                              long long cap, KLOut* __restrict__ out) {
+    KLView d(args);
     constexpr int NW = KL_LOOP_THREADS / 64;
     extern __shared__ __attribute__((aligned(16))) unsigned char smem[];
     __shared__ u64 red0[NW], red1[NW];
@@ -1759,8 +1813,8 @@
     __shared__ int s_stop;
     const int tid = threadIdx.x, lane = tid & 63, wv = tid >> 6;
     const int words = (d.n + 31) / 32;
-    u64* ck0 = d.ckey0;
-    u64* ck1 = d.ckey1;
+    u64* ck0 = d.ckey0();
+    u64* ck1 = d.ckey1();
     uint32_t* s_side = nullptr;
     uint32_t* s_lock = nullptr;
     if constexpr (SMEM) {
@@ -1768,16 +1822,16 @@
         ck1 = ck0 + d.nck0;
         s_side = reinterpret_cast<uint32_t*>(ck1 + d.nck1);
         s_lock = s_side + words;
-        for (int i = tid; i < d.nck0; i += KL_LOOP_THREADS) ck0[i] = d.ckey0[i];
-        for (int i = tid; i < d.nck1; i += KL_LOOP_THREADS) ck1[i] = d.ckey1[i];
+        for (int i = tid; i < d.nck0; i += KL_LOOP_THREADS) ck0[i] = d.ckey0()[i];
+        for (int i = tid; i < d.nck1; i += KL_LOOP_THREADS) ck1[i] = d.ckey1()[i];
         for (int i = tid; i < words; i += KL_LOOP_THREADS) {
-            s_side[i] = side_word(d.side_init, d.n, i);
+            s_side[i] = side_word(d.side_init(), d.n, i);
             s_lock[i] = 0u;
         }
     }
     if (tid == 0) s_w = 0.0f;
     __syncthreads();
-    float cut = *d.cut0, best = cut;
+    float cut = *d.cut0(), best = cut;
     long long best_it = 0, it = 0;
     unsigned term = 0;
     unsigned long long tph[4] = {0, 0, 0, 0}, tstamp = 0;
@@ -1791,6 +1845,7 @@
         }
     };
     for (;;) {
+        d.pin();
         stamp(-1);
         u64 k0 = 0ull, k1 = 0ull;
         for (int c = tid; c < d.nck0; c += KL_LOOP_THREADS) k0 = ck0[c] > k0 ? ck0[c] : k0;
@@ -1812,29 +1867,29 @@
         }
         if (k0 == 0ull || k1 == 0ull) break;
         const int posA = int(~uint32_t(k0 & 0xffffffffull)), posB = int(~uint32_t(k1 & 0xffffffffull));
-        const int A = d.order0[posA], B = d.order1[posB];
-        const int pa = d.rowptr[A], la = d.rowptr[A + 1] - pa;
-        const int pb = d.rowptr[B], lb = d.rowptr[B + 1] - pb;
+        const int A = d.order0()[posA], B = d.order1()[posB];
+        const int pa = d.rowptr()[A], la = d.rowptr()[A + 1] - pa;
+        const int pb = d.rowptr()[B], lb = d.rowptr()[B + 1] - pb;
         float gA = 0.f, gB = 0.f;
         if (tid == 0) {
-            gA = d.gp0[posA];
-            gB = d.gp1[posB];
-            d.gp0[posA] = __builtin_nanf("");
-            d.gp1[posB] = __builtin_nanf("");
+            gA = d.gp0()[posA];
+            gB = d.gp1()[posB];
+            d.gp0()[posA] = __builtin_nanf("");
+            d.gp1()[posB] = __builtin_nanf("");
             if constexpr (SMEM) {
                 s_side[A >> 5] |= 1u << (A & 31);
                 s_side[B >> 5] &= ~(1u << (B & 31));
                 s_lock[A >> 5] |= 1u << (A & 31);
                 s_lock[B >> 5] |= 1u << (B & 31);
             } else {
-                d.side[A] = 1;
-                d.side[B] = 0;
-                d.locked[A] = 1;
-                d.locked[B] = 1;
+                d.side()[A] = 1;
+                d.side()[B] = 0;
+                d.locked()[A] = 1;
+                d.locked()[B] = 1;
             }
         }
         for (int i = tid; i < la; i += KL_LOOP_THREADS)
-            if (d.col[pa + i] == B) s_w = d.w[pa + i];
+            if (d.col()[pa + i] == B) s_w = d.w()[pa + i];
         __syncthreads();
         stamp(1);
         if (tid == 0) {
@@ -1856,23 +1911,23 @@
             s_stop = stop;
         }
         for (int i = tid; i < la + lb; i += KL_LOOP_THREADS) {
-            const int u = i < la ? d.col[pa + i] : d.col[pb + i - la];
+            const int u = i < la ? d.col()[pa + i] : d.col()[pb + i - la];
             bool lk;
             if constexpr (SMEM) lk = (s_lock[u >> 5] >> (u & 31)) & 1u;
-            else lk = d.locked[u] != 0;
+            else lk = d.locked()[u] != 0;
             if (!lk) {
-                const float g = row_gain<SMEM>(d.rowptr, d.col, d.w, s_side, d.side, u, nullptr);
-                const uint32_t pl = d.plist[u];
-                ((pl >> 31) ? d.gp1 : d.gp0)[pl & 0x7fffffffu] = g;
+                const float g = row_gain<SMEM>(d.rowptr(), d.col(), d.w(), s_side, d.side(), u, nullptr);
+                const uint32_t pl = d.plist()[u];
+                ((pl >> 31) ? d.gp1() : d.gp0())[pl & 0x7fffffffu] = g;
             }
         }
         __syncthreads();
         stamp(2);
         for (int i = wv; i < la + lb + 2; i += NW) {
-            const int u = i < la ? d.col[pa + i] : i < la + lb ? d.col[pb + i - la] : (i == la + lb ? A : B);
-            const uint32_t pl = d.plist[u];
+            const int u = i < la ? d.col()[pa + i] : i < la + lb ? d.col()[pb + i - la] : (i == la + lb ? A : B);
+            const uint32_t pl = d.plist()[u];
             const int s = int(pl >> 31), c = int(pl & 0x7fffffffu) / KL_CHUNK;
-            const u64 k = s ? chunk_key(d.gp1, 1, c, lane) : chunk_key(d.gp0, 0, c, lane);
+            const u64 k = s ? chunk_key(d.gp1(), 1, c, lane) : chunk_key(d.gp0(), 0, c, lane);
             if (lane == 0) (s ? ck1 : ck0)[c] = k;
         }
         if (tid == 0) s_w = 0.0f;
@@ -1882,12 +1937,12 @@
     }
     if constexpr (SMEM) {
         __syncthreads();
-        for (int u = tid; u < d.n; u += KL_LOOP_THREADS) d.side[u] = uint8_t((s_side[u >> 5] >> (u & 31)) & 1u);
+        for (int u = tid; u < d.n; u += KL_LOOP_THREADS) d.side()[u] = uint8_t((s_side[u >> 5] >> (u & 31)) & 1u);
     }
     if (tid == 0) {
         out->iterations = it;
         out->best_iter = best_it;
-        out->initial_cut = *d.cut0;
+        out->initial_cut = *d.cut0();
         out->best_cut = best;
         out->final_cut = cut;
         out->status = SMEM ? 1u : 0u;
@@ -2153,45 +2208,89 @@
     if (acc == 0x7fffabcd) sink[0] = acc;
 }
 
+KLArgs kl_args(const KLDev& d) {
+    KLArgs a;
+    a.base = d.arena;
+    auto put = [&](int k, const void* p) {
+        if (!p) return;
+        const auto* q = static_cast<const unsigned char*>(p);
+        const size_t o = size_t(q - d.arena);
+        if (!d.arena || q < d.arena || o > d.arena_bytes || (o & 15) != 0 || (o >> KL_ARENA_UNIT_SHIFT) > UINT32_MAX)
+            fail(EK_ESTATE, "KL loop: array %d is not in the KL arena", k);
+        a.off[k] = uint32_t(o >> KL_ARENA_UNIT_SHIFT);
+    };
+    put(KA_SEGC, d.segc);
+    put(KA_SEG, d.seg);
+    put(KA_AUX, d.aux);
+    put(KA_PINFO0, d.pinfo0);
+    put(KA_PINFO1, d.pinfo1);
+    put(KA_ND, d.nd);
+    put(KA_CINFO0, d.cinfo0);
+    put(KA_CINFO1, d.cinfo1);
+    put(KA_CKEY0, d.ckey0);
+    put(KA_CKEY1, d.ckey1);
+    put(KA_GP0, d.gp0);
+    put(KA_GP1, d.gp1);
+    put(KA_COL, d.col);
+    put(KA_W, d.w);
+    put(KA_WDICT, d.wdict);
+    put(KA_LOCKED, d.locked);
+    put(KA_SIDE_INIT, d.side_init);
+    put(KA_SIDE, d.side);
+    put(KA_CUT0, d.cut0);
+    put(KA_ROWPTR, d.rowptr);
+    put(KA_ORDER0, d.order0);
+    put(KA_ORDER1, d.order1);
+    put(KA_PLIST, d.plist);
+    a.n = d.n;
+    a.n0 = d.n0;
+    a.n1 = d.n1;
+    a.nck0 = d.nck0;
+    a.nck1 = d.nck1;
+    a.nwd = d.nwd;
+    a.wcolbits = d.wcolbits;
+    a.has_seg = d.seg != nullptr;
+    a.nnz = d.nnz;
+    return a;
+}
+
 void kl_loop(hipStream_t s, const KLDev& d_in, int limit, ek_swap* log, long long cap, KLOut* out) {
     const LoopForm form = loop_form(d_in);
     const KLDev d = with_chunk(d_in, form.ch);
     const size_t lds = form.lds, lds_gb = form.lds_gb;
     if (!std::getenv("EK_KL_NOTOUCH")) {
         int* sink = reinterpret_cast<int*>(&out->prof[13]);
-        if (d.segc)
-            hipLaunchKernelGGL(k_touch, dim3(4096), dim3(256), 0, s, reinterpret_cast<const int4*>(d.segc),
-                               (long long)d.nnz * KL_SEGC_PIECES, sink);
-        else if (d.seg)
-            hipLaunchKernelGGL(k_touch, dim3(4096), dim3(256), 0, s, reinterpret_cast<const int4*>(d.seg),
-                               (long long)d.nnz * KL_SEG_LANES, sink);
-        hipLaunchKernelGGL(k_touch, dim3(1024), dim3(256), 0, s, reinterpret_cast<const int4*>(d.aux), (long long)d.nnz,
-                           sink);
-    }
+        const KLInfo* sg = d.segc ? d.segc : d.seg;
+        const KLInfo* first = sg ? sg : d.aux;
+        const long long n16 = (d.aux + d.nnz) - first;
+        if (n16 > 0)
+            hipLaunchKernelGGL(k_touch, dim3(4096), dim3(256), 0, s, reinterpret_cast<const int4*>(first), n16, sink);
+    }
+    const KLArgs a = kl_args(d);
     const bool prof = std::getenv("EK_KL_PROF") != nullptr;
     const char* pe = std::getenv("EK_KL_PIPE");
     const bool pipe = pe && pe[0] ? pe[0] != '0' : false;
     if (lds && pipe && !std::getenv("EK_KL_GLOBAL_STATE")) {
         if (prof && d.segc)
-            hipLaunchKernelGGL((k_kl_swap_pipe<true, true>), dim3(1), dim3(KL_LOOP_THREADS), lds, s, d, limit, log, cap, out);
+            hipLaunchKernelGGL((k_kl_swap_pipe<true, true>), dim3(1), dim3(KL_LOOP_THREADS), lds, s, a, limit, log, cap, out);
         else if (prof)
-            hipLaunchKernelGGL((k_kl_swap_pipe<true, false>), dim3(1), dim3(KL_LOOP_THREADS), lds, s, d, limit, log, cap, out);
+            hipLaunchKernelGGL((k_kl_swap_pipe<true, false>), dim3(1), dim3(KL_LOOP_THREADS), lds, s, a, limit, log, cap, out);
         else if (d.segc)
-            hipLaunchKernelGGL((k_kl_swap_pipe<false, true>), dim3(1), dim3(KL_LOOP_THREADS), lds, s, d, limit, log, cap, out);
+            hipLaunchKernelGGL((k_kl_swap_pipe<false, true>), dim3(1), dim3(KL_LOOP_THREADS), lds, s, a, limit, log, cap, out);
         else
-            hipLaunchKernelGGL((k_kl_swap_pipe<false, false>), dim3(1), dim3(KL_LOOP_THREADS), lds, s, d, limit, log, cap, out);
+            hipLaunchKernelGGL((k_kl_swap_pipe<false, false>), dim3(1), dim3(KL_LOOP_THREADS), lds, s, a, limit, log, cap, out);
         return;
     }
     const bool global_state = std::getenv("EK_KL_GLOBAL_STATE") != nullptr;
     if (!lds && lds_gb) {
         if (prof && d.segc)
-            hipLaunchKernelGGL((k_kl_swap_loop<true, true, true>), dim3(1), dim3(KL_LOOP_THREADS), lds_gb, s, d, limit,
+            hipLaunchKernelGGL((k_kl_swap_loop<true, true, true>), dim3(1), dim3(KL_LOOP_THREADS), lds_gb, s, a, limit,
                                log, cap, out);
         else if (d.segc)
-            hipLaunchKernelGGL((k_kl_swap_loop<false, true, true>), dim3(1), dim3(KL_LOOP_THREADS), lds_gb, s, d, limit,
+            hipLaunchKernelGGL((k_kl_swap_loop<false, true, true>), dim3(1), dim3(KL_LOOP_THREADS), lds_gb, s, a, limit,
                                log, cap, out);
         else
-            hipLaunchKernelGGL((k_kl_swap_loop<false, false, true>), dim3(1), dim3(KL_LOOP_THREADS), lds_gb, s, d, limit,
+            hipLaunchKernelGGL((k_kl_swap_loop<false, false, true>), dim3(1), dim3(KL_LOOP_THREADS), lds_gb, s, a, limit,
                                log, cap, out);
         return;
     }
@@ -2199,27 +2298,27 @@
     const size_t lds_fix = lds && !global_state && !prof && !(fx && fx[0] == '0') ? kl_loop_lds_bytes(d, true, true) : 0;
     if (lds_fix) {
         if (d.segc)
-            hipLaunchKernelGGL((k_kl_swap_loop<false, true, false, true>), dim3(1), dim3(KL_LOOP_THREADS), lds_fix, s, d,
+            hipLaunchKernelGGL((k_kl_swap_loop<false, true, false, true>), dim3(1), dim3(KL_LOOP_THREADS), lds_fix, s, a,
                                limit, log, cap, out);
         else
-            hipLaunchKernelGGL((k_kl_swap_loop<false, false, false, true>), dim3(1), dim3(KL_LOOP_THREADS), lds_fix, s, d,
+            hipLaunchKernelGGL((k_kl_swap_loop<false, false, false, true>), dim3(1), dim3(KL_LOOP_THREADS), lds_fix, s, a,
                                limit, log, cap, out);
         return;
     }
     if (lds && !global_state && prof && d.segc)
-        hipLaunchKernelGGL((k_kl_swap_loop<true, true>), dim3(1), dim3(KL_LOOP_THREADS), lds, s, d, limit, log, cap, out);
+        hipLaunchKernelGGL((k_kl_swap_loop<true, true>), dim3(1), dim3(KL_LOOP_THREADS), lds, s, a, limit, log, cap, out);
     else if (lds && !global_state && prof)
-        hipLaunchKernelGGL((k_kl_swap_loop<true, false>), dim3(1), dim3(KL_LOOP_THREADS), lds, s, d, limit, log, cap, out);
+        hipLaunchKernelGGL((k_kl_swap_loop<true, false>), dim3(1), dim3(KL_LOOP_THREADS), lds, s, a, limit, log, cap, out);
     else if (lds && !global_state && d.segc)
-        hipLaunchKernelGGL((k_kl_swap_loop<false, true>), dim3(1), dim3(KL_LOOP_THREADS), lds, s, d, limit, log, cap,
+        hipLaunchKernelGGL((k_kl_swap_loop<false, true>), dim3(1), dim3(KL_LOOP_THREADS), lds, s, a, limit, log, cap,
                            out);
     else if (lds && !global_state)
-        hipLaunchKernelGGL((k_kl_swap_loop<false, false>), dim3(1), dim3(KL_LOOP_THREADS), lds, s, d, limit, log, cap,
+        hipLaunchKernelGGL((k_kl_swap_loop<false, false>), dim3(1), dim3(KL_LOOP_THREADS), lds, s, a, limit, log, cap,
                            out);
     else if (prof)
-        hipLaunchKernelGGL((k_kl_loop<false, true>), dim3(1), dim3(KL_LOOP_THREADS), 0, s, d, limit, log, cap, out);
+        hipLaunchKernelGGL((k_kl_loop<false, true>), dim3(1), dim3(KL_LOOP_THREADS), 0, s, a, limit, log, cap, out);
     else
-        hipLaunchKernelGGL((k_kl_loop<false, false>), dim3(1), dim3(KL_LOOP_THREADS), 0, s, d, limit, log, cap, out);
+        hipLaunchKernelGGL((k_kl_loop<false, false>), dim3(1), dim3(KL_LOOP_THREADS), 0, s, a, limit, log, cap, out);
 }
 
 void kl_replay(hipStream_t s, int n, const uint8_t* side_init, const ek_swap* log, const long long* count,
```

Result: no change. 0.05999 (+0.6%).
